# austinjeng/Shift-GCN

Hardware: AMD Instinct MI355X
Metric: skeleton clips/sec fwd+bwd, NTU (3,300,25,2) bs=64; 1/2/4/8 MI355X (higher is better)
Workload: dtype fp32; 1 GPU; NTU Shift-GCN training step (fwd+CE+bwd+SGD), x=(64,3,300,25,2) per GPU; global_batch=64, per_gpu_batch=64, parallelism=dp1, hipgraph=False, world_size=1, backend=none

## Files before the change

### include/shiftgcn.h

```cpp
#ifndef SHIFTGCN_H_
#define SHIFTGCN_H_

#include <stddef.h>

#ifdef __cplusplus
extern "C" {
#endif

#define SGCN_EINVAL (-22)
#define SGCN_ABI_VERSION 23
#define SGCN_ABI_DIAG_FLAG 0x10000

int sgcn_abi_version(void);


int sgcn_tshift_fwd(const float* in, float* out, const float* xpos, const float* ypos,
                    const float* in_scale, const float* in_shift, float* plane_stats,
                    int B, int C, int H, int W, int stride, int ypos_is_raw, void* stream);

int sgcn_tshift_fwd_pre(const float* z, float* out, const float* xpos, const float* ypos,
                        const float* pre_scale, const float* pre_shift, const float* r,
                        const float* r_scale, const float* r_shift, const float* in_scale,
                        const float* in_shift, int B, int C, int H, int W, int stride,
                        int ypos_is_raw, void* stream);

int sgcn_tshift_fwd_tail(const float* in, float* out, const float* xpos, const float* ypos,
                         const float* post_scale, const float* post_shift, const float* r,
                         const float* r_scale, const float* r_shift, const float* gather_m,
                         float* out_gathered, int B, int C, int H, int W, int stride,
                         int ypos_is_raw, void* stream);

int sgcn_tshift_bwd_bnin(const float* dy, const float* y, const float* s, const float* coef,
                         const float* in, const float* xpos, const float* ypos, float* gin,
                         float* gx, float* gy, void* ws, size_t ws_bytes, int B, int C, int H,
                         int W, int ypos_is_raw, void* stream);
size_t sgcn_tshift_bwd_ws_bytes(int B, int C);

int sgcn_tshift_pos_finalize(const void* ws, int B, int C, float* gx, float* gy, void* stream);

int sgcn_tshift_bwd(const float* gout, const float* in, const float* xpos, const float* ypos,
                    const float* in_scale, const float* in_shift, int relu_mask,
                    const float* bn_mean, const float* bn_invstd, float* bn_part, float* gin,
                    float* gx, float* gy, void* ws, size_t ws_bytes, int B, int C, int H,
                    int W, int stride, int ypos_is_raw, void* stream);

int sgcn_tshift_fwd_f64(const double* in, double* out, const double* xpos, const double* ypos,
                        int B, int C, int H, int W, int stride, int ypos_is_raw, void* stream);
size_t sgcn_tshift_bwd_f64_ws_bytes(int B, int C);
int sgcn_tshift_bwd_f64(const double* gout, const double* in, const double* xpos,
                        const double* ypos, double* gin, double* gx, double* gy, void* ws,
                        size_t ws_bytes, int B, int C, int H, int W, int stride,
                        int ypos_is_raw, void* stream);

int sgcn_tshift_bwd_gbn(const float* gout, const float* in, const float* xpos,
                        const float* ypos, const float* in_scale, const float* in_shift,
                        const float* bn_mean, const float* bn_invstd, float* bn_part,
                        const float* z, const float* z_mean, const float* z_invstd,
                        float* z_part, const float* d, const float* d_mean,
                        const float* d_invstd, float* d_part, float* gin, float* gx, float* gy,
                        void* ws, size_t ws_bytes, int B, int C, int H, int W, void* stream);


int sgcn_pw_fwd(const float* w, int w_mcontig, const float* bias, const float* x,
                long long x_bstride, long long x_cstride, int x_tstride, int x_rsign,
                const float* mask, float* y, long long y_bstride, long long y_cstride,
                int y_tstride, int y_rsign, int relu, int accumulate, int B, int M, int K,
                int T, int V, void* stream);

size_t sgcn_pw_tshift_ws_bytes(int K);
int sgcn_pw_fwd_tshift(const float* w, const float* bias, const float* x, long long x_bstride,
                       long long x_cstride, const float* xpos, const float* ypos,
                       const float* in_scale, const float* in_shift, float* x_shifted,
                       void* ws, size_t ws_bytes, float* y, long long y_bstride,
                       long long y_cstride, int relu, int two_row, int B, int M, int K, int T,
                       int V, void* stream);

size_t sgcn_pw_dw_ws_bytes(int B, int M, int Nc, int T, int V);

int sgcn_pw_dw(const float* g, long long g_bstride, long long g_cstride, int g_tstride,
               int g_rsign, const float* x, long long x_bstride, long long x_cstride,
               int x_tstride, int x_rsign, const float* mask, float* dw, int dw_transpose,
               int dw_accumulate, float* dbias, int dbias_accumulate, void* ws,
               size_t ws_bytes, int B, int M, int Nc, int T, int V, void* stream);


size_t sgcn_moments_ws_bytes(int B, int C, int V, int per_joint);

int sgcn_moments(const float* x, float* part, int B, int C, int T, int V, int per_joint,
                 void* stream);


int sgcn_bn_finalize(const float* part, int B, int F, int n_part, int perm_V,
                     const float* gamma, const float* beta, float eps, float momentum,
                     float* running_mean, float* running_var, long long* num_batches,
                     float* mean, float* invstd, float* scale, float* shift, void* stream);

int sgcn_bn_eval_coef(int F, int perm_V, const float* gamma, const float* beta,
                      const float* running_mean, const float* running_var, float eps,
                      float* mean, float* invstd, float* scale, float* shift, void* stream);

int sgcn_bn_apply(const float* x, const float* scale, const float* shift, int per_joint,
                  const float* r, const float* rscale, const float* rshift, int relu,
                  float* y, float* y_stats, const float* gather_m, float* y_gathered, int B,
                  int C, int T, int V, void* stream);
int sgcn_bn_bwd_reduce(const float* dy, const float* y, int relu, const float* x,
                       const float* mean, const float* invstd, int per_joint, const float* r,
                       const float* rmean, const float* rinvstd, const float* dy_coef,
                       float* part, float* rpart, int B, int C, int T, int V, void* stream);

int sgcn_bn_bwd_finalize(const float* part, int B, int F, long long n_total, int perm_V,
                         const float* mean, const float* invstd, const float* gamma,
                         float* dgamma, float* dbeta, int accumulate, int batch_stats,
                         float* coef, void* stream);

int sgcn_bn_bwd_finalize_gbn(const float* part6, int B, int C, int V, long long n_total,
                             const float* dy_coef, const float* dy_mean, const float* mean,
                             const float* invstd, const float* gamma, float* dgamma,
                             float* dbeta, int accumulate, int batch_stats, float* coef,
                             void* stream);

int sgcn_bn_bwd_apply(const float* dy, const float* y, int relu, const float* x,
                      const float* coef, int per_joint, const float* r, const float* rcoef,
                      const float* dy_coef, float* dx, float* dr, int B, int C, int T, int V,
                      void* stream);

int sgcn_mask_prep(const float* mask, float* m, int n, void* stream);

int sgcn_gcn_gather(const float* x0, const float* m, float* xg, int B, int C, int T, int V,
                    void* stream);

int sgcn_gcn_dx_finish(const float* dxt, const float* x0, const float* m, const float* add1,
                       const float* add2, const float* add2_mask, float* dx, float* dmask_part,
                       const float* prev_s, const float* prev_mean, const float* prev_invstd,
                       float* prev_part, int B, int C, int T, int V, void* stream);

int sgcn_mask_grad_finalize(const float* part, const float* mask, int B, int C, int V,
                            float* dmask, int accumulate, void* stream);

int sgcn_modalities(const float* joint, const int* parent, float* out_joint, float* out_bone,
                    float* out_joint_motion, float* out_bone_motion, const float* scale,
                    const float* shift, int planes, int N, int C, int T, int V, int M,
                    void* stream);


size_t sgcn_head_ws_bytes(int N, int C, int V, int M);

int sgcn_head_moments(const float* x, float* part, int N, int C, int T, int V, int M,
                      void* stream);

int sgcn_head_apply(const float* x, const float* scale, const float* shift, float* y, int N,
                    int C, int T, int V, int M, void* stream);

int sgcn_head_bwd_reduce(const float* g, const float* x, const float* mean, const float* invstd,
                         float* part, int N, int C, int T, int V, int M, void* stream);

int sgcn_head_bwd_apply(const float* g, const float* x, const float* coef, float* dx, int N,
                        int C, int T, int V, int M, void* stream);

int sgcn_pool(const float* x, float* out, int N, int M, int C, long long P, void* stream);

int sgcn_pool_bwd(const float* dout, float* dx, int N, int M, int C, long long P,
                  void* stream);


int sgcn_sgd_chunk_elems(void);

int sgcn_sgd_step(const void* table, const int* numel, const int* chunks, int n_chunks,
                  float momentum, int nesterov, void* stream);

#define SGCN_BATCH_MAX 32
int sgcn_tshift_pos_finalize_many(const void* const* partials, float* const* gx,
                                  float* const* gy, const int* B, const int* C, int n,
                                  void* stream);
int sgcn_mask_prep_many(const float* const* mask, float* const* m, const int* count, int n,
                        void* stream);
int sgcn_mask_grad_finalize_many(const float* const* part, const float* const* mask,
                                 float* const* dmask, const int* B, const int* C,
                                 const int* V, int n, void* stream);

#ifdef __cplusplus
}
#endif

#endif
```

### shift-gcn_amd/csrc/bn.hip

```cpp
#include "common.hpp"

namespace sgcn {
namespace {

constexpr int kThreads = 256;

constexpr int kU = 4;

constexpr int kUM = 8;

template <bool PER_JOINT, bool ZU = false>
__global__ __launch_bounds__(kThreads) void moments_kernel(const float* __restrict__ x,
                                                            float2* __restrict__ part, int T,
                                                            int V, int C) {
  SGCN_CRIT_PRIO();
  __shared__ float s1[kThreads], s2[kThreads], red[2 * kThreads / 64];
  const int plane = gridDim.x - 1 - blockIdx.x;
  const int P = T * V;
  const float* __restrict__ xp = x + (size_t)plane * P;
  const int i = threadIdx.x;
  if (PER_JOINT) {
    const int G = kThreads / V;
    float a = 0.f, q = 0.f;
    const int v = i % V, r = i / V;
// ... 286 lines not shown
  if (OUT_STATS) {
    block_sum2(s1, s2, red);
    if (threadIdx.x == 0) {
      const float n = (float)P;
      ystats[plane] = make_float2(k0 + s1 / n, s2 - s1 * s1 / n);
    }
  }
}

template <int NT, int LPT, bool PER_JOINT, int RES, bool RELU, int OUTX, bool ZU>
__global__ __launch_bounds__(NT) void bn_apply_ja_kernel(
    const float* __restrict__ x, const float* __restrict__ scale,
    const float* __restrict__ shift, const float* __restrict__ r,
    const float* __restrict__ rscale, const float* __restrict__ rshift,
    float* __restrict__ y, float2* __restrict__ ystats, const float* __restrict__ gm,
    float* __restrict__ yg, int C, int T, int V) {
  SGCN_CRIT_PRIO();
  constexpr bool OUT_STATS = OUTX == 1, OUT_G = OUTX == 2;
  __shared__ float red[2 * NT / 64];
  const int plane = blockIdx.x, c = plane % C, rc = c % V;
  const int GR = NT / V, NTJ = GR * V, tid = threadIdx.x;
  const bool own = tid < NTJ;
  const int w = tid % V;
  const int P = T * V;
  const size_t off = (size_t)plane * P;
  const unsigned vo = own ? (unsigned)tid * 4u : 0x80000000u, vstep = (unsigned)NTJ * 4u;
  const unsigned pb = (unsigned)P * 4u;
  int wz = w - rc;
  wz = wz < 0 ? wz + V : wz;
  const unsigned xo = vo + (unsigned)((ZU ? wz - w : 0) * 4);
  const unsigned go = vo + (unsigned)((wz - w) * 4);
  float xv[LPT], rv[RES ? LPT : 1];
  {
    const auto xr = make_rsrc(x + off, pb);
#pragma unroll
    for (int e = 0; e < LPT; ++e) xv[e] = bload(xr, xo + e * vstep, 0);
    if (RES) {
      const auto rr = make_rsrc(r + off, pb);
#pragma unroll
      for (int e = 0; e < LPT; ++e) rv[e] = bload(rr, vo + e * vstep, 0);
    }
  }
  const float sc = PER_JOINT ? scale[c * V + w] : scale[c];
  const float sh = PER_JOINT ? shift[c * V + w] : shift[c];
  const float rsc = RES == 2 ? rscale[c] : 1.f, rsh = RES == 2 ? rshift[c] : 0.f;
  const float gmu = OUT_G ? gm[wz * C + c] : 0.f;
  const auto yr = make_rsrc(y + off, pb);
  const auto ygr = make_rsrc(OUT_G ? yg + off : y + off, OUT_G ? pb : 0u);
  const int nval = own ? (P - tid + NTJ - 1) / NTJ : 0;
  float s1 = 0.f;
#pragma unroll
  for (int e = 0; e < LPT; ++e) {
    float a = xv[e] * sc + sh;
    if (RES == 1) a += rv[e];
    if (RES == 2) a += rv[e] * rsc + rsh;
    if (RELU) a = fmaxf(a, 0.f);
    bstore(yr, a, vo + e * vstep, 0);
    if (OUT_G) bstore(ygr, a * gmu, go + e * vstep, 0);
    if (OUT_STATS) {
      xv[e] = e < nval ? a : 0.f;
      s1 += xv[e];
    }
  }
  if (OUT_STATS) {
    s1 = block_sum(s1, red);
    const float mean = s1 / (float)P;
    float m2 = 0.f;
#pragma unroll
    for (int e = 0; e < LPT; ++e) {
      const float d = xv[e] - mean;
      m2 += e < nval ? d * d : 0.f;
    }
    m2 = block_sum(m2, red);
    if (tid == 0) ystats[plane] = make_float2(mean, m2);
  }
}

template <bool PER_JOINT, bool RELU, bool RESBN, bool DYT>
__global__ __launch_bounds__(kThreads) void bn_bwd_reduce_kernel(
    const float* __restrict__ dy, const float* __restrict__ y, const float* __restrict__ x,
    const float* __restrict__ mean, const float* __restrict__ invstd,
    const float* __restrict__ r, const float* __restrict__ rmean,
    const float* __restrict__ rinvstd, const float* __restrict__ dyc, float2* __restrict__ part,
    float2* __restrict__ rpart, int C, int T, int V) {
  SGCN_CRIT_PRIO();
  __shared__ float s0[kThreads], s1[kThreads], red[2 * kThreads / 64];
  const int plane = blockIdx.x, c = plane % C;
  const int P = T * V;
  const size_t off = (size_t)plane * P;
  const int i = threadIdx.x;
  float rm = 0.f, ri = 0.f, d1 = 1.f, d2 = 0.f, d3 = 0.f;
  if (RESBN) { rm = rmean[c]; ri = rinvstd[c]; }
  if (DYT) { d1 = dyc[c]; d2 = dyc[C + c]; d3 = dyc[2 * C + c]; }
  float a0 = 0.f, a1 = 0.f, b0 = 0.f, b1 = 0.f;
  if (PER_JOINT) {
    const int G = kThreads / V;
    const int v = i % V, rr = i / V;
    const int vc = min(v, V - 1);
    const float mu = mean[c * V + vc], is = invstd[c * V + vc];
    int vx = v - c % V;
    vx = vx < 0 ? vx + V : vx;
    const int xd = vx - v;
    if (i < G * V) {
      for (int t0 = rr; t0 < T; t0 += G * kU) {
        float gv[kU], yv[kU], xv[kU], rv[kU];
#pragma unroll
        for (int u = 0; u < kU; ++u) {
          const int o = min(t0 + u * G, T - 1) * V + v;
          gv[u] = dy[off + o];
          if (RELU) yv[u] = y[off + o];
          xv[u] = x[off + o + xd];
          if (RESBN) rv[u] = r[off + o];
        }
#pragma unroll
        for (int u = 0; u < kU; ++u) {
          float g = gv[u];
          if (DYT) g = d1 * g + d2 * yv[u] + d3;
          g = (t0 + u * G < T) ? g : 0.f;
          if (RELU) g = yv[u] > 0.f ? g : 0.f;
          a0 += g;
          a1 += g * ((xv[u] - mu) * is);
          if (RESBN) { b0 += g; b1 += g * ((rv[u] - rm) * ri); }
        }
      }
    }
    if (RESBN) block_sum2(b0, b1, red);
    s0[i] = a0;
    s1[i] = a1;
    __syncthreads();
    if (i < V) {
      float t0 = 0.f, t1 = 0.f;
      for (int g = 0; g < G; ++g) { t0 += s0[g * V + i]; t1 += s1[g * V + i]; }
      part[(size_t)plane * V + i] = make_float2(t0, t1);
    }
    if (RESBN && i == 0) rpart[plane] = make_float2(b0, b1);
  } else {
    const float mu = mean[c], is = invstd[c];
    for (int base = 0; base < P; base += kThreads * kU) {
      float gv[kU], yv[kU], xv[kU], rv[kU];
#pragma unroll
      for (int u = 0; u < kU; ++u) {
        const int o = min(base + u * kThreads + i, P - 1);
        gv[u] = dy[off + o];
        if (RELU) yv[u] = y[off + o];
        xv[u] = x[off + o];
        if (RESBN) rv[u] = r[off + o];
      }
#pragma unroll
      for (int u = 0; u < kU; ++u) {
        float g = gv[u];
        if (DYT) g = d1 * g + d2 * yv[u] + d3;
        g = (base + u * kThreads + i < P) ? g : 0.f;
        if (RELU) g = yv[u] > 0.f ? g : 0.f;
        a0 += g;
        a1 += g * ((xv[u] - mu) * is);
        if (RESBN) { b0 += g; b1 += g * ((rv[u] - rm) * ri); }
      }
    }
    block_sum2(a0, a1, red);
    if (RESBN) block_sum2(b0, b1, red);
    if (i == 0) {
      part[plane] = make_float2(a0, a1);
      if (RESBN) rpart[plane] = make_float2(b0, b1);
    }
  }
}

template <int NT, int LPT, bool PER_JOINT, bool RELU, bool RESBN, bool DYT>
__global__ __launch_bounds__(NT) void bn_bwd_reduce_ja_kernel(
    const float* __restrict__ dy, const float* __restrict__ y, const float* __restrict__ x,
    const float* __restrict__ mean, const float* __restrict__ invstd,
    const float* __restrict__ r, const float* __restrict__ rmean,
    const float* __restrict__ rinvstd, const float* __restrict__ dyc, float2* __restrict__ part,
    float2* __restrict__ rpart, int C, int T, int V) {
  SGCN_CRIT_PRIO();
  __shared__ float s0[NT], s1[NT], red[2 * NT / 64];
  const int plane = blockIdx.x, c = plane % C;
  const int GR = NT / V, NTJ = GR * V, tid = threadIdx.x;
  const bool own = tid < NTJ;
  const int w = tid % V;
  const int P = T * V;
  const size_t off = (size_t)plane * P;
  const unsigned vo = own ? (unsigned)tid * 4u : 0x80000000u, vstep = (unsigned)NTJ * 4u;
  const unsigned pb = (unsigned)P * 4u;
  int vx = w - c % V;
  vx = vx < 0 ? vx + V : vx;
  const unsigned xo = vo + (unsigned)((PER_JOINT ? vx - w : 0) * 4);
  float gv[LPT], yv[RELU ? LPT : 1], xv[LPT], rv[RESBN ? LPT : 1];
  {
    const auto dyr = make_rsrc(dy + off, pb), xr = make_rsrc(x + off, pb);
#pragma unroll
    for (int e = 0; e < LPT; ++e) {
      gv[e] = bload(dyr, vo + e * vstep, 0);
      xv[e] = bload(xr, xo + e * vstep, 0);
    }
    if (RELU) {
      const auto yr = make_rsrc(y + off, pb);
#pragma unroll
      for (int e = 0; e < LPT; ++e) yv[e] = bload(yr, vo + e * vstep, 0);
    }
    if (RESBN) {
      const auto rr = make_rsrc(r + off, pb);
#pragma unroll
      for (int e = 0; e < LPT; ++e) rv[e] = bload(rr, vo + e * vstep, 0);
    }
  }
  float rm = 0.f, ri = 0.f, d1 = 1.f, d2 = 0.f, d3 = 0.f;
  if (RESBN) { rm = rmean[c]; ri = rinvstd[c]; }
  if (DYT) { d1 = dyc[c]; d2 = dyc[C + c]; d3 = dyc[2 * C + c]; }
  const float mu = PER_JOINT ? mean[c * V + w] : mean[c];
  const float is = PER_JOINT ? invstd[c * V + w] : invstd[c];
  const int nval = own ? (P - tid + NTJ - 1) / NTJ : 0;
  float a0 = 0.f, a1 = 0.f, b0 = 0.f, b1 = 0.f;
#pragma unroll
  for (int e = 0; e < LPT; ++e) {
    float g = gv[e];
    if (DYT) g = d1 * g + d2 * yv[e] + d3;
    g = e < nval ? g : 0.f;
    if (RELU) g = yv[e] > 0.f ? g : 0.f;
    a0 += g;
    a1 = fmaf(g, (xv[e] - mu) * is, a1);
    if (RESBN) { b0 += g; b1 = fmaf(g, (rv[e] - rm) * ri, b1); }
  }
  if (PER_JOINT) {
    if (RESBN) block_sum2(b0, b1, red);
    s0[tid] = a0;
    s1[tid] = a1;
    __syncthreads();
    if (tid < V) {
      float t0 = 0.f, t1 = 0.f;
      for (int g = 0; g < GR; ++g) { t0 += s0[g * V + tid]; t1 += s1[g * V + tid]; }
      part[(size_t)plane * V + tid] = make_float2(t0, t1);
    }
    if (RESBN && tid == 0) rpart[plane] = make_float2(b0, b1);
  } else {
    block_sum2(a0, a1, red);
    if (RESBN) block_sum2(b0, b1, red);
    if (tid == 0) {
      part[plane] = make_float2(a0, a1);
      if (RESBN) rpart[plane] = make_float2(b0, b1);
    }
  }
}

__global__ __launch_bounds__(64 * kFSW) void bn_bwd_finalize_kernel(
    const float2* __restrict__ part, int B, int F, double n_total, int perm_V,
    const float* __restrict__ mean, const float* __restrict__ invstd,
    const float* __restrict__ gamma, float* __restrict__ dgamma, float* __restrict__ dbeta,
    int accumulate, int batch_stats, float* __restrict__ coef) {
  SGCN_CRIT_PRIO();
  double sg, sgx, unused;
  int f;
  if (!feature_sums(part, B, F, sg, sgx, unused, f)) return;
  const int rf = ref_feature(f, perm_V, F);
  if (dgamma) dgamma[rf] = accumulate ? dgamma[rf] + (float)sgx : (float)sgx;
  if (dbeta) dbeta[rf] = accumulate ? dbeta[rf] + (float)sg : (float)sg;
  const float g = gamma ? gamma[rf] : 1.f;
  const float3 k = bn_bwd_coef(sg, sgx, g, invstd[f], mean[f], n_total, batch_stats);
  coef[f] = k.x;
  coef[F + f] = k.y;
  coef[2 * F + f] = k.z;
}

#ifndef SGCN_GBN_WAVES
#define SGCN_GBN_WAVES 4
#endif
constexpr int kGbnW = SGCN_GBN_WAVES;
__global__ __launch_bounds__(64 * kGbnW) void bn_bwd_finalize_gbn_kernel(
    const float* __restrict__ part6, int B, int F, int V, double n_total,
    const float* __restrict__ dyc, const float* __restrict__ dym, int C,
    const float* __restrict__ mean, const float* __restrict__ invstd,
    const float* __restrict__ gamma, float* __restrict__ dgamma, float* __restrict__ dbeta,
    int accumulate, int batch_stats, float* __restrict__ coef) {
  SGCN_CRIT_PRIO();
  __shared__ double red[kGbnW - 1][6][64];
  const int lane = threadIdx.x & 63, w = threadIdx.x >> 6;
  const int f = blockIdx.x * 64 + lane;
  const int fc = min(f, F - 1);
// ... 93 lines not shown
      }
    }
#pragma unroll
    for (int u = 0; u < kU; ++u) {
      const int o = base + u * kThreads + threadIdx.x;
      float g = gv[u];
      if (DYT) g = d1 * g + d2 * yv[u] + d3;
      if (RELU) g = yv[u] > 0.f ? g : 0.f;
      if (PER_JOINT) { k1 = k_s[v]; k2 = k_s[kThreads + v]; k3 = k_s[2 * kThreads + v]; }
      if (o < P) {
        int od = o;
        if (GATH) {
          const int w = v - rc;
          od = o - v + (w < 0 ? w + V : w);
        }
        dx[off + od] = k1 * g + k2 * xv[u] + k3;
        if (RES == 1) dr[off + o] = g;
        if (RES == 2) dr[off + o] = q1 * g + q2 * rv[u] + q3;
      }
      v += dv;
      if (v >= V) v -= V;
    }
  }
}

template <int NT, int LPT, int PJM, bool RELU, int RES, bool DYT>
__global__ __launch_bounds__(NT) void bn_bwd_apply_ja_kernel(
    const float* __restrict__ dy, const float* __restrict__ y, const float* __restrict__ x,
    const float* __restrict__ coef, int F, const float* __restrict__ r,
    const float* __restrict__ rcoef, int RF, const float* __restrict__ dyc,
    float* __restrict__ dx, float* __restrict__ dr, int C, int T, int V) {
  SGCN_CRIT_PRIO();
  static_assert(PJM == 0 || PJM == 3, "per-channel, or per-joint gathered (ZU)");
  constexpr bool PER_JOINT = PJM == 3;
  const int plane = blockIdx.x, c = plane % C, rc = c % V;
  const int GR = NT / V, NTJ = GR * V, tid = threadIdx.x;
  const bool own = tid < NTJ;
  const int w = tid % V;
  const int P = T * V;
  const size_t off = (size_t)plane * P;
  const unsigned vo = own ? (unsigned)tid * 4u : 0x80000000u, vstep = (unsigned)NTJ * 4u;
  const unsigned pb = (unsigned)P * 4u;
  int wz = w - rc;
  wz = wz < 0 ? wz + V : wz;
  const unsigned go = vo + (unsigned)((PER_JOINT ? wz - w : 0) * 4);
  float gv[LPT], yv[RELU ? LPT : 1], xv[LPT], rv[RES == 2 ? LPT : 1];
  {
    const auto dyr = make_rsrc(dy + off, pb);
    const auto xr = make_rsrc(x + off, pb);
#pragma unroll
    for (int e = 0; e < LPT; ++e) {
      gv[e] = bload(dyr, vo + e * vstep, 0);
      xv[e] = bload(xr, go + e * vstep, 0);
    }
    if (RELU) {
      const auto yr = make_rsrc(y + off, pb);
#pragma unroll
      for (int e = 0; e < LPT; ++e) yv[e] = bload(yr, vo + e * vstep, 0);
    }
    if (RES == 2) {
      const auto rr = make_rsrc(r + off, pb);
#pragma unroll
      for (int e = 0; e < LPT; ++e) rv[e] = bload(rr, vo + e * vstep, 0);
    }
  }
  const int f = PER_JOINT ? c * V + w : c;
  const float k1 = coef[f], k2 = coef[F + f], k3 = coef[2 * F + f];
  float d1 = 1.f, d2 = 0.f, d3 = 0.f, q1 = 0.f, q2 = 0.f, q3 = 0.f;
  if (DYT) { d1 = dyc[c]; d2 = dyc[C + c]; d3 = dyc[2 * C + c]; }
  if (RES == 2) { q1 = rcoef[c]; q2 = rcoef[RF + c]; q3 = rcoef[2 * RF + c]; }
  const auto dxr = make_rsrc(dx + off, pb);
  const auto drr = make_rsrc(RES ? dr + off : dx + off, RES ? pb : 0u);
#pragma unroll
  for (int e = 0; e < LPT; ++e) {
    float g = gv[e];
    if (DYT) g = d1 * g + d2 * yv[e] + d3;
    if (RELU) g = yv[e] > 0.f ? g : 0.f;
    bstore(dxr, k1 * g + k2 * xv[e] + k3, go + e * vstep, 0);
    if (RES == 1) bstore(drr, g, vo + e * vstep, 0);
    if (RES == 2) bstore(drr, q1 * g + q2 * rv[e] + q3, vo + e * vstep, 0);
  }
}

template <int NT, int LPT, bool ADD1, bool ADD2, bool PART, bool A2M>
__global__ __launch_bounds__(NT) void gcn_dx_finish_ja_kernel(
    const float* __restrict__ dxt, const float* __restrict__ x0, const float* __restrict__ m,
    const float* __restrict__ add1, const float* __restrict__ add2, float* __restrict__ dx,
    float* __restrict__ dmask_part, const float* __restrict__ ps,
    const float* __restrict__ pmean, const float* __restrict__ pinvstd,
    float2* __restrict__ bn_part, int C, int T, int V, const float* __restrict__ add2m) {
  SGCN_CRIT_PRIO();
#ifdef SGCN_DIAG_F1B_REAL
  return;
#endif
  __shared__ float s0[NT];
  __shared__ float red[2 * NT / 64];
  const int plane = blockIdx.x, c = plane % C, rc = c % V;
  const int GR = NT / V, NTJ = GR * V, tid = threadIdx.x;
  const bool own = tid < NTJ;
  const int vd = tid % V;
  int us = vd - rc;
  us = us < 0 ? us + V : us;
  const int P = T * V;
  const size_t off = (size_t)plane * P;
  const unsigned vo = own ? (unsigned)tid * 4u : 0x80000000u, vstep = (unsigned)NTJ * 4u;
  const unsigned pb = (unsigned)P * 4u;
  const unsigned uo = vo + (unsigned)((us - vd) * 4);
  float gv[LPT], xq[LPT], a1[ADD1 ? LPT : 1], a2[ADD2 ? LPT : 1], a2q[A2M ? LPT : 1];
  float sv[PART ? LPT : 1];
  {
#ifdef SGCN_DIAG_F1B_BOUND
    const auto gr = make_rsrc(dxt + off, 0u), xr = make_rsrc(x0 + off, pb);
#else
    const auto gr = make_rsrc(dxt + off, pb), xr = make_rsrc(x0 + off, pb);
#endif
#pragma unroll
    for (int e = 0; e < LPT; ++e) {
      gv[e] = bload(gr, uo + e * vstep, 0);
      xq[e] = bload(xr, vo + e * vstep, 0);
    }
    if (ADD1) {
      const auto ar = make_rsrc(add1 + off, pb);
#pragma unroll
      for (int e = 0; e < LPT; ++e) a1[e] = bload(ar, vo + e * vstep, 0);
    }
    if (ADD2) {
      const auto ar = make_rsrc(add2 + off, pb);
#pragma unroll
      for (int e = 0; e < LPT; ++e) a2[e] = bload(ar, vo + e * vstep, 0);
    }
    if (A2M) {
      const auto ar = make_rsrc(add2m + off, pb);
#pragma unroll
      for (int e = 0; e < LPT; ++e) a2q[e] = bload(ar, vo + e * vstep, 0);
    }
    if (PART) {
      const auto ar = make_rsrc(ps + off, pb);
#pragma unroll
      for (int e = 0; e < LPT; ++e) sv[e] = bload(ar, vo + e * vstep, 0);
    }
  }
  const float mu = m[us * C + c];
  float pm = 0.f, pi = 0.f;
  if (PART) { pm = pmean[c]; pi = pinvstd[c]; }
  const auto dxr = make_rsrc(dx + off, pb);
  float acc = 0.f, b0 = 0.f, b1 = 0.f;
#pragma unroll
  for (int e = 0; e < LPT; ++e) {
    float val = gv[e] * mu;
    if (ADD1) val += a1[e];
    if (ADD2) val += A2M ? (a2q[e] > 0.f ? a2[e] : 0.f) : a2[e];
    bstore(dxr, val, vo + e * vstep, 0);
    acc = fmaf(gv[e], xq[e], acc);
    if (PART) {
      const float g = xq[e] > 0.f ? val : 0.f;
      b0 += g;
      b1 = fmaf(g, (sv[e] - pm) * pi, b1);
    }
  }
  if (PART) {
    block_sum2(b0, b1, red);
    if (tid == 0) bn_part[plane] = make_float2(b0, b1);
  }
  s0[tid] = acc;
  __syncthreads();
  if (tid < V) {
    int vq = tid + rc;
    vq = vq >= V ? vq - V : vq;
    float sum = 0.f;
    for (int g = 0; g < GR; ++g) sum += s0[g * V + vq];
    dmask_part[(size_t)plane * V + tid] = sum;
  }
}

__global__ __launch_bounds__(kThreads) void gcn_gather_kernel(const float* __restrict__ x0,
                                                              const float* __restrict__ m,
                                                              float* __restrict__ xg, int C,
                                                              int T, int V) {
  SGCN_CRIT_PRIO();
  __shared__ float m_s[kThreads];
  const int plane = blockIdx.x, c = plane % C;
  const int P = T * V;
  const size_t off = (size_t)plane * P;
  const int rc = c % V;
  if ((int)threadIdx.x < V) m_s[threadIdx.x] = m[threadIdx.x * C + c];
  __syncthreads();
  const int dv = kThreads % V;
  int w = threadIdx.x % V;
  for (int base = 0; base < P; base += kThreads * kU) {
    float xv[kU], mv[kU];
    int ww = w;
#pragma unroll
    for (int u = 0; u < kU; ++u) {
      const int oraw = base + u * kThreads + (int)threadIdx.x;
      int src = ww + rc;
      src = src >= V ? src - V : src;
      xv[u] = x0[off + min(oraw - ww + src, P - 1)];
      mv[u] = m_s[ww];
      ww += dv;
      if (ww >= V) ww -= V;
    }
#pragma unroll
    for (int u = 0; u < kU; ++u) {
      const int o = base + u * kThreads + (int)threadIdx.x;
      if (o < P) xg[off + o] = xv[u] * mv[u];
    }
    w = ww;
  }
}

template <bool ADD1, bool ADD2, bool PART, bool A2M = false>
__global__ __launch_bounds__(kThreads) void gcn_dx_finish_kernel(
    const float* __restrict__ dxt, const float* __restrict__ x0, const float* __restrict__ m,
    const float* __restrict__ add1, const float* __restrict__ add2, float* __restrict__ dx,
    float* __restrict__ dmask_part, const float* __restrict__ ps,
    const float* __restrict__ pmean, const float* __restrict__ pinvstd,
    float2* __restrict__ bn_part, int C, int T, int V, const float* __restrict__ add2m) {
  SGCN_CRIT_PRIO();
  __shared__ float s0[kThreads];
  const int plane = blockIdx.x, c = plane % C;
  const size_t off = (size_t)plane * T * V;
  const int rc = c % V;
  const int i = threadIdx.x;
  const int G = kThreads / V;
  const int vd = i % V, rr = i / V;
  int us = vd - rc;
  us = us < 0 ? us + V : us;
  const float mu = m[us * C + c];
  float pm = 0.f, pi = 0.f;
  if (PART) { pm = pmean[c]; pi = pinvstd[c]; }
  float acc = 0.f, b0 = 0.f, b1 = 0.f;
  if (i < G * V) {
    for (int t0 = rr; t0 < T; t0 += G * kU) {
      float gv[kU], xq[kU], a1[kU], a2[kU], sv[kU], a2q[kU];
#pragma unroll
      for (int k = 0; k < kU; ++k) {
        const int row = min(t0 + k * G, T - 1) * V;
        gv[k] = dxt[off + row + us];
        xq[k] = x0[off + row + vd];
        if (ADD1) a1[k] = add1[off + row + vd];
        if (ADD2) a2[k] = add2[off + row + vd];
        if (A2M) a2q[k] = add2m[off + row + vd];
        if (PART) sv[k] = ps[off + row + vd];
      }
#pragma unroll
      for (int k = 0; k < kU; ++k) {
        const int t = t0 + k * G;
        float val = gv[k] * mu;
        if (ADD1) val += a1[k];
        if (ADD2) val += A2M ? (a2q[k] > 0.f ? a2[k] : 0.f) : a2[k];
        if (t < T) dx[off + t * V + vd] = val;
        acc += (t < T) ? gv[k] * xq[k] : 0.f;
        if (PART) {
          const float g = (t < T && xq[k] > 0.f) ? val : 0.f;
          b0 += g;
          b1 += g * ((sv[k] - pm) * pi);
        }
      }
    }
  }
  if (PART) {
    __shared__ float red[2 * kThreads / 64];
    block_sum2(b0, b1, red);
    if (i == 0) bn_part[plane] = make_float2(b0, b1);
  }
  s0[i] = acc;
  __syncthreads();
  if (i < V) {
    int vq = i + rc;
    vq = vq >= V ? vq - V : vq;
    float sum = 0.f;
    for (int g = 0; g < G; ++g) sum += s0[g * V + vq];
    dmask_part[(size_t)plane * V + i] = sum;
  }
}

__global__ void mask_prep_kernel(const float* __restrict__ mask, float* __restrict__ m, int n) {
  const int i = blockIdx.x * blockDim.x + threadIdx.x;
  if (i < n) m[i] = tanhf(mask[i]) + 1.f;
}

struct MaskPrepBatch {
  const float* mask[SGCN_BATCH_MAX];
  float* m[SGCN_BATCH_MAX];
  int n[SGCN_BATCH_MAX];
};
__global__ void mask_prep_many_kernel(const MaskPrepBatch t) {
  const int e = blockIdx.y;
  const int i = blockIdx.x * blockDim.x + threadIdx.x;
  if (i < t.n[e]) t.m[e][i] = tanhf(t.mask[e][i]) + 1.f;
}

__device__ __forceinline__ void mask_grad_body(const float* __restrict__ part,
                                               const float* __restrict__ mask, int B, int C,
                                               int V, float* __restrict__ dmask,
                                               int accumulate);
__global__ __launch_bounds__(64 * kFW) void mask_grad_finalize_kernel(
    const float* __restrict__ part, const float* __restrict__ mask, int B, int C, int V,
    float* __restrict__ dmask, int accumulate) {
  mask_grad_body(part, mask, B, C, V, dmask, accumulate);
}
struct MaskGradBatch {
  const float* part[SGCN_BATCH_MAX];
  const float* mask[SGCN_BATCH_MAX];
  float* dmask[SGCN_BATCH_MAX];
  int B[SGCN_BATCH_MAX];
  int C[SGCN_BATCH_MAX];
  int V[SGCN_BATCH_MAX];
};
__global__ __launch_bounds__(64 * kFW) void mask_grad_finalize_many_kernel(const MaskGradBatch t) {
  const int i = blockIdx.y;
  if ((int)blockIdx.x * kFW >= t.C[i] * t.V[i]) return;
  mask_grad_body(t.part[i], t.mask[i], t.B[i], t.C[i], t.V[i], t.dmask[i], 0);
}
__device__ __forceinline__ void mask_grad_body(const float* __restrict__ part,
                                               const float* __restrict__ mask, int B, int C,
                                               int V, float* __restrict__ dmask,
                                               int accumulate) {
  const int F = C * V;
  const int lane = threadIdx.x & 63;
  const int f = blockIdx.x * kFW + (int)(threadIdx.x >> 6);
  const int fc = min(f, F - 1);
  double a = 0.0;
  for (int b0 = lane; b0 < B; b0 += 64 * 4) {
    float pv[4];
#pragma unroll
    for (int u = 0; u < 4; ++u) {
      const int b = b0 + u * 64;
      pv[u] = b < B ? part[(size_t)b * F + fc] : 0.f;
    }
#pragma unroll
    for (int u = 0; u < 4; ++u) a += pv[u];
  }
  const double s = wave_dsum(a);
// ... 105 lines not shown
  if (per_joint == 3) SGCN_REQUIRE(relu && !y_gathered);
  {
    const int nt = T * V <= kJaSplit ? kThreads : 512;
    const int lpt = ja_lpt(T, V, nt);
    if (lpt) {
      const int ox = ys ? 1 : (y_gathered ? 2 : 0);
#define SGCN_AJ(NT, L, PJ, RS, RL, OX, ZU)                                                     \
  bn_apply_ja_kernel<NT, L, PJ, RS, RL, OX, ZU><<<g, NT, 0, st>>>(                             \
      x, scale, shift, r, rscale, rshift, y, ys, gather_m, y_gathered, C, T, V)
#define SGCN_AJ_L(NT, PJ, RS, RL, OX, ZU)                                                      \
  do {                                                                                         \
    if (lpt == 8) SGCN_AJ(NT, 8, PJ, RS, RL, OX, ZU);                                          \
    else if (lpt == 16) SGCN_AJ(NT, 16, PJ, RS, RL, OX, ZU);                                   \
    else if (lpt == 24) SGCN_AJ(NT, 24, PJ, RS, RL, OX, ZU);                                   \
    else SGCN_AJ(NT, 32, PJ, RS, RL, OX, ZU);                                                  \
  } while (0)
#define SGCN_AJ_T(PJ, RS, RL, OX, ZU)                                                          \
  do {                                                                                         \
    if (nt == kThreads) SGCN_AJ_L(kThreads, PJ, RS, RL, OX, ZU);                               \
    else SGCN_AJ_L(512, PJ, RS, RL, OX, ZU);                                                   \
  } while (0)
#define SGCN_AJ_O(PJ, RS, RL, ZU)                                                              \
  do {                                                                                         \
    if (ox == 1) SGCN_AJ_T(PJ, RS, RL, 1, ZU);                                                 \
    else if (ox == 2) SGCN_AJ_T(PJ, RS, RL, 2, ZU);                                            \
    else SGCN_AJ_T(PJ, RS, RL, 0, ZU);                                                         \
  } while (0)
      if (per_joint == 3) {
        if (ys) {
          if (res == 0) SGCN_AJ_T(true, 0, true, 1, true);
          else if (res == 1) SGCN_AJ_T(true, 1, true, 1, true);
          else SGCN_AJ_T(true, 2, true, 1, true);
        } else {
          if (res == 0) SGCN_AJ_T(true, 0, true, 0, true);
          else if (res == 1) SGCN_AJ_T(true, 1, true, 0, true);
          else SGCN_AJ_T(true, 2, true, 0, true);
        }
      } else if (relu) {
        if (res == 0) SGCN_AJ_O(false, 0, true, false);
        else if (res == 1) SGCN_AJ_O(false, 1, true, false);
        else SGCN_AJ_O(false, 2, true, false);
      } else {
        if (res == 0) SGCN_AJ_O(false, 0, false, false);
        else if (res == 1) SGCN_AJ_O(false, 1, false, false);
        else SGCN_AJ_O(false, 2, false, false);
      }
#undef SGCN_AJ_O
#undef SGCN_AJ_T
#undef SGCN_AJ_L
#undef SGCN_AJ
      SGCN_LAUNCH_CHECK();
      return 0;
    }
  }
#define SGCN_APPLY_X(PJ, RS, RL, OX)                                                        \
  bn_apply_kernel<PJ, RS, RL, OX><<<g, kThreads, 0, st>>>(x, scale, shift, r, rscale, rshift, y, \
                                                          ys, gather_m, y_gathered, C, T, V)
#define SGCN_APPLY(PJ, RS, RL)                                                               \
  (ys ? SGCN_APPLY_X(PJ, RS, RL, 1)                                                          \
      : (y_gathered ? SGCN_APPLY_X(PJ, RS, RL, 2) : SGCN_APPLY_X(PJ, RS, RL, 0)))
#define SGCN_APPLY_R(PJ, RL) \
  if (res == 0) SGCN_APPLY(PJ, 0, RL); else if (res == 1) SGCN_APPLY(PJ, 1, RL); else SGCN_APPLY(PJ, 2, RL)
  if (per_joint == 3) {
#define SGCN_APPLY_ZU(RS)                                                                      \
  (ys ? bn_apply_kernel<true, RS, true, 1, true><<<g, kThreads, 0, st>>>(                      \
            x, scale, shift, r, rscale, rshift, y, ys, gather_m, y_gathered, C, T, V)          \
      : bn_apply_kernel<true, RS, true, 0, true><<<g, kThreads, 0, st>>>(                      \
            x, scale, shift, r, rscale, rshift, y, ys, gather_m, y_gathered, C, T, V))
    if (res == 0) SGCN_APPLY_ZU(0); else if (res == 1) SGCN_APPLY_ZU(1); else SGCN_APPLY_ZU(2);
#undef SGCN_APPLY_ZU
  }
  else if (relu) { SGCN_APPLY_R(false, true); } else { SGCN_APPLY_R(false, false); }
#undef SGCN_APPLY_R
#undef SGCN_APPLY
#undef SGCN_APPLY_X
  SGCN_LAUNCH_CHECK();
  return 0;
}

int sgcn_bn_bwd_reduce(const float* dy, const float* y, int relu, const float* x,
                       const float* mean, const float* invstd, int per_joint, const float* r,
                       const float* rmean,
                       const float* rinvstd, const float* dy_coef, float* part, float* rpart,
                       int B, int C, int T, int V, void* stream) {
  SGCN_PLANE_CHECK();
  SGCN_REQUIRE(B > 0 && T > 0 && dy && x && mean && invstd && part && (y || !relu));
  SGCN_REQUIRE(!dy_coef || (y && relu));
  SGCN_REQUIRE((r == nullptr) == (rpart == nullptr) && (!r || (rmean && rinvstd)));
  SGCN_REQUIRE(per_joint == 0 || per_joint == 3);
  hipStream_t st = (hipStream_t)stream;
  dim3 g(B * C);
  const bool rb = r != nullptr;
  if (per_joint == 3) SGCN_REQUIRE(relu);
  {
    const int nt = T * V <= kJaSplit ? kThreads : 512;
    const int lpt = ja_lpt(T, V, nt);
    if (lpt) {
#define SGCN_RJ(NT, L, PJ, RL, RB)                                                             \
  (dy_coef ? bn_bwd_reduce_ja_kernel<NT, L, PJ, RL, RB, true><<<g, NT, 0, st>>>(                \
                 dy, y, x, mean, invstd, r, rmean, rinvstd, dy_coef, (float2*)part,            \
                 (float2*)rpart, C, T, V)                                                      \
           : bn_bwd_reduce_ja_kernel<NT, L, PJ, RL, RB, false><<<g, NT, 0, st>>>(               \
                 dy, y, x, mean, invstd, r, rmean, rinvstd, dy_coef, (float2*)part,            \
                 (float2*)rpart, C, T, V))
#define SGCN_RJ_L(NT, PJ, RL, RB)                                                              \
  do {                                                                                         \
    if (lpt == 8) SGCN_RJ(NT, 8, PJ, RL, RB); else if (lpt == 16) SGCN_RJ(NT, 16, PJ, RL, RB); \
    else if (lpt == 24) SGCN_RJ(NT, 24, PJ, RL, RB);                                           \
    else SGCN_RJ(NT, 32, PJ, RL, RB);                                                          \
  } while (0)
#define SGCN_RJ_T(PJ, RL, RB)                                                                  \
  do { if (nt == kThreads) SGCN_RJ_L(kThreads, PJ, RL, RB); else SGCN_RJ_L(512, PJ, RL, RB); } while (0)
      if (per_joint == 3) { if (rb) SGCN_RJ_T(true, true, true); else SGCN_RJ_T(true, true, false); }
      else if (relu) { if (rb) SGCN_RJ_T(false, true, true); else SGCN_RJ_T(false, true, false); }
      else { if (rb) SGCN_RJ_T(false, false, true); else SGCN_RJ_T(false, false, false); }
#undef SGCN_RJ_T
#undef SGCN_RJ_L
#undef SGCN_RJ
      SGCN_LAUNCH_CHECK();
      return 0;
    }
  }
#define SGCN_RED(PJ, RL, RB)                                                                \
  (dy_coef ? bn_bwd_reduce_kernel<PJ, RL, RB, true><<<g, kThreads, 0, st>>>(                   \
                 dy, y, x, mean, invstd, r, rmean, rinvstd, dy_coef, (float2*)part,           \
                 (float2*)rpart, C, T, V)                                                     \
           : bn_bwd_reduce_kernel<PJ, RL, RB, false><<<g, kThreads, 0, st>>>(                  \
                 dy, y, x, mean, invstd, r, rmean, rinvstd, dy_coef, (float2*)part,           \
                 (float2*)rpart, C, T, V))
  if (per_joint == 3) {
    if (rb) SGCN_RED(true, true, true); else SGCN_RED(true, true, false);
  } else {
    if (relu) { if (rb) SGCN_RED(false, true, true); else SGCN_RED(false, true, false); }
    else { if (rb) SGCN_RED(false, false, true); else SGCN_RED(false, false, false); }
  }
#undef SGCN_RED
  SGCN_LAUNCH_CHECK();
  return 0;
}

int sgcn_bn_bwd_finalize(const float* part, int B, int F, long long n_total, int perm_V,
                         const float* mean, const float* invstd, const float* gamma,
                         float* dgamma, float* dbeta, int accumulate, int batch_stats,
                         float* coef, void* stream) {
  SGCN_REQUIRE(part && B > 0 && F > 0 && n_total > 0 && mean && invstd && coef);
  SGCN_REQUIRE(perm_V <= 0 || F % perm_V == 0);
  bn_bwd_finalize_kernel<<<(F + 63) / 64, 64 * kFSW, 0, (hipStream_t)stream>>>(
      (const float2*)part, B, F, (double)n_total, perm_V, mean, invstd, gamma, dgamma, dbeta,
      accumulate, batch_stats, coef);
  SGCN_LAUNCH_CHECK();
  return 0;
}

int sgcn_bn_bwd_finalize_gbn(const float* part6, int B, int C, int V, long long n_total,
                             const float* dy_coef, const float* dy_mean, const float* mean,
                             const float* invstd, const float* gamma, float* dgamma,
                             float* dbeta, int accumulate, int batch_stats, float* coef,
                             void* stream) {
  SGCN_REQUIRE(part6 && B > 0 && C > 0 && V > 0 && n_total > 0 && dy_coef && dy_mean && mean &&
               invstd && coef);
  const int F = C * V;
  bn_bwd_finalize_gbn_kernel<<<(F + 63) / 64, 64 * kGbnW, 0, (hipStream_t)stream>>>(
      part6, B, F, V, (double)n_total, dy_coef, dy_mean, C, mean, invstd, gamma, dgamma, dbeta,
      accumulate, batch_stats, coef);
  SGCN_LAUNCH_CHECK();
  return 0;
}

int sgcn_bn_bwd_apply(const float* dy, const float* y, int relu, const float* x,
                      const float* coef, int per_joint, const float* r, const float* rcoef,
                      const float* dy_coef, float* dx, float* dr, int B, int C, int T, int V,
                      void* stream) {
  SGCN_PLANE_CHECK();
  if (B == 0 || T == 0) return 0;
  SGCN_REQUIRE(dy && x && coef && dx && (y || !relu));
  SGCN_REQUIRE(!dy_coef || (y && relu));
  SGCN_REQUIRE(!rcoef || (r && dr));
  SGCN_REQUIRE(per_joint == 0 || per_joint == 3);
  hipStream_t st = (hipStream_t)stream;
  const int res = dr == nullptr ? 0 : (rcoef ? 2 : 1);
  const int F = per_joint ? C * V : C;
  dim3 g(B * C);
  if (per_joint == 3) SGCN_REQUIRE(relu);
  {
    const int nt = T * V <= kJaSplit ? kThreads : 512;
    const int lpt = ja_lpt(T, V, nt);
    if (lpt) {
#define SGCN_BJ(NT, L, PJ, RL, RS)                                                             \
  (dy_coef ? bn_bwd_apply_ja_kernel<NT, L, PJ, RL, RS, true><<<g, NT, 0, st>>>(                 \
                 dy, y, x, coef, F, r, rcoef, C, dy_coef, dx, dr, C, T, V)             \
           : bn_bwd_apply_ja_kernel<NT, L, PJ, RL, RS, false><<<g, NT, 0, st>>>(                \
                 dy, y, x, coef, F, r, rcoef, C, dy_coef, dx, dr, C, T, V))
#define SGCN_BJ_L(NT, PJ, RL, RS)                                                              \
  do {                                                                                         \
    if (lpt == 8) SGCN_BJ(NT, 8, PJ, RL, RS);                                                  \
    else if (lpt == 16) SGCN_BJ(NT, 16, PJ, RL, RS);                                           \
    else if (lpt == 24) SGCN_BJ(NT, 24, PJ, RL, RS);                                           \
    else SGCN_BJ(NT, 32, PJ, RL, RS);                                                          \
  } while (0)
#define SGCN_BJ_T(PJ, RL, RS)                                                                  \
  do { if (nt == kThreads) SGCN_BJ_L(kThreads, PJ, RL, RS); else SGCN_BJ_L(512, PJ, RL, RS); } while (0)
#define SGCN_BJ_R(PJ, RL)                                                                      \
  do {                                                                                         \
    if (res == 0) SGCN_BJ_T(PJ, RL, 0);                                                        \
    else if (res == 1) SGCN_BJ_T(PJ, RL, 1);                                                   \
    else SGCN_BJ_T(PJ, RL, 2);                                                                 \
  } while (0)
      if (per_joint == 3) SGCN_BJ_R(3, true);
      else if (relu) SGCN_BJ_R(0, true);
      else SGCN_BJ_R(0, false);
#undef SGCN_BJ_R
#undef SGCN_BJ_T
// ... 2 lines not shown
      SGCN_LAUNCH_CHECK();
      return 0;
    }
  }
#define SGCN_BA(PJ, RL, RS)                                                                   \
  (dy_coef ? bn_bwd_apply_kernel<PJ, RL, RS, true><<<g, kThreads, 0, st>>>(                      \
                 dy, y, x, coef, F, r, rcoef, C, dy_coef, dx, dr, C, T, V)                      \
           : bn_bwd_apply_kernel<PJ, RL, RS, false><<<g, kThreads, 0, st>>>(                     \
                 dy, y, x, coef, F, r, rcoef, C, dy_coef, dx, dr, C, T, V))
#define SGCN_BA_R(PJ, RL) \
  if (res == 0) SGCN_BA(PJ, RL, 0); else if (res == 1) SGCN_BA(PJ, RL, 1); else SGCN_BA(PJ, RL, 2)
  if (per_joint == 3) { SGCN_BA_R(3, true); }
  else if (relu) { SGCN_BA_R(0, true); } else { SGCN_BA_R(0, false); }
#undef SGCN_BA_R
#undef SGCN_BA
  SGCN_LAUNCH_CHECK();
  return 0;
}

int sgcn_mask_prep(const float* mask, float* m, int n, void* stream) {
  SGCN_REQUIRE(mask && m && n > 0);
  mask_prep_kernel<<<(n + 255) / 256, 256, 0, (hipStream_t)stream>>>(mask, m, n);
  SGCN_LAUNCH_CHECK();
  return 0;
}

int sgcn_mask_prep_many(const float* const* mask, float* const* m, const int* count, int n,
                        void* stream) {
  SGCN_REQUIRE(n >= 0 && n <= SGCN_BATCH_MAX);
  if (n == 0) return 0;
  SGCN_REQUIRE(mask && m && count);
  MaskPrepBatch t{};
  int mx = 0;
  for (int i = 0; i < n; ++i) {
    SGCN_REQUIRE(mask[i] && m[i] && count[i] > 0);
    t.mask[i] = mask[i];
    t.m[i] = m[i];
    t.n[i] = count[i];
    mx = max(mx, count[i]);
  }
  mask_prep_many_kernel<<<dim3((mx + 255) / 256, n), 256, 0, (hipStream_t)stream>>>(t);
  SGCN_LAUNCH_CHECK();
  return 0;
}

int sgcn_mask_grad_finalize_many(const float* const* part, const float* const* mask,
                                 float* const* dmask, const int* B, const int* C,
                                 const int* V, int n, void* stream) {
  SGCN_REQUIRE(n >= 0 && n <= SGCN_BATCH_MAX);
  if (n == 0) return 0;
  SGCN_REQUIRE(part && mask && dmask && B && C && V);
  MaskGradBatch t{};
  int mf = 0;
  for (int i = 0; i < n; ++i) {
    SGCN_REQUIRE(part[i] && mask[i] && dmask[i] && B[i] > 0 && C[i] > 0 && V[i] > 0);
    t.part[i] = part[i];
    t.mask[i] = mask[i];
    t.dmask[i] = dmask[i];
    t.B[i] = B[i];
    t.C[i] = C[i];
    t.V[i] = V[i];
    mf = max(mf, C[i] * V[i]);
  }
  mask_grad_finalize_many_kernel<<<dim3((mf + kFW - 1) / kFW, n), 64 * kFW, 0,
                                   (hipStream_t)stream>>>(t);
  SGCN_LAUNCH_CHECK();
  return 0;
}

int sgcn_gcn_gather(const float* x0, const float* m, float* xg, int B, int C, int T, int V,
                    void* stream) {
  SGCN_PLANE_CHECK();
  if (B == 0 || T == 0) return 0;
  SGCN_REQUIRE(x0 && m && xg && x0 != xg);
  gcn_gather_kernel<<<B * C, kThreads, 0, (hipStream_t)stream>>>(x0, m, xg, C, T, V);
  SGCN_LAUNCH_CHECK();
  return 0;
}

int sgcn_gcn_dx_finish(const float* dxt, const float* x0, const float* m, const float* add1,
                       const float* add2, const float* add2_mask, float* dx, float* dmask_part,
                       const float* prev_s, const float* prev_mean, const float* prev_invstd,
                       float* prev_part, int B,
                       int C, int T, int V, void* stream) {
  SGCN_PLANE_CHECK();
  if (B == 0 || T == 0) return 0;
  SGCN_REQUIRE(dxt && x0 && m && dx && dmask_part);
  SGCN_REQUIRE(!prev_part || (prev_s && prev_mean && prev_invstd));
  SGCN_REQUIRE(!add2_mask || add2);
  hipStream_t st = (hipStream_t)stream;
  float2* pp = (float2*)prev_part;
  if (add2_mask) SGCN_REQUIRE(add1);
  {
    const int nt = T * V <= kJaSplit ? kThreads : 512;
    const int lpt = ja_lpt(T, V, nt);
    if (lpt) {
#define SGCN_FJ(NT, L, A1, A2, PT, AM)                                                         \
  gcn_dx_finish_ja_kernel<NT, L, A1, A2, PT, AM><<<B * C, NT, 0, st>>>(                        \
      dxt, x0, m, add1, add2, dx, dmask_part, prev_s, prev_mean, prev_invstd, pp, C, T, V,     \
      add2_mask)
#define SGCN_FJ_L(NT, A1, A2, PT, AM)                                                          \
  do {                                                                                         \
    if (lpt == 8) SGCN_FJ(NT, 8, A1, A2, PT, AM);                                              \
    else if (lpt == 16) SGCN_FJ(NT, 16, A1, A2, PT, AM);                                       \
    else if (lpt == 24) SGCN_FJ(NT, 24, A1, A2, PT, AM);                                       \
    else SGCN_FJ(NT, 32, A1, A2, PT, AM);                                                      \
  } while (0)
#define SGCN_FJ_T(A1, A2, PT, AM)                                                              \
  do { if (nt == kThreads) SGCN_FJ_L(kThreads, A1, A2, PT, AM); else SGCN_FJ_L(512, A1, A2, PT, AM); } while (0)
#define SGCN_FJ_P(A1, A2, AM)                                                                  \
  do { if (pp) SGCN_FJ_T(A1, A2, true, AM); else SGCN_FJ_T(A1, A2, false, AM); } while (0)
      if (add2_mask) SGCN_FJ_P(true, true, true);
      else if (add1) { if (add2) SGCN_FJ_P(true, true, false); else SGCN_FJ_P(true, false, false); }
      else { if (add2) SGCN_FJ_P(false, true, false); else SGCN_FJ_P(false, false, false); }
#undef SGCN_FJ_P
#undef SGCN_FJ_T
#undef SGCN_FJ_L
#undef SGCN_FJ
      SGCN_LAUNCH_CHECK();
      return 0;
    }
  }
  if (add2_mask) {
    if (pp)
      gcn_dx_finish_kernel<true, true, true, true><<<B * C, kThreads, 0, st>>>(
          dxt, x0, m, add1, add2, dx, dmask_part, prev_s, prev_mean, prev_invstd, pp, C, T, V,
          add2_mask);
    else
      gcn_dx_finish_kernel<true, true, false, true><<<B * C, kThreads, 0, st>>>(
          dxt, x0, m, add1, add2, dx, dmask_part, prev_s, prev_mean, prev_invstd, pp, C, T, V,
          add2_mask);
    SGCN_LAUNCH_CHECK();
    return 0;
  }
#define SGCN_FIN(A1, A2, PT)                                                                \
  gcn_dx_finish_kernel<A1, A2, PT><<<B * C, kThreads, 0, st>>>(                           \
      dxt, x0, m, add1, add2, dx, dmask_part, prev_s, prev_mean, prev_invstd, pp, C, T, V,  \
      nullptr)
#define SGCN_FIN_P(A1, A2)                                                                  \
  do {                                                                                      \
    if (pp) SGCN_FIN(A1, A2, true);                                                         \
    else SGCN_FIN(A1, A2, false);                                                           \
  } while (0)
  if (add1) { if (add2) SGCN_FIN_P(true, true); else SGCN_FIN_P(true, false); }
  else { if (add2) SGCN_FIN_P(false, true); else SGCN_FIN_P(false, false); }
#undef SGCN_FIN_P
#undef SGCN_FIN
  SGCN_LAUNCH_CHECK();
  return 0;
}

int sgcn_mask_grad_finalize(const float* part, const float* mask, int B, int C, int V,
                            float* dmask, int accumulate, void* stream) {
  SGCN_REQUIRE(part && mask && dmask && B > 0 && C > 0 && V > 0);
  mask_grad_finalize_kernel<<<(C * V + kFW - 1) / kFW, 64 * kFW, 0,
                              (hipStream_t)stream>>>(part, mask, B, C, V, dmask, accumulate);
  SGCN_LAUNCH_CHECK();
  return 0;
}

}
```

### shift-gcn_amd/csrc/head.hip

```cpp
#include "common.hpp"

namespace sgcn {
namespace {

constexpr int kHT = 256;
constexpr int kHU = 8;

__device__ __forceinline__ int clip_col(int j, int V, int M) {
  const int m = j / V, v = j - m * V;
  return v * M + m;
}

__global__ __launch_bounds__(kHT) void head_moments_kernel(const float* __restrict__ x,
                                                           float2* __restrict__ part, int C,
                                                           int T, int V, int M) {
  SGCN_CRIT_PRIO();
  __shared__ float s1[kHT], s2[kHT];
  const int nc = blockIdx.x, n = nc / C, c = nc - n * C;
  const int J = V * M, F = J * C;
  const float* __restrict__ xs = x + (size_t)nc * T * J;
  const int i = threadIdx.x;
  const int Jc = min(J, kHT), G = kHT / Jc;
  const int jl = i % Jc, r = i / Jc;
  for (int jb = 0; jb < J; jb += Jc) {
// ... 82 lines not shown
        for (int u = 0; u < kHU; ++u) {
          const float gg = (t0 + u * G < T) ? gv[u] : 0.f;
          a += gg;
          b += gg * ((xv[u] - mu) * is);
        }
      }
    }
    s1[i] = a;
    s2[i] = b;
    __syncthreads();
    if (i < Jc && jb + i < J) {
      float ta = 0.f, tb = 0.f;
      for (int k = 0; k < G; ++k) { ta += s1[k * Jc + i]; tb += s2[k * Jc + i]; }
      const int jj = jb + i, mm = jj / V, vv = jj - mm * V;
      part[(size_t)n * F + (mm * V + vv) * C + c] = make_float2(ta, tb);
    }
    __syncthreads();
  }
}

__global__ __launch_bounds__(kHT) void head_bwd_apply_kernel(
    const float* __restrict__ g, const float* __restrict__ x, const float* __restrict__ coef,
    float* __restrict__ dx, long long total, int C, int T, int V, int M) {
  SGCN_CRIT_PRIO();
  const long long i = (long long)blockIdx.x * kHT + threadIdx.x;
  if (i >= total) return;
  long long r = i;
  const int m = (int)(r % M); r /= M;
  const int v = (int)(r % V); r /= V;
  const int t = (int)(r % T); r /= T;
  const int c = (int)(r % C);
  const long long n = r / C;
  const int F = M * V * C, f = (m * V + v) * C + c;
  const float gv = g[(((n * M + m) * C + c) * T + t) * V + v];
  dx[i] = coef[f] * gv + coef[F + f] * x[i] + coef[2 * F + f];
}

__global__ __launch_bounds__(kHT) void pool_kernel(const float* __restrict__ x,
                                                   float* __restrict__ out, int C, int M,
                                                   long long P) {
  SGCN_CRIT_PRIO();
  __shared__ float red[2 * kHT / 64];
  const int nc = blockIdx.x, n = nc / C, c = nc - n * C;
  float acc = 0.f;
  for (int m = 0; m < M; ++m) {
    const float* __restrict__ xp = x + (((size_t)n * M + m) * C + c) * P;
    float s[4] = {0.f, 0.f, 0.f, 0.f};
    for (long long p0 = threadIdx.x; p0 < P; p0 += 4 * kHT) {
#pragma unroll
      for (int u = 0; u < 4; ++u) {
        const long long p = p0 + u * kHT;
        s[u] += p < P ? xp[p] : 0.f;
      }
    }
    float tot = (s[0] + s[1]) + (s[2] + s[3]);
    tot = block_sum(tot, red);
    acc += tot * (1.f / (float)P);
  }
  if (threadIdx.x == 0) out[nc] = acc * (1.f / (float)M);
}

__global__ __launch_bounds__(kHT) void pool_bwd_kernel(const float* __restrict__ dout,
                                                       float* __restrict__ dx, long long total,
                                                       int C, int M, long long P) {
  SGCN_CRIT_PRIO();
  const long long i0 = ((long long)blockIdx.x * kHT + threadIdx.x) * 4;
  if (i0 >= total) return;
  const float rm = 1.f / (float)M, rp = 1.f / (float)P;
  float v[4];
#pragma unroll
  for (int u = 0; u < 4; ++u) {
    const long long row = (i0 + u) / P;
    const int c = (int)(row % C);
    const long long n = row / C / M;
    v[u] = i0 + u < total ? (dout[n * C + c] * rm) * rp : 0.f;
  }
  if (i0 + 4 <= total) {
    *reinterpret_cast<float4*>(dx + i0) = make_float4(v[0], v[1], v[2], v[3]);
  } else {
    for (int u = 0; u < 4 && i0 + u < total; ++u) dx[i0 + u] = v[u];
  }
}

unsigned grid1(long long total) { return (unsigned)((total + kHT - 1) / kHT); }

}
}

using namespace sgcn;

extern "C" {

size_t sgcn_head_ws_bytes(int N, int C, int V, int M) {
  return (size_t)(N > 0 ? N : 0) * C * V * M * sizeof(float2);
}

int sgcn_head_moments(const float* x, float* part, int N, int C, int T, int V, int M,
                      void* stream) {
  SGCN_REQUIRE(N >= 0 && C > 0 && T > 0 && V > 0 && M > 0);
  if (N == 0) return 0;
  SGCN_REQUIRE(x && part);
  SGCN_REQUIRE((long long)N * C < (1ll << 31) && (long long)T * V * M < (1ll << 31));
  head_moments_kernel<<<N * C, kHT, 0, (hipStream_t)stream>>>(x, (float2*)part, C, T, V, M);
  SGCN_LAUNCH_CHECK();
  return 0;
}

int sgcn_head_apply(const float* x, const float* scale, const float* shift, float* y, int N,
                    int C, int T, int V, int M, void* stream) {
  SGCN_REQUIRE(N >= 0 && C > 0 && T > 0 && V > 0 && M > 0);
  const long long total = (long long)N * M * C * T * V;
  if (total == 0) return 0;
  SGCN_REQUIRE(x && scale && shift && y);
  SGCN_REQUIRE(total < (1ll << 40));
  head_apply_kernel<<<grid1(total), kHT, 0, (hipStream_t)stream>>>(x, scale, shift, y, total,
                                                                    C, T, V, M);
  SGCN_LAUNCH_CHECK();
  return 0;
}

int sgcn_head_bwd_reduce(const float* g, const float* x, const float* mean, const float* invstd,
                         float* part, int N, int C, int T, int V, int M, void* stream) {
  SGCN_REQUIRE(N >= 0 && C > 0 && T > 0 && V > 0 && M > 0);
  if (N == 0) return 0;
  SGCN_REQUIRE(g && x && mean && invstd && part);
  SGCN_REQUIRE((long long)N * C < (1ll << 31) && (long long)T * V * M < (1ll << 31));
  head_bwd_reduce_kernel<<<N * C, kHT, 0, (hipStream_t)stream>>>(g, x, mean, invstd,
                                                                 (float2*)part, C, T, V, M);
  SGCN_LAUNCH_CHECK();
  return 0;
}

int sgcn_head_bwd_apply(const float* g, const float* x, const float* coef, float* dx, int N,
                        int C, int T, int V, int M, void* stream) {
  SGCN_REQUIRE(N >= 0 && C > 0 && T > 0 && V > 0 && M > 0);
  const long long total = (long long)N * M * C * T * V;
  if (total == 0) return 0;
  SGCN_REQUIRE(g && x && coef && dx);
  SGCN_REQUIRE(total < (1ll << 40));
  head_bwd_apply_kernel<<<grid1(total), kHT, 0, (hipStream_t)stream>>>(g, x, coef, dx, total, C,
                                                                        T, V, M);
  SGCN_LAUNCH_CHECK();
  return 0;
}

int sgcn_pool(const float* x, float* out, int N, int M, int C, long long P, void* stream) {
  SGCN_REQUIRE(N >= 0 && M > 0 && C > 0 && P > 0);
  if (N == 0) return 0;
  SGCN_REQUIRE(x && out);
  SGCN_REQUIRE((long long)N * C < (1ll << 31));
  pool_kernel<<<N * C, kHT, 0, (hipStream_t)stream>>>(x, out, C, M, P);
  SGCN_LAUNCH_CHECK();
  return 0;
}

int sgcn_pool_bwd(const float* dout, float* dx, int N, int M, int C, long long P,
                  void* stream) {
  SGCN_REQUIRE(N >= 0 && M > 0 && C > 0 && P > 0);
  const long long total = (long long)N * M * C * P;
  if (total == 0) return 0;
  SGCN_REQUIRE(dout && dx && ((uintptr_t)dx & 15) == 0);
  SGCN_REQUIRE(total < (1ll << 40));
  pool_bwd_kernel<<<grid1((total + 3) / 4), kHT, 0, (hipStream_t)stream>>>(dout, dx, total, C,
                                                                           M, P);
  SGCN_LAUNCH_CHECK();
  return 0;
}

}
```

### shift-gcn_amd/csrc/tshift.hip

```cpp
#include "common.hpp"

#pragma clang fp contract(off)

namespace sgcn {
namespace {

constexpr int kThreads = 256;


struct Geom {
  int x1, y1;
  float dx, dy;
};

__device__ __forceinline__ Geom make_geom(float x, float y) {
  Geom g;
  g.x1 = (int)floorf(x);
  g.y1 = (int)floorf(y);
  g.dx = x - (float)g.x1;
  g.dy = y - (float)g.y1;
  return g;
}

__device__ __forceinline__ float blend(float q11, float q21, float q12, float q22, float dx,
// ... 660 lines not shown
        const int h2 = h1 + 1;
        const int hq1 = (h1 % 2 == 0) ? h1 / 2 : -1;
        const int hq2 = (h2 % 2 == 0) ? h2 / 2 : -1;
        TapIdx t1, t2;
        tap_idx(hq1, w1, Ho, W, t1);
        tap_idx(hq2, w1, Ho, W, t2);
        ti.o00 = t1.o00; ti.o01 = t1.o01; ti.m00 = t1.m00; ti.m01 = t1.m01;
        ti.o10 = t2.o00; ti.o11 = t2.o01; ti.m10 = t2.m00; ti.m11 = t2.m01;
      }
      float val = 0.f;
      if (nt > 0) {
        const float q11 = sel(gs[ti.o00], ti.m00), q21 = sel(gs[ti.o01], ti.m01);
        const float q12 = sel(gs[ti.o10], ti.m10), q22 = sel(gs[ti.o11], ti.m11);
        val = blend(q11, q21, q12, q22, r.dx, r.dy);
      }
      const float rin = xs[o];
      if (RELU_MASK) val = rin > 0.f ? val : 0.f;
      gi[o] = val;
      if (BNP) {
        bs0 += val;
        bs1 += val * ((rin - bmu) * bis);
      }
      pos.next();
    }
  }

  if (JA) {
    const Geom g = make_geom(x, y);
    const int NTJ = (NT / W) * W, GR = NT / W;
    if ((int)threadIdx.x < NTJ) {
      const int w = (int)threadIdx.x % W, wc = w + g.x1;
      const bool c0 = (unsigned)wc < (unsigned)W, c1 = (unsigned)(wc + 1) < (unsigned)W;
      const int cc0 = min(max(wc, 0), W - 1), cc1 = min(max(wc + 1, 0), W - 1);
      int h = (int)threadIdx.x / W;
      for (int o = threadIdx.x; o < nt; o += NTJ, h += GR) {
        const int rr = h * STRIDE + g.y1;
        const bool r0 = (unsigned)rr < (unsigned)Hb, r1 = (unsigned)(rr + 1) < (unsigned)Hb;
        const int p0 = min(max(rr, 0), Hb - 1) * W, p1 = min(max(rr + 1, 0), Hb - 1) * W;
        float q11 = xs[p0 + cc0], q21 = xs[p0 + cc1], q12 = xs[p1 + cc0], q22 = xs[p1 + cc1];
        if (AFFINE) { q11 = q11 * a + b; q21 = q21 * a + b; q12 = q12 * a + b; q22 = q22 * a + b; }
        q11 = (r0 && c0) ? q11 : 0.f;
        q21 = (r0 && c1) ? q21 : 0.f;
        q12 = (r1 && c0) ? q12 : 0.f;
        q22 = (r1 && c1) ? q22 : 0.f;
        const float vx = (1.f - g.dy) * (q21 - q11) + g.dy * (q22 - q12);
        const float vy = (1.f - g.dx) * (q12 - q11) + g.dx * (q22 - q21);
        const float gg = gs[o];
        ax += vx * gg;
        ay += vy * gg;
      }
    }
  } else {
    const Geom g = make_geom(x, y);
    Walker pos(threadIdx.x, NT, W);
    for (int o = threadIdx.x; o < nt; o += NT) {
      TapIdx ti;
      tap_idx(pos.h * STRIDE + g.y1, pos.w + g.x1, Hb, W, ti);
      float q11 = xs[ti.o00], q21 = xs[ti.o01], q12 = xs[ti.o10], q22 = xs[ti.o11];
      if (AFFINE) { q11 = q11 * a + b; q21 = q21 * a + b; q12 = q12 * a + b; q22 = q22 * a + b; }
      q11 = sel(q11, ti.m00);
      q21 = sel(q21, ti.m01);
      q12 = sel(q12, ti.m10);
      q22 = sel(q22, ti.m11);
      const float vx = (1.f - g.dy) * (q21 - q11) + g.dy * (q22 - q12);
      const float vy = (1.f - g.dx) * (q12 - q11) + g.dx * (q22 - q21);
      const float gg = gs[o];
      ax += vx * gg;
      ay += vy * gg;
      pos.next();
    }
  }
  if (BNP) {
    block_sum4(ax, ay, bs0, bs1, red);
    if (threadIdx.x == 0) {
      pgrad[plane] = make_float2(ax, ay);
      bn_part[plane] = make_float2(bs0, bs1);
    }
  } else {
    block_sum2(ax, ay, red);
    if (threadIdx.x == 0) pgrad[plane] = make_float2(ax, ay);
  }
}

template <int NT, int LPT, bool AFFINE, bool RELU_MASK, bool BNP, bool GP, bool GBN,
          bool GBD = false>
__global__ __launch_bounds__(NT) void tshift_bwd_ra_kernel(
    const float* __restrict__ gout, const float* __restrict__ in,
    const float* __restrict__ xpos, const float* __restrict__ ypos,
    const float* __restrict__ scale, const float* __restrict__ shift,
    const float* __restrict__ bn_mean, const float* __restrict__ bn_invstd,
    float* __restrict__ gin, float2* __restrict__ pgrad, float2* __restrict__ bn_part, int C,
    int H, int W, const float* __restrict__ gdy, const float* __restrict__ gy,
    const float* __restrict__ gx, const float* __restrict__ gcoef,
    const float* __restrict__ gz, const float* __restrict__ gzm,
    const float* __restrict__ gzi, float* __restrict__ gzpart, const float* __restrict__ gd = nullptr,
    const float* __restrict__ gdm = nullptr, const float* __restrict__ gdi = nullptr,
    float* __restrict__ gdpart = nullptr) {
  SGCN_CRIT_PRIO();
  static_assert(!GBN || (AFFINE && BNP && !GP), "GBN: shift_in with BNP");
  static_assert(!GBD || GBN, "GBD extends GBN");
  extern __shared__ float lds[];
  __shared__ float red[4 * NT / 64];
  const int plane = gridDim.x - 1 - blockIdx.x;
  const int c = plane % C;
  const int n = H * W, WP = W + 2;
  const int GR = NT / W, NTE = GR * W;
  const int tid = threadIdx.x;
  const bool own = tid < NTE;
  const int w = tid % W, h0 = tid / W;
  const unsigned vo = own ? (unsigned)tid * 4u : 0x80000000u;
  const unsigned vstep = (unsigned)NTE * 4u, nbytes = (unsigned)n * 4u;
  const size_t poff = (size_t)plane * n;
#ifdef SGCN_DIAG_X1B_BOUND
  const unsigned gbytes = AFFINE && !GP && C >= SGCN_DIAG_X1B_BOUND ? 0u : nbytes;
#else
  const unsigned gbytes = nbytes;
#endif
  float t[LPT], rin_r[LPT];
  float zr[GBN ? LPT : 1], dr[GBD ? LPT : 1];
  {
    const auto inr = make_rsrc(in + poff, nbytes);
    if (GP) {
      const auto dyr = make_rsrc(gdy + poff, nbytes);
      const auto yr = make_rsrc(gy + poff, nbytes);
      const auto xr = make_rsrc(gx + poff, nbytes);
      float u1[LPT], u2[LPT];
#pragma unroll
      for (int e = 0; e < LPT; ++e) {
        const unsigned vb = vo + e * vstep;
        t[e] = bload(dyr, vb, 0);
        u1[e] = bload(yr, vb, 0);
        u2[e] = bload(xr, vb, 0);
        rin_r[e] = bload(inr, vb, 0);
      }
      const float k1 = gcoef[c], k2 = gcoef[C + c], k3 = gcoef[2 * C + c];
#pragma unroll
      for (int e = 0; e < LPT; ++e) t[e] = k1 * (u1[e] > 0.f ? t[e] : 0.f) + k2 * u2[e] + k3;
    } else {
      const auto gr = make_rsrc(gout + poff, gbytes);
#pragma unroll
      for (int e = 0; e < LPT; ++e) {
        t[e] = bload(gr, vo + e * vstep, 0);
        rin_r[e] = bload(inr, vo + e * vstep, 0);
      }
      if (GBN) {
        const auto zrr = make_rsrc(gz + poff, nbytes);
        int wz = w - c % W;
        wz = wz < 0 ? wz + W : wz;
        const unsigned zo = vo + (unsigned)((wz - w) * 4);
#pragma unroll
        for (int e = 0; e < LPT; ++e) zr[e] = bload(zrr, zo + e * vstep, 0);
      }
      if (GBD) {
        const auto drr = make_rsrc(gd + poff, nbytes);
#pragma unroll
        for (int e = 0; e < LPT; ++e) dr[e] = bload(drr, vo + e * vstep, 0);
      }
    }
  }
  zero_pad<NT>(lds, H, W);
  const int lbase = (h0 + kPadRows) * WP + w + 1, lstep = GR * WP;
  const int lspare = ra_pad_floats(H, W);
#pragma unroll
  for (int e = 0; e < LPT; ++e)
    lds[own && e * NTE + tid < n ? lbase + e * lstep : lspare] = t[e];
  float bmu = 0.f, bis = 0.f;
  if (BNP) { bmu = bn_mean[c]; bis = bn_invstd[c]; }
  const float x = xpos[c], y = ypos[c];
  float a = 1.f, b = 0.f;
  if (AFFINE) { a = scale[c]; b = shift[c]; }
  float zm = 0.f, zi = 0.f, dmu = 0.f, dis = 0.f;
  if (GBN) { zm = gzm[c * W + w]; zi = gzi[c * W + w]; }
  if (GBD) { dmu = gdm[c]; dis = gdi[c]; }
  __syncthreads();

  const Geom r = make_geom(-x, -y);
  const Geom g = make_geom(x, y);
  const bool fits = r.y1 >= -kPadRows && r.y1 <= kPadRows - 1 && g.y1 >= -kPadRows &&
                    g.y1 <= kPadRows - 1 && r.x1 >= -1 && r.x1 <= 0 && g.x1 >= -1 && g.x1 <= 0;
  const int kq = r.y1 * WP + r.x1, kg = (-g.y1 - 1) * WP - g.x1 - 1;
  const int nfull = n / NTE;
  const int lmax = (H - 1 + kPadRows) * WP + W;
  const auto gir = make_rsrc(gin + poff, nbytes);
  float bs0 = 0.f, bs1 = 0.f, ax = 0.f, ay = 0.f;
  float a6[6] = {0.f, 0.f, 0.f, 0.f, 0.f, 0.f};
  float d6[6] = {0.f, 0.f, 0.f, 0.f, 0.f, 0.f};
  auto elem = [&](int e, bool tail, float q11, float q21, float q12, float q22, float G11,
                  float G21, float G12, float G22) {
    const bool ok = !tail || e * NTE + tid < n;
    float val = blend(q11, q21, q12, q22, r.dx, r.dy);
    const float rin = rin_r[e];
    if (RELU_MASK) val = rin > 0.f ? val : 0.f;
    if (tail) val = ok ? val : 0.f;
    bstore(gir, val, vo + e * vstep, 0);
    if (GBN) {
      const bool act = rin > 0.f;
      const float hc = act ? rin - bmu : 0.f, zh = act ? (zr[e] - zm) * zi : 0.f;
      const float vv = act ? val : 0.f;
      a6[0] += vv;
      a6[1] += hc;
      a6[2] += act ? 1.f : 0.f;
      a6[3] = fmaf(vv, zh, a6[3]);
      a6[4] = fmaf(hc, zh, a6[4]);
      a6[5] += zh;
      if (GBD) {
        const float dh = act ? (dr[e] - dmu) * dis : 0.f;
        d6[0] += vv;
        d6[1] += hc;
        d6[2] += act ? 1.f : 0.f;
        d6[3] = fmaf(vv, dh, d6[3]);
        d6[4] = fmaf(hc, dh, d6[4]);
        d6[5] += dh;
      }
    }
    if (BNP) {
      bs0 += val;
      bs1 = fmaf(val, (rin - bmu) * bis, bs1);
    }
    const float cx = (1.f - g.dy) * (G21 - G11) + g.dy * (G22 - G12);
    const float cy = (1.f - g.dx) * (G12 - G11) + g.dx * (G22 - G21);
// ... 235 lines not shown
  return true;
}

template <int EPT, int STRIDE>
void launch_bwd(bool affine, bool relu, const float* gout, const float* in, const float* xpos,
                const float* ypos, const float* scale, const float* shift, const float* bmu,
                const float* bis, float* gin, float2* pg, float2* bp, int B, int C, int H,
                int W, int Ho, int add_half, hipStream_t st) {
  dim3 grid(B * C), block(kThreads);
#define SGCN_BWD(A, R, P)                                                                    \
  tshift_bwd_kernel<EPT, A, R, STRIDE, P><<<grid, block, 0, st>>>(                            \
      gout, in, xpos, ypos, scale, shift, bmu, bis, gin, pg, bp, C, H, W, Ho, add_half)
  if (bp) {
    if (affine) {
      if (relu) SGCN_BWD(true, true, true); else SGCN_BWD(true, false, true);
    } else {
      if (relu) SGCN_BWD(false, true, true); else SGCN_BWD(false, false, true);
    }
  } else {
    if (affine) {
      if (relu) SGCN_BWD(true, true, false); else SGCN_BWD(true, false, false);
    } else {
      if (relu) SGCN_BWD(false, true, false); else SGCN_BWD(false, false, false);
    }
  }
#undef SGCN_BWD
}

constexpr int kBwdThreads = 512;

template <int LPT, bool JA>
void launch_bwd_s2(bool affine, bool relu, const float* gout, const float* in,
                   const float* xpos, const float* ypos, const float* scale,
                   const float* shift, const float* bmu, const float* bis, float* gin,
                   float2* pg, float2* bp, int B, int C, int H, int W, int Ho, int add_half,
                   hipStream_t st) {
  constexpr int NT = kBwdThreads;
  dim3 grid(B * C), block(NT);
  const size_t lds = (size_t)(H + Ho) * W * sizeof(float);
#define SGCN_BWDL(A, R, P)                                                                  \
  tshift_bwd_s2_kernel<NT, LPT, A, R, P, JA><<<grid, block, lds, st>>>(                      \
      gout, in, xpos, ypos, scale, shift, bmu, bis, gin, pg, bp, C, H, W, Ho, add_half)
  if (bp) {
    if (affine) {
      if (relu) SGCN_BWDL(true, true, true); else SGCN_BWDL(true, false, true);
    } else {
      if (relu) SGCN_BWDL(false, true, true); else SGCN_BWDL(false, false, true);
    }
  } else {
    if (affine) {
      if (relu) SGCN_BWDL(true, true, false); else SGCN_BWDL(true, false, false);
    } else {
      if (relu) SGCN_BWDL(false, true, false); else SGCN_BWDL(false, false, false);
    }
  }
#undef SGCN_BWDL
}

int pick_lpt(int n, int nt) {
  const int per = (n + nt - 1) / nt;
  return per <= 8 ? 8 : (per <= 16 ? 16 : 32);
}

int ra_lpt(int n, int nt, int W) {
  const int nte = (nt / W) * W;
  if (nte <= 0 || W > 64) return 0;
  const int per = (n + nte - 1) / nte;
  if (nt == 512 && per > 8 && per <= 12) return 12;
  if (nt == 512 && per > 16 && per <= 20) return 20;
  return per <= 8 ? 8 : (per <= 16 ? 16 : (per <= 24 ? 24 : (per <= 32 ? 32 : 0)));
}

constexpr int kRaSplit256 = 8192;
#ifndef SGCN_GBD_SPLIT
#define SGCN_GBD_SPLIT 1
#endif

size_t ra_lds_bytes(int H, int W, int nt, bool gbn) {
  const int f = ra_pad_floats(H, W);
  return (size_t)(gbn ? max(f + 1, 6 * nt) : f + 1) * sizeof(float);
}
constexpr size_t kRaLdsMax = 65536;

template <bool AFFINE, bool RELU, bool BNP, bool GP, bool GBN, bool GBD = false>
bool launch_ra(int nt, const float* gout, const float* in, const float* xpos,
               const float* ypos, const float* scale, const float* shift, const float* bmu,
               const float* bis, float* gin, float2* pg, float2* bp, int B, int C, int H,
               int W, const float* gdy, const float* gy, const float* gx, const float* gcoef,
               const float* gz, const float* gzm, const float* gzi, float* gzpart,
               hipStream_t st, const float* gd = nullptr, const float* gdm = nullptr,
               const float* gdi = nullptr, float* gdpart = nullptr) {
  const int lpt = ra_lpt(H * W, nt, W);
  const size_t lds = ra_lds_bytes(H, W, nt, GBN);
  if (lpt == 0 || lds > kRaLdsMax) return false;
#define SGCN_RA(NT, L)                                                                         \
  tshift_bwd_ra_kernel<NT, L, AFFINE, RELU, BNP, GP, GBN, GBD><<<B * C, NT, lds, st>>>(        \
      gout, in, xpos, ypos, scale, shift, bmu, bis, gin, pg, bp, C, H, W, gdy, gy, gx, gcoef,  \
      gz, gzm, gzi, gzpart, gd, gdm, gdi, gdpart)
  if (nt == 256) {
    if (lpt == 8) SGCN_RA(256, 8); else if (lpt == 16) SGCN_RA(256, 16); else if (lpt == 24) SGCN_RA(256, 24); else SGCN_RA(256, 32);
  } else {
    if (lpt == 8) SGCN_RA(512, 8); else if (lpt == 12) SGCN_RA(512, 12); else if (lpt == 16) SGCN_RA(512, 16);
    else if (lpt == 20) SGCN_RA(512, 20); else if (lpt == 24) SGCN_RA(512, 24); else SGCN_RA(512, 32);
  }
#undef SGCN_RA
  return true;
}

int pick_ept(int n) {
  const int per = (n + kThreads - 1) / kThreads;
  return per <= 8 ? 8 : (per <= 16 ? 16 : 32);
}

}
}

using namespace sgcn;

extern "C" {

int sgcn_tshift_fwd(const float* in, float* out, const float* xpos, const float* ypos,
                    const float* in_scale, const float* in_shift, float* plane_stats, int B,
                    int C, int H, int W, int stride, int ypos_is_raw, void* stream) {
  SGCN_REQUIRE(B >= 0 && C > 0 && H >= 0 && W > 0 && stride >= 1);
  SGCN_REQUIRE((in_scale == nullptr) == (in_shift == nullptr));
  const int Ho = H / stride;
  if (B == 0 || Ho == 0) return 0;
  SGCN_REQUIRE(in && out && xpos && ypos);
  SGCN_REQUIRE((long long)H * W < (1LL << 30) && (long long)B * C < (1LL << 31));
  hipStream_t st = (hipStream_t)stream;
  const bool aff = in_scale != nullptr, stats = plane_stats != nullptr;
  float2* ps = (float2*)plane_stats;
  const int ah = (ypos_is_raw && stride != 1) ? 1 : 0;
  if (H * W <= kFwdLdsMax2 &&
      (H * W <= kFwdLdsMax
           ? launch_fwd_pad<kThreads>(aff, stats, in, out, xpos, ypos, in_scale, in_shift, ps, B, C, H, W, Ho, stride, ah, st)
           : launch_fwd_pad<512>(aff, stats, in, out, xpos, ypos, in_scale, in_shift, ps, B, C, H, W, Ho, stride, ah, st))) {
    SGCN_LAUNCH_CHECK();
    return 0;
  }
  if (H * W <= kFwdLdsMax) {
    switch (pick_lpt(H * W, kThreads)) {
      case 8: launch_fwd_lds<8>(aff, stats, in, out, xpos, ypos, in_scale, in_shift, ps, B, C, H, W, Ho, stride, ah, st); break;
      case 16: launch_fwd_lds<16>(aff, stats, in, out, xpos, ypos, in_scale, in_shift, ps, B, C, H, W, Ho, stride, ah, st); break;
      default: launch_fwd_lds<32>(aff, stats, in, out, xpos, ypos, in_scale, in_shift, ps, B, C, H, W, Ho, stride, ah, st); break;
    }
    SGCN_LAUNCH_CHECK();
    return 0;
  }
  if (H * W <= kFwdLdsMax2) {
    launch_fwd_lds<32, 512>(aff, stats, in, out, xpos, ypos, in_scale, in_shift, ps, B, C, H, W, Ho, stride, ah, st);
    SGCN_LAUNCH_CHECK();
    return 0;
  }
  switch (pick_ept(Ho * W)) {
    case 8: launch_fwd<8>(aff, stats, in, out, xpos, ypos, in_scale, in_shift, ps, B, C, H, W, Ho, stride, ah, st); break;
    case 16: launch_fwd<16>(aff, stats, in, out, xpos, ypos, in_scale, in_shift, ps, B, C, H, W, Ho, stride, ah, st); break;
    default: launch_fwd<32>(aff, stats, in, out, xpos, ypos, in_scale, in_shift, ps, B, C, H, W, Ho, stride, ah, st); break;
  }
  SGCN_LAUNCH_CHECK();
  return 0;
}

int sgcn_tshift_fwd_pre(const float* z, float* out, const float* xpos, const float* ypos,
                        const float* pre_scale, const float* pre_shift, const float* r,
                        const float* r_scale, const float* r_shift, const float* in_scale,
                        const float* in_shift, int B, int C, int H, int W, int stride,
                        int ypos_is_raw, void* stream) {
  SGCN_REQUIRE(B >= 0 && C > 0 && H >= 0 && W > 0 && W <= 1024 && stride >= 1);
  SGCN_REQUIRE((r_scale == nullptr) == (r_shift == nullptr));
  SGCN_REQUIRE(H * W <= kFwdLdsMax2);
  const int Ho = H / stride;
  if (B == 0 || Ho == 0) return 0;
  SGCN_REQUIRE(z && out && xpos && ypos && pre_scale && pre_shift && r && in_scale &&
               in_shift && out != z);
  SGCN_REQUIRE((long long)B * C < (1LL << 31));
  hipStream_t st = (hipStream_t)stream;
  const int ah = (ypos_is_raw && stride != 1) ? 1 : 0;
  {
    const int nt = H * W <= kFwdLdsMax ? kThreads : 512;
    const int lpt = pad_fwd_lpt(H, W, nt);
// ... 33 lines not shown
    }
  } else {
    SGCN_PRE_R(512, 32);
  }
#undef SGCN_PRE_R
#undef SGCN_PRE
  SGCN_LAUNCH_CHECK();
  return 0;
}

int sgcn_tshift_fwd_tail(const float* in, float* out, const float* xpos, const float* ypos,
                         const float* post_scale, const float* post_shift, const float* r,
                         const float* r_scale, const float* r_shift, const float* gather_m,
                         float* out_gathered, int B, int C, int H, int W, int stride,
                         int ypos_is_raw, void* stream) {
  SGCN_REQUIRE(B >= 0 && C > 0 && H >= 0 && W > 0 && W <= 1024 && stride >= 1);
  SGCN_REQUIRE((r_scale == nullptr) == (r_shift == nullptr) && (r || !r_scale));
  SGCN_REQUIRE((gather_m == nullptr) == (out_gathered == nullptr));
  SGCN_REQUIRE(H * W <= kFwdLdsMax2);
  const int Ho = H / stride;
  if (B == 0 || Ho == 0) return 0;
  SGCN_REQUIRE(in && out && xpos && ypos && post_scale && post_shift && out != in);
  SGCN_REQUIRE((long long)B * C < (1LL << 31));
  hipStream_t st = (hipStream_t)stream;
  const int ah = (ypos_is_raw && stride != 1) ? 1 : 0;
  const int res = r == nullptr ? 0 : (r_scale ? 2 : 1);
  const bool go = out_gathered != nullptr;
  {
    const int nt = H * W <= kFwdLdsMax ? kThreads : 512;
    const int lpt = pad_fwd_lpt(H, W, nt);
    if (lpt) {
      const size_t plds = (size_t)(ra_pad_floats(H, W) + 1) * sizeof(float);
#define SGCN_TAILP(NT, L, R, G)                                                                \
  tshift_fwd_pad_kernel<NT, L, 2, false, false, R, G><<<B * C, NT, plds, st>>>(                \
      in, out, xpos, ypos, post_scale, post_shift, nullptr, C, H, W, Ho, stride, ah, nullptr,  \
      nullptr, r, r_scale, r_shift, gather_m, out_gathered)
#define SGCN_TAILP_RG(NT, L)                                                                   \
  do {                                                                                         \
    if (res == 0) { if (go) SGCN_TAILP(NT, L, 0, true); else SGCN_TAILP(NT, L, 0, false); }    \
    else if (res == 1) { if (go) SGCN_TAILP(NT, L, 1, true); else SGCN_TAILP(NT, L, 1, false); } \
    else { if (go) SGCN_TAILP(NT, L, 2, true); else SGCN_TAILP(NT, L, 2, false); }             \
  } while (0)
      if (nt == kThreads) {
        if (lpt == 8) SGCN_TAILP_RG(kThreads, 8); else if (lpt == 16) SGCN_TAILP_RG(kThreads, 16); else if (lpt == 24) SGCN_TAILP_RG(kThreads, 24); else SGCN_TAILP_RG(kThreads, 32);
      } else {
        if (lpt == 8) SGCN_TAILP_RG(512, 8); else if (lpt == 12) SGCN_TAILP_RG(512, 12); else if (lpt == 16) SGCN_TAILP_RG(512, 16);
        else if (lpt == 20) SGCN_TAILP_RG(512, 20); else if (lpt == 24) SGCN_TAILP_RG(512, 24); else SGCN_TAILP_RG(512, 32);
      }
#undef SGCN_TAILP_RG
#undef SGCN_TAILP
      SGCN_LAUNCH_CHECK();
      return 0;
    }
  }
  const size_t lds = (size_t)H * W * sizeof(float);
#define SGCN_TAIL(NT, L, R, G)                                                                \
  tshift_fwd_tail_kernel<NT, L, R, G><<<B * C, NT, lds, st>>>(                                \
      in, out, xpos, ypos, post_scale, post_shift, r, r_scale, r_shift, gather_m,            \
      out_gathered, C, H, W, Ho, stride, ah)
#define SGCN_TAIL_RG(NT, L)                                                                   \
  do {                                                                                        \
    if (res == 0) { if (go) SGCN_TAIL(NT, L, 0, true); else SGCN_TAIL(NT, L, 0, false); }     \
    else if (res == 1) { if (go) SGCN_TAIL(NT, L, 1, true); else SGCN_TAIL(NT, L, 1, false); } \
    else { if (go) SGCN_TAIL(NT, L, 2, true); else SGCN_TAIL(NT, L, 2, false); }              \
  } while (0)
  if (H * W <= kFwdLdsMax) {
    switch (pick_lpt(H * W, kThreads)) {
      case 8: SGCN_TAIL_RG(kThreads, 8); break;
      case 16: SGCN_TAIL_RG(kThreads, 16); break;
      default: SGCN_TAIL_RG(kThreads, 32); break;
    }
  } else {
    SGCN_TAIL_RG(512, 32);
  }
#undef SGCN_TAIL_RG
#undef SGCN_TAIL
  SGCN_LAUNCH_CHECK();
  return 0;
}

int sgcn_tshift_bwd_bnin(const float* dy, const float* y, const float* s, const float* coef,
                         const float* in, const float* xpos, const float* ypos, float* gin,
                         float* gx, float* gy, void* ws, size_t ws_bytes, int B, int C, int H,
                         int W, int ypos_is_raw, void* stream) {
  SGCN_REQUIRE(B > 0 && C > 0 && H > 0 && W > 0);
  SGCN_REQUIRE(H * W <= kBwdLdsMax);
  SGCN_REQUIRE(dy && y && s && coef && in && xpos && ypos && gin && ws);
  SGCN_REQUIRE((gx == nullptr) == (gy == nullptr));
  SGCN_REQUIRE(ws_bytes >= sgcn_tshift_bwd_ws_bytes(B, C));
  SGCN_REQUIRE((long long)B * C < (1LL << 31));
  (void)ypos_is_raw;
  hipStream_t st = (hipStream_t)stream;
  float2* pg = (float2*)ws;
  const int ntb = H * W <= 4096 ? 256 : 512;
  const bool ok = launch_ra<false, true, false, true, false>(
      ntb, nullptr, in, xpos, ypos, nullptr, nullptr, nullptr, nullptr, gin, pg, nullptr, B, C,
      H, W, dy, y, s, coef, nullptr, nullptr, nullptr, nullptr, st);
  SGCN_REQUIRE(ok);
  SGCN_LAUNCH_CHECK();
  if (gx) tshift_pos_finalize_kernel<<<(C + 3) / 4, 256, 0, st>>>(pg, B, C, gx, gy);
  SGCN_LAUNCH_CHECK();
  return 0;
}

size_t sgcn_tshift_bwd_ws_bytes(int B, int C) { return (size_t)B * C * sizeof(float2); }

int sgcn_tshift_pos_finalize_many(const void* const* partials, float* const* gx,
                                  float* const* gy, const int* B, const int* C, int n,
                                  void* stream) {
  SGCN_REQUIRE(n >= 0 && n <= SGCN_BATCH_MAX);
  if (n == 0) return 0;
  SGCN_REQUIRE(partials && gx && gy && B && C);
  PosBatch t{};
  int max_c = 0;
  for (int i = 0; i < n; ++i) {
    SGCN_REQUIRE(partials[i] && gx[i] && gy[i] && B[i] > 0 && C[i] > 0);
    t.p[i] = (const float2*)partials[i];
    t.gx[i] = gx[i];
    t.gy[i] = gy[i];
    t.B[i] = B[i];
    t.C[i] = C[i];
    max_c = max(max_c, C[i]);
  }
  tshift_pos_finalize_many_kernel<<<dim3((max_c + 3) / 4, n), 256, 0, (hipStream_t)stream>>>(t);
  SGCN_LAUNCH_CHECK();
  return 0;
}

int sgcn_tshift_pos_finalize(const void* ws, int B, int C, float* gx, float* gy, void* stream) {
  SGCN_REQUIRE(B > 0 && C > 0 && ws && gx && gy);
  tshift_pos_finalize_kernel<<<(C + 3) / 4, 256, 0, (hipStream_t)stream>>>((const float2*)ws, B,
                                                                           C, gx, gy);
  SGCN_LAUNCH_CHECK();
  return 0;
}

int sgcn_tshift_bwd_gbn(const float* gout, const float* in, const float* xpos,
                        const float* ypos, const float* in_scale, const float* in_shift,
                        const float* bn_mean, const float* bn_invstd, float* bn_part,
                        const float* z, const float* z_mean, const float* z_invstd,
                        float* z_part, const float* d, const float* d_mean,
                        const float* d_invstd, float* d_part, float* gin, float* gx, float* gy,
                        void* ws, size_t ws_bytes, int B, int C, int H, int W, void* stream) {
  SGCN_REQUIRE(B > 0 && C > 0 && H > 0 && W > 0 && W <= 64);
  SGCN_REQUIRE((d == nullptr) == (d_part == nullptr) && (!d || (d_mean && d_invstd)));
  SGCN_REQUIRE(H * W <= kBwdLdsMax);
  SGCN_REQUIRE(gout && in && xpos && ypos && in_scale && in_shift && bn_mean && bn_invstd &&
               bn_part && z && z_mean && z_invstd && z_part && gin && ws);
  SGCN_REQUIRE((gx == nullptr) == (gy == nullptr));
  SGCN_REQUIRE(ws_bytes >= sgcn_tshift_bwd_ws_bytes(B, C));
  SGCN_REQUIRE((long long)B * C < (1LL << 31));
  hipStream_t st = (hipStream_t)stream;
  float2* pg = (float2*)ws;
  float2* bp = (float2*)bn_part;
  const int n = H * W;
  const int l256 = n <= kRaSplit256 ? ra_lpt(n, 256, W) : 0;
  const int ntg = l256 && !(SGCN_GBD_SPLIT && d && l256 > 24) ? 256 : kBwdThreads;
  const bool ok =
      d ? launch_ra<true, false, true, false, true, true>(
              ntg, gout, in, xpos, ypos, in_scale, in_shift, bn_mean, bn_invstd, gin, pg, bp, B,
              C, H, W, nullptr, nullptr, nullptr, nullptr, z, z_mean, z_invstd, z_part, st, d,
              d_mean, d_invstd, d_part)
        : launch_ra<true, false, true, false, true>(
              ntg, gout, in, xpos, ypos, in_scale, in_shift, bn_mean, bn_invstd, gin, pg, bp, B,
              C, H, W, nullptr, nullptr, nullptr, nullptr, z, z_mean, z_invstd, z_part, st);
  SGCN_REQUIRE(ok);
  SGCN_LAUNCH_CHECK();
  if (gx) tshift_pos_finalize_kernel<<<(C + 3) / 4, 256, 0, st>>>(pg, B, C, gx, gy);
  SGCN_LAUNCH_CHECK();
  return 0;
}

int sgcn_tshift_bwd(const float* gout, const float* in, const float* xpos, const float* ypos,
                    const float* in_scale, const float* in_shift, int relu_mask,
                    const float* bn_mean, const float* bn_invstd, float* bn_part, float* gin,
                    float* gx, float* gy, void* ws, size_t ws_bytes, int B, int C, int H,
                    int W, int stride, int ypos_is_raw, void* stream) {
  SGCN_REQUIRE(B > 0 && C > 0 && H >= 0 && W > 0 && (stride == 1 || stride == 2));
  SGCN_REQUIRE((in_scale == nullptr) == (in_shift == nullptr));
  const int Ho = H / stride;
// ... 60 lines not shown
```

### shift-gcn_amd/shiftgcn/_lib.py

```python
from __future__ import annotations

import ctypes
import os

import torch

LIB_NAME = "libshiftgcn_hip.so"
LIB_PATH = os.path.join(os.path.dirname(os.path.abspath(__file__)), LIB_NAME)
LIB_PATH = os.environ.get("SGCN_LIB_PATH", LIB_PATH)
ABI_VERSION = 23
BATCH_MAX = 32
ABI_DIAG_FLAG = 0x10000
EINVAL = -22

_lib = None

_P = ctypes.c_void_p
_I = ctypes.c_int
_F = ctypes.c_float
_Z = ctypes.c_size_t
_L = ctypes.c_longlong

SIGNATURES = {
    "sgcn_abi_version": (_I, []),
    "sgcn_sgd_chunk_elems": (_I, []),
    "sgcn_sgd_step": (_I, [_P, _P, _P, _I, _F, _I, _P]),
    "sgcn_tshift_fwd": (_I, [_P, _P, _P, _P, _P, _P, _P, _I, _I, _I, _I, _I, _I, _P]),
    "sgcn_tshift_fwd_pre": (_I, [_P, _P, _P, _P, _P, _P, _P, _P, _P, _P, _P, _I, _I, _I, _I,
                                 _I, _I, _P]),
    "sgcn_tshift_fwd_tail": (_I, [_P, _P, _P, _P, _P, _P, _P, _P, _P, _P, _P, _I, _I, _I, _I,
                                  _I, _I, _P]),
    "sgcn_tshift_bwd_ws_bytes": (_Z, [_I, _I]),
    "sgcn_tshift_pos_finalize": (_I, [_P, _I, _I, _P, _P, _P]),
    "sgcn_tshift_bwd": (_I, [_P, _P, _P, _P, _P, _P, _I, _P, _P, _P, _P, _P, _P, _P, _Z, _I,
                             _I, _I, _I, _I, _I, _P]),
    "sgcn_tshift_fwd_f64": (_I, [_P, _P, _P, _P, _I, _I, _I, _I, _I, _I, _P]),
    "sgcn_tshift_bwd_f64_ws_bytes": (_Z, [_I, _I]),
    "sgcn_tshift_bwd_f64": (_I, [_P, _P, _P, _P, _P, _P, _P, _P, _Z, _I, _I, _I, _I, _I, _I,
                                 _P]),
    "sgcn_pw_fwd": (_I, [_P, _I, _P, _P, _L, _L, _I, _I, _P, _P, _L, _L, _I, _I, _I, _I, _I,
                         _I, _I, _I, _I, _P]),
    "sgcn_pw_tshift_ws_bytes": (_Z, [_I]),
    "sgcn_pw_fwd_tshift": (_I, [_P, _P, _P, _L, _L, _P, _P, _P, _P, _P, _P, _Z, _P, _L, _L, _I,
                                _I, _I, _I, _I, _I, _I, _P]),
    "sgcn_pw_dw_ws_bytes": (_Z, [_I, _I, _I, _I, _I]),
    "sgcn_pw_dw": (_I, [_P, _L, _L, _I, _I, _P, _L, _L, _I, _I, _P, _P, _I, _I, _P, _I, _P, _Z,
                        _I, _I, _I, _I, _I, _P]),
    "sgcn_moments_ws_bytes": (_Z, [_I, _I, _I, _I]),
    "sgcn_moments": (_I, [_P, _P, _I, _I, _I, _I, _I, _P]),
    "sgcn_bn_finalize": (_I, [_P, _I, _I, _I, _I, _P, _P, _F, _F, _P, _P, _P, _P, _P, _P, _P,
                              _P]),
    "sgcn_bn_eval_coef": (_I, [_I, _I, _P, _P, _P, _P, _F, _P, _P, _P, _P, _P]),
    "sgcn_bn_apply": (_I, [_P, _P, _P, _I, _P, _P, _P, _I, _P, _P, _P, _P, _I, _I, _I, _I,
                           _P]),
    "sgcn_bn_bwd_reduce": (_I, [_P, _P, _I, _P, _P, _P, _I, _P, _P, _P, _P, _P, _P, _I, _I, _I,
                                _I, _P]),
    "sgcn_bn_bwd_finalize": (_I, [_P, _I, _I, _L, _I, _P, _P, _P, _P, _P, _I, _I, _P, _P]),
    "sgcn_bn_bwd_apply": (_I, [_P, _P, _I, _P, _P, _I, _P, _P, _P, _P, _P, _I, _I, _I, _I,
                               _P]),
    "sgcn_mask_prep": (_I, [_P, _P, _I, _P]),
    "sgcn_gcn_gather": (_I, [_P, _P, _P, _I, _I, _I, _I, _P]),
    "sgcn_gcn_dx_finish": (_I, [_P, _P, _P, _P, _P, _P, _P, _P, _P, _P, _P, _P, _I, _I, _I, _I,
                                _P]),
    "sgcn_tshift_bwd_bnin": (_I, [_P, _P, _P, _P, _P, _P, _P, _P, _P, _P, _P, _Z, _I, _I, _I,
                                  _I, _I, _P]),
    "sgcn_mask_grad_finalize": (_I, [_P, _P, _I, _I, _I, _P, _I, _P]),
    "sgcn_modalities": (_I, [_P, _P, _P, _P, _P, _P, _P, _P, _I, _I, _I, _I, _I, _I, _P]),
    "sgcn_tshift_bwd_gbn": (_I, [_P, _P, _P, _P, _P, _P, _P, _P, _P, _P, _P, _P, _P, _P, _P, _P,
                                 _P, _P, _P, _P, _P, _Z, _I, _I, _I, _I, _P]),
    "sgcn_bn_bwd_finalize_gbn": (_I, [_P, _I, _I, _I, _L, _P, _P, _P, _P, _P, _P, _P, _I, _I,
                                      _P, _P]),
    "sgcn_head_ws_bytes": (_Z, [_I, _I, _I, _I]),
    "sgcn_head_moments": (_I, [_P, _P, _I, _I, _I, _I, _I, _P]),
    "sgcn_head_apply": (_I, [_P, _P, _P, _P, _I, _I, _I, _I, _I, _P]),
    "sgcn_head_bwd_reduce": (_I, [_P, _P, _P, _P, _P, _I, _I, _I, _I, _I, _P]),
    "sgcn_head_bwd_apply": (_I, [_P, _P, _P, _P, _I, _I, _I, _I, _I, _P]),
    "sgcn_pool": (_I, [_P, _P, _I, _I, _I, _L, _P]),
    "sgcn_pool_bwd": (_I, [_P, _P, _I, _I, _I, _L, _P]),
    "sgcn_tshift_pos_finalize_many": (_I, [_P, _P, _P, _P, _P, _I, _P]),
    "sgcn_mask_prep_many": (_I, [_P, _P, _P, _I, _P]),
    "sgcn_mask_grad_finalize_many": (_I, [_P, _P, _P, _P, _P, _P, _I, _P]),
}


class NativeLibraryError(RuntimeError):
    pass


def _open(path):
    lib = ctypes.CDLL(path, mode=ctypes.RTLD_LOCAL)
    lib.sgcn_abi_version.restype = _I
    lib.sgcn_abi_version.argtypes = []
    abi = lib.sgcn_abi_version()
    if abi & ABI_DIAG_FLAG:
        if os.environ.get("SGCN_ALLOW_DIAG_LIB") != "1" or os.path.basename(path) == LIB_NAME:
            raise NativeLibraryError(
                f"{path} is a DIAGNOSTIC build (SGCN_PW_DIAG / SGCN_PW_STAMPS / SGCN_DIAG_*: "
                "its results are wrong); rebuild with `make -C shift-gcn_amd/csrc`")
        abi &= ~ABI_DIAG_FLAG
    if abi != ABI_VERSION:
        raise NativeLibraryError(f"{path}: ABI version {abi} != {ABI_VERSION}; rebuild it")
    for name, (res, args) in SIGNATURES.items():
        fn = getattr(lib, name)
        fn.restype = res
        fn.argtypes = args
    return lib


def load():
    global _lib
    if _lib is not None:
        return _lib
    if not os.path.exists(LIB_PATH):
        raise NativeLibraryError(
            f"{LIB_PATH} not found: build it with `python -c 'import __graft_entry__ as g; "
            f"g.build()'` (or `make -C shift-gcn_amd/csrc`). There is no CPU fallback.")
    _lib = _open(LIB_PATH)
    return _lib


def check(rc: int, name: str) -> None:
    if rc == 0:
        return
    if rc == EINVAL:
        raise ValueError(f"{name}: invalid argument (shape/pointer/stride)")
    raise RuntimeError(f"{name}: HIP error {rc}")
```

### shift-gcn_amd/shiftgcn/fused.py

```python
from __future__ import annotations

import os
import threading

import torch

from . import ops
from .ops import PlaneView as PV


def _empty(*shape, like):
    return torch.empty(shape, device=like.device, dtype=torch.float32)


_SIDE = {}


def _side_stream(device):
    s = _SIDE.get(device)
    if s is None:
        s = _SIDE[device] = torch.cuda.Stream(device=device)
    return s


# ... 114 lines not shown
def _pos_grads(gx, gy, shift):
    if not isinstance(gx, ops.PosPartials):
        return gx, gy
    ox, oy = ops.grad_like(shift.xpos), ops.grad_like(shift.ypos)
    if BATCH_SIDE:
        _task(gx.ws.device).pos.append((gx, ox, oy))
    else:
        with _OffPath(True, gx.ws):
            gx.finalize(ox, oy)
    return _Later(ox), _Later(oy)


def _pos_alloc(shift, off):
    return None if off else (ops.grad_like(shift.xpos), ops.grad_like(shift.ypos))


TAIL_MAIN = int(os.environ.get("SGCN_TAIL_MAIN", "3"))


class GcnSaved:
    __slots__ = ("x0", "xg", "Z", "zst", "D0", "dst", "H", "m", "h_moments")


def gcn_forward(mod, x0, training, off=False):
    B, Cin, T, V = x0.shape
    Cout = mod.out_channels
    D0 = dst = None
    if mod.has_down:
        conv, bn = mod.down[0], mod.down[1]
        D0 = _empty(B, Cout, T, V, like=x0)
        down = _OffPath(off, x0)
        with down:
            ops.pw_fwd(conv.weight, False, conv.bias, PV(x0), PV(D0), Cout, Cin, T, V)
            if training:
                dst = ops.bn_finalize(ops.moments(D0, False), B, Cout, T * V, bn)
            else:
                dst = ops.bn_eval_coef(bn, Cout)
    cache = mod.__dict__.pop("_gather_cache", None)
    if cache is not None and cache[0] is x0:
        xg, m = cache[1], cache[2]
    else:
        m = _mask_of(mod)
        xg = ops.gcn_gather(x0, m)
    Z = _empty(B, Cout, T, V, like=x0)
    ops.pw_fwd(mod.Linear_weight, True, mod.Linear_bias, PV(xg), PV(Z), Cout, Cin, T, V)
    if training:
        zst = ops.bn_finalize(ops.moments(Z, 3), B, Cout * V, T, mod.bn, perm_V=V)
    else:
        zst = ops.bn_eval_coef(mod.bn, Cout * V, perm_V=V)
    if mod.has_down:
        down.wait()
        H, hm = ops.bn_apply(Z, zst, 3, r=D0, rst=dst, relu=True, out_stats=training)
    else:
        H, hm = ops.bn_apply(Z, zst, 3, r=x0, relu=True, out_stats=training)
    s = GcnSaved()
    s.x0, s.xg, s.Z, s.zst, s.D0, s.dst, s.H, s.m = x0, xg, Z, zst, D0, dst, H, m
    s.h_moments = hm
    return H, s


def _mask_of(gcn):
    fm = gcn.Feature_Mask
    r = gcn.__dict__.get("_mask_ready")
    if r is not None and r[0] is fm and r[1] == fm._version:
        return r[2]
    if gcn.training:
        return ops.mask_prep(fm)
    return ops.cached(gcn, "_sgcn_mask", ops._src_key((fm,)), lambda: ops.mask_prep(fm),
                      fm.device)


def prepare_masks(gcns):
    fms = [g.Feature_Mask for g in gcns]
    if any(g.training for g in gcns):
        ms = ops.mask_prep_many(fms)
    else:
        ms = ops.cached(gcns[0], "_sgcn_masks", ops._src_key(fms) + tuple(map(id, gcns)),
                        lambda: ops.mask_prep_many(fms), fms[0].device)
    for g, m in zip(gcns, ms):
        g.__dict__["_mask_ready"] = (g.Feature_Mask, g.Feature_Mask._version, m)


def gcn_backward(mod, s: GcnSaved, dH, extra_dx=None, dy_coef=None, prev=None, extra_out=None,
                 pre6=None, off=False):
    x0 = s.x0
    B, Cin, T, V = x0.shape
    Cout = mod.out_channels
    g = {}
    rpart = None
    if pre6 is not None:
        assert dy_coef is not None and (pre6[2] is not None) == mod.has_down
        coefZ, g["bn.weight"], g["bn.bias"] = ops.bn_bwd_finalize_gbn(
            pre6[0], B, Cout, V, B * T, dy_coef, pre6[1], s.zst, mod.bn)
    else:
        if mod.has_down:
            conv, bnd = mod.down[0], mod.down[1]
            part, rpart = ops.bn_bwd_reduce(dH, s.H, True, s.Z, s.zst, 3, r=s.D0,
                                            rst=s.dst, dy_coef=dy_coef)
        else:
            part, rpart = ops.bn_bwd_reduce(dH, s.H, True, s.Z, s.zst, 3, dy_coef=dy_coef)
        coefZ, g["bn.weight"], g["bn.bias"] = ops.bn_bwd_finalize(part, B, Cout * V, B * T,
                                                                   s.zst, mod.bn, perm_V=V)
    dZ = _empty(B, Cout, T, V, like=x0)
    g_id = dD0 = None
    if mod.has_down:
        conv, bnd = mod.down[0], mod.down[1]
        if pre6 is not None:
            coefD, g["down.1.weight"], g["down.1.bias"] = ops.bn_bwd_finalize_gbn(
                pre6[2], B, Cout, 1, B * T * V, dy_coef, pre6[1], s.dst, bnd)
        else:
            coefD, g["down.1.weight"], g["down.1.bias"] = ops.bn_bwd_finalize(
                rpart, B, Cout, B * T * V, s.dst, bnd)
        dD0 = _empty(B, Cout, T, V, like=x0)
        ops.bn_bwd_apply(dH, s.H, True, s.Z, coefZ, 3, r=s.D0, rcoef=coefD, dr=dD0, dx=dZ,
                         dy_coef=dy_coef)
    else:
        g_id = _empty(B, Cin, T, V, like=x0)
        ops.bn_bwd_apply(dH, s.H, True, s.Z, coefZ, 3, dr=g_id, dx=dZ, dy_coef=dy_coef)
    dLW = ops.grad_like(mod.Linear_weight)
    dLb = ops.grad_like(mod.Linear_bias)
    dXt = _empty(B, Cin, T, V, like=x0)
    ops.pw_fwd(mod.Linear_weight, False, None, PV(dZ), PV(dXt), Cin, Cout, T, V)
    with _OffPath(off, dZ, s.xg):
        ops.pw_dw(PV(dZ), PV(s.xg), dLW, Cout, Cin, T, V, transpose=True, dbias=dLb)
    g["Linear_weight"], g["Linear_bias"] = _late(dLW, off), _late(dLb, off)
    a2, a2m = extra_dx if isinstance(extra_dx, tuple) else (extra_dx, None)
    if prev is not None:
        dx, mpart, extra_out["prev_part"] = ops.gcn_dx_finish(dXt, x0, s.m, add1=g_id,
                                                              add2=a2, prev=prev,
                                                              add2_mask=a2m)
    else:
        dx, mpart = ops.gcn_dx_finish(dXt, x0, s.m, add1=g_id, add2=a2, add2_mask=a2m)
    dmask = ops.grad_like(mod.Feature_Mask)
    fm = mod.Feature_Mask
    if BATCH_SIDE and (off or _defer_ok((fm,))):
        _task(mpart.device).mask.append((mpart, fm, B, Cin, V, dmask))
        g["Feature_Mask"] = _Later(dmask)
    else:
        with _OffPath(off, mpart):
            ops.mask_grad_finalize(mpart, fm, B, Cin, V, out=dmask)
        g["Feature_Mask"] = _late(dmask, off)
    if mod.has_down:
        dWd = ops.grad_like(conv.weight)
        dbd = ops.grad_like(conv.bias)
        ops.pw_fwd(conv.weight, True, None, PV(dD0), PV(dx), Cin, Cout, T, V, accumulate=True)
        with _OffPath(off, dD0, x0):
            ops.pw_dw(PV(dD0), PV(x0), dWd, Cout, Cin, T, V, dbias=dbd)
        g["down.0.weight"], g["down.0.bias"] = _late(dWd, off), _late(dbd, off)
    return dx, g


class TcnSaved:
    __slots__ = ("H", "ast", "As", "R", "S", "sst")


def tshift_fused(C):
    return C >= TSHIFT_FUSION_MIN_C


def folded_conv_bn(conv, bn):
    srcs = (conv.weight, conv.bias, bn.weight, bn.bias, bn.running_mean, bn.running_var)
    key = ops._src_key(srcs) + (float(bn.eps),)

    def make():
        st = ops.bn_eval_coef(bn, conv.out_channels)
        with torch.no_grad():
            w = (conv.weight.detach() *
                 st.scale.view(-1, *([1] * (conv.weight.dim() - 1)))).contiguous()
            b = (conv.bias.detach() * st.scale + st.shift if conv.bias is not None
                 else st.shift.clone())
        return w, b
    return ops.cached(conv, "_sgcn_fold", key, make, conv.weight.device)


def convbn_infer_folded(mod, x):
    B, Cin, T, V = x.shape
    conv = mod.conv
    Cout = conv.out_channels
    To = (T - 1) // mod.stride + 1
    w, b = folded_conv_bn(conv, mod.bn)
    R = _empty(B, Cout, To, V, like=x)
    ops.pw_fwd(w, False, b, PV(x, mod.stride), PV(R), Cout, Cin, To, V)
    return R


def gcn_infer_z(mod, x0):
    B, Cin, T, V = x0.shape
    Cout = mod.out_channels
    cache = mod.__dict__.pop("_gather_cache", None)
    if cache is not None and cache[0] is x0:
        xg = cache[1]
    else:
        xg = ops.gcn_gather(x0, _mask_of(mod))
    Z = _empty(B, Cout, T, V, like=x0)
    ops.pw_fwd(mod.Linear_weight, True, mod.Linear_bias, PV(xg), PV(Z, 1, +1), Cout, Cin, T, V)
    zst = ops.bn_eval_coef(mod.bn, Cout * V, perm_V=V)
    if mod.has_down:
        conv, bn = mod.down[0], mod.down[1]
        D0 = _empty(B, Cout, T, V, like=x0)
        if EVAL_FOLD:
            w, b = folded_conv_bn(conv, bn)
            ops.pw_fwd(w, False, b, PV(x0), PV(D0), Cout, Cin, T, V)
            return Z, zst, D0, None
        ops.pw_fwd(conv.weight, False, conv.bias, PV(x0), PV(D0), Cout, Cin, T, V)
        return Z, zst, D0, ops.bn_eval_coef(bn, Cout)
    return Z, zst, x0, None


def tcn_core_forward(mod, H, training, h_moments=None, tail=None, pre=None):
    src = H if H is not None else pre[0]
    B, C, T, V = src.shape
    Cout = mod.out_channels
    si, so = mod.shift_in, mod.shift_out
    stride = so.stride
    if training:
# ... 32 lines not shown
    return S, sst, s


def tcn_core_backward(mod, s: TcnSaved, dS, materialize_dx=True, gpre=None, gcn_z=None,
                      out=None, off=False):
    H = s.H
    B, C, T, V = H.shape
    Cout = mod.out_channels
    si, so = mod.shift_in, mod.shift_out
    g = {}
    if gpre is not None:
        dRp, gx, gy = ops.tshift_bwd_bnin(gpre[0], gpre[1], s.S, gpre[2], s.R,
                                          so.xpos.detach(), so.ypos.detach(), defer_pos=off,
                                          pos_out=_pos_alloc(so, off))
    else:
        dRp, gx, gy = ops.tshift_bwd(dS, s.R, so.xpos.detach(), so.ypos.detach(), so.stride,
                                     relu_mask=True, defer_pos=off,
                                     pos_out=_pos_alloc(so, off))
    g["shift_out.xpos"], g["shift_out.ypos"] = _pos_grads(gx, gy, so)
    tl = mod.temporal_linear
    dWt = ops.grad_like(tl.weight)
    dbt = ops.grad_like(tl.bias)

    dAs = _empty(B, C, T, V, like=H)
    ops.pw_fwd(tl.weight, True, None, PV(dRp), PV(dAs), C, Cout, T, V)
    with _OffPath(off, dRp, s.As):
        ops.pw_dw(PV(dRp), PV(s.As), dWt, Cout, C, T, V, dbias=dbt)
    g["temporal_linear.weight"], g["temporal_linear.bias"] = _late(dWt, off), _late(dbt, off)
    if gcn_z is not None and GBN_FUSION and si.stride == 1 and ops.ra_fits(T * V, V):
        down = gcn_z[2] if len(gcn_z) > 2 else None
        res = ops.tshift_bwd_gbn(dAs, H, si.xpos.detach(), si.ypos.detach(), s.ast, gcn_z[0],
                                 gcn_z[1], defer_pos=off, down=down,
                                 pos_out=_pos_alloc(si, off))
        dA, gx, gy, part, zpart = res[:5]
        out["pre6"] = (zpart, s.ast, res[5] if down is not None else None)
    else:
        dA, gx, gy, part = ops.tshift_bwd(
            dAs, H, si.xpos.detach(), si.ypos.detach(), si.stride, scale=s.ast.scale,
            shift=s.ast.shift, bn_stats=s.ast, defer_pos=off, pos_out=_pos_alloc(si, off))
    g["shift_in.xpos"], g["shift_in.ypos"] = _pos_grads(gx, gy, si)
    coef, g["bn.weight"], g["bn.bias"] = ops.bn_bwd_finalize(part, B, C, B * T * V, s.ast,
                                                             mod.bn)
    if not materialize_dx:
        return (dA, coef), g
    dH = ops.bn_bwd_apply(dA, None, False, H, coef, False)
    return dH, g


class ConvBnSaved:
    __slots__ = ("x", "Rc", "rst", "To")


def convbn_core_forward(mod, x, training):
    B, Cin, T, V = x.shape
    conv, bn = mod.conv, mod.bn
    Cout = conv.out_channels
    s_t = mod.stride
    To = (T - 1) // s_t + 1
    Rc = _empty(B, Cout, To, V, like=x)
    ops.pw_fwd(conv.weight, False, conv.bias, PV(x, s_t), PV(Rc), Cout, Cin, To, V)
    if training:
        rst = ops.bn_finalize(ops.moments(Rc, False), B, Cout, To * V, bn)
    else:
        rst = ops.bn_eval_coef(bn, Cout)
    s = ConvBnSaved()
    s.x, s.Rc, s.rst, s.To = x, Rc, rst, To
    return Rc, rst, s


def convbn_dx_and_dw(mod, s: ConvBnSaved, dRc, dx, accumulate, off=False):
    B, Cin, T, V = s.x.shape
    conv = mod.conv
    Cout = conv.out_channels
    dW = ops.grad_like(conv.weight)
    db = ops.grad_like(conv.bias)
    ops.pw_fwd(conv.weight, True, None, PV(dRc), PV(dx, mod.stride), Cin, Cout, s.To, V,
               accumulate=accumulate)
    with _OffPath(off, dRc, s.x):
        ops.pw_dw(PV(dRc), PV(s.x, mod.stride), dW, Cout, Cin, s.To, V, dbias=db)
    return {"conv.weight": _late(dW, off), "conv.bias": _late(db, off)}


class UnitSaved:
    __slots__ = ("x", "gs", "ts", "rs", "out", "prev", "off")


def unit_forward(unit, x, training):
    consumer = unit.__dict__.get("_gather_consumer")
    if (not training and _INFER.active and
            x.shape[2] * x.shape[3] <= ops.TAIL_MAX_PLANE):
        pre = gcn_infer_z(unit.gcn1, x)
        r = rst = None
        if unit.residual_kind == "conv":
            if EVAL_FOLD:
                r = convbn_infer_folded(unit.residual, x)
            else:
                r, rst, _ = convbn_core_forward(unit.residual, x, training)
        elif unit.residual_kind == "identity":
            r = x
        gm = _mask_of(consumer) if consumer is not None else None
        out, xg_next = tcn_core_forward(unit.tcn1, None, training, tail=(r, rst, gm),
                                        pre=pre)
        if gm is not None:
            consumer.__dict__["_gather_cache"] = (out, xg_next, gm)
        return out, None
    prev = unit.__dict__.pop("_prev_tail", None)
    prev = prev[1:] if prev is not None and prev[0] is x else None
    off = (ASYNC_DW and bool(unit.__dict__.get("_off_path")) and
           not torch.cuda.is_current_stream_capturing())
    mp = None
    if consumer is not None:
        if "_mask_ready" in consumer.__dict__:
            gm = _mask_of(consumer)
        else:
            mp = _OffPath(off, consumer.Feature_Mask)
            with mp:
                gm = ops.mask_prep(consumer.Feature_Mask)
    H, gs = gcn_forward(unit.gcn1, x, training, off=off)
    rs = None
    if unit.residual_kind == "conv":
        res = _OffPath(off, x)
        with res:
            Rc, rst, rs = convbn_core_forward(unit.residual, x, training)
    S, sst, ts = tcn_core_forward(unit.tcn1, H, training, h_moments=gs.h_moments)
    if mp is not None:
        mp.wait()
    elif consumer is None:
        gm = None
    if unit.residual_kind == "conv":
        res.wait()
        out = ops.bn_apply(S, sst, False, r=Rc, rst=rst, relu=True, gather_m=gm)
    elif unit.residual_kind == "identity":
        out = ops.bn_apply(S, sst, False, r=x, relu=True, gather_m=gm)
    else:
        out = ops.bn_apply(S, sst, False, relu=True, gather_m=gm)
    if gm is not None:
        out, xg_next = out
        consumer.__dict__["_gather_cache"] = (out, xg_next, gm)
    nxt = unit.__dict__.get("_next_unit")
    if (nxt is not None and unit.residual_kind != "conv" and nxt.residual_kind != "conv"
            and not nxt.gcn1.has_down):
        nxt.__dict__["_prev_tail"] = (out, (S, sst), unit)
    s = UnitSaved()
    s.x, s.gs, s.ts, s.rs, s.out, s.prev = x, gs, ts, rs, out, prev
    s.off = off
    return out, s


def _gcn_z(unit, s: UnitSaved):
    if unit.gcn1.has_down:
        return (s.gs.Z, s.gs.zst, (s.gs.D0, s.gs.dst)) if GBN_FUSION >= 2 else None
    return (s.gs.Z, s.gs.zst)


def _off_path_ok(unit, s: UnitSaved):
    if not s.off or torch.cuda.is_current_stream_capturing():
        return False
    if not _defer_ok([p for p in unit.parameters() if p.requires_grad]):
        return False
    _task(s.x.device).side = True
    return True


def unit_backward(unit, s: UnitSaved, dout):
    return _unit_backward(unit, s, dout, _off_path_ok(unit, s))


def _unit_backward(unit, s: UnitSaved, dout, off):
    ts = s.ts
    S = ts.S
    so = unit.tcn1.shift_out
    B, Cout, To, V = S.shape
    kind = unit.residual_kind
    g = {}
    cached = unit.__dict__.pop("_bwd_part", None)
    if cached is not None and cached[0] is dout and kind != "conv":
        part, rpart = cached[1], None
    elif kind == "conv":
        part, rpart = ops.bn_bwd_reduce(dout, s.out, True, S, ts.sst, False, r=s.rs.Rc,
                                        rst=s.rs.rst)
    else:
        part, rpart = ops.bn_bwd_reduce(dout, s.out, True, S, ts.sst, False)
    coef2, g["tcn1.bn2.weight"], g["tcn1.bn2.bias"] = ops.bn_bwd_finalize(
        part, B, Cout, B * To * V, ts.sst, unit.tcn1.bn2)
    if kind != "conv" and so.stride == 1 and ops.ra_fits(To * V, V):
        fo = {}
        (dA, coefA), gt = tcn_core_backward(unit.tcn1, ts, None, materialize_dx=False,
                                            gpre=(dout, s.out, coef2), gcn_z=_gcn_z(unit, s),
                                            out=fo, off=off)
        g.update({"tcn1." + k: v for k, v in gt.items()})
        extra = {}
        dx, gg = gcn_backward(unit.gcn1, s.gs, dA,
                              extra_dx=(dout, s.out) if kind == "identity" else None,
                              dy_coef=coefA, prev=None if s.prev is None else s.prev[0],
                              extra_out=extra, pre6=fo.get("pre6"), off=off)
        if s.prev is not None:
            s.prev[1].__dict__["_bwd_part"] = (dx, extra["prev_part"])
        g.update({"gcn1." + k: v for k, v in gg.items()})
        return dx, g
    dS = torch.empty_like(S)
    dres = None
    if kind == "conv":
        coefR, g["residual.bn.weight"], g["residual.bn.bias"] = ops.bn_bwd_finalize(
            rpart, B, Cout, B * To * V, s.rs.rst, unit.residual.bn)
        dres = torch.empty_like(s.rs.Rc)
        ops.bn_bwd_apply(dout, s.out, True, S, coef2, False, r=s.rs.Rc, rcoef=coefR, dr=dres,
                         dx=dS)
    elif kind == "identity":
        dres = torch.empty_like(s.x)
        ops.bn_bwd_apply(dout, s.out, True, S, coef2, False, dr=dres, dx=dS)
    else:
        ops.bn_bwd_apply(dout, s.out, True, S, coef2, False, dx=dS)
    fo = {}
    (dA, coefA), gt = tcn_core_backward(unit.tcn1, ts, dS, materialize_dx=False,
                                        gcn_z=_gcn_z(unit, s), out=fo, off=off)
    g.update({"tcn1." + k: v for k, v in gt.items()})
    extra = {}
    dx, gg = gcn_backward(unit.gcn1, s.gs, dA, extra_dx=dres if kind == "identity" else None,
                          dy_coef=coefA, prev=None if s.prev is None else s.prev[0],
                          extra_out=extra, pre6=fo.get("pre6"), off=off)
    if s.prev is not None:
        s.prev[1].__dict__["_bwd_part"] = (dx, extra["prev_part"])
    g.update({"gcn1." + k: v for k, v in gg.items()})
    if kind == "conv":
        gr = convbn_dx_and_dw(unit.residual, s.rs, dres, dx, accumulate=True, off=off)
        g.update({"residual." + k: v for k, v in gr.items()})
    return dx, g


TSHIFT_FUSION_MIN_C = int(os.environ.get("SGCN_TSHIFT_FUSION_MIN_C", "512"))
TSHIFT_TWO_ROW = int(os.environ.get("SGCN_TSHIFT_TWO_ROW", "2"))
EVAL_FOLD = int(os.environ.get("SGCN_EVAL_FOLD", "1"))
GBN_FUSION = int(os.environ.get("SGCN_GBN_FUSION", "2"))
ASYNC_DW = int(os.environ.get("SGCN_ASYNC_DW", "1"))


def trainable(module):
    return [(n, p) for n, p in module.named_parameters() if p.requires_grad]


class _BlockFunction(torch.autograd.Function):

    @staticmethod
    def forward(ctx, impl, module, x, *params):
        fwd, bwd = impl
        training = module.training
        y, saved = fwd(module, x.contiguous(), training)
        ctx.impl, ctx.module, ctx.saved, ctx.training = impl, module, saved, training
        tr = trainable(module)
        ctx.names, ctx.params = [n for n, _ in tr], [p for _, p in tr]
        ctx.save_for_backward(x, y)
        return y

    @staticmethod
    def backward(ctx, dy):
        ctx.saved_tensors
        if ctx.saved is None:
            raise RuntimeError(
                f"{type(ctx.module).__name__}: backward through the fused HIP block was "
                "called a second time; its saved activations are released after the first "
                "backward (retain_graph=True / double backward is not supported)")
        _, bwd = ctx.impl
        dx, grads = bwd(ctx.module, ctx.saved, dy.contiguous())
        ctx.saved = None
        out = []
        for n, p in zip(ctx.names, ctx.params):
            g = grads.get(n)
            if isinstance(g, _Later):
                _task(g.t.device).grads.append((p, g.t))
                g = None
            out.append(g)
        return (None, None, dx) + tuple(out)


class _InferFlag(threading.local):
    active = False


_INFER = _InferFlag()


def run_block(impl, module, x):
    params = [p for _, p in trainable(module)]
    prev = _INFER.active
    _INFER.active = not (torch.is_grad_enabled() and
                         (x.requires_grad or any(p.requires_grad for p in params)))
    try:
        return _BlockFunction.apply(impl, module, x, *params)
    finally:
        _INFER.active = prev


def _gcn_standalone_bwd(mod, s, dy):
    return gcn_backward(mod, s, dy)


def _tcn_standalone_fwd(mod, H, training):
    S, sst, ts = tcn_core_forward(mod, H, training)
    y = ops.bn_apply(S, sst, False)
    return y, ts


def _tcn_standalone_bwd(mod, ts, dy):
    S = ts.S
    B, C, To, V = S.shape
    part, _ = ops.bn_bwd_reduce(dy, None, False, S, ts.sst, False)
    coef, dg, db = ops.bn_bwd_finalize(part, B, C, B * To * V, ts.sst, mod.bn2)
    dS = ops.bn_bwd_apply(dy, None, False, S, coef, False)
    dH, g = tcn_core_backward(mod, ts, dS)
    g["bn2.weight"], g["bn2.bias"] = dg, db
    return dH, g


def _convbn_standalone_fwd(mod, x, training):
    Rc, rst, s = convbn_core_forward(mod, x, training)
    return ops.bn_apply(Rc, rst, False), s


def _convbn_standalone_bwd(mod, s, dy):
    B, C, To, V = s.Rc.shape
    part, _ = ops.bn_bwd_reduce(dy, None, False, s.Rc, s.rst, False)
    coef, dg, db = ops.bn_bwd_finalize(part, B, C, B * To * V, s.rst, mod.bn)
    dRc = ops.bn_bwd_apply(dy, None, False, s.Rc, coef, False)
    dx = torch.zeros_like(s.x)
    g = convbn_dx_and_dw(mod, s, dRc, dx, accumulate=True)
    g["bn.weight"], g["bn.bias"] = dg, db
    return dx, g


GCN_IMPL = (gcn_forward, _gcn_standalone_bwd)
TCN_IMPL = (_tcn_standalone_fwd, _tcn_standalone_bwd)
CONVBN_IMPL = (_convbn_standalone_fwd, _convbn_standalone_bwd)
UNIT_IMPL = (unit_forward, unit_backward)
```

### shift-gcn_amd/shiftgcn/head.py

```python
from __future__ import annotations

import torch

from . import ops


def _batch_stats(bn) -> bool:
    return bn.training or (bn.running_mean is None and bn.running_var is None)


class _DataBnFunction(torch.autograd.Function):
    @staticmethod
    def forward(ctx, x, weight, bias, bn):
        N, C, T, V, M = x.shape
        F = M * V * C
        if _batch_stats(bn):
            if N * T <= 1:
                raise ValueError("Expected more than 1 value per channel when training, got "
                                 f"input size {torch.Size([N, F, T])}")
            st = ops.bn_finalize(ops.head_moments(x), N, F, T, bn, training=bn.training)
        else:
            st = ops.bn_eval_coef(bn, F)
        ctx.save_for_backward(x)
        ctx.st, ctx.bn = st, bn
        return ops.head_apply(x, st)

    @staticmethod
    def backward(ctx, gy):
        (x,) = ctx.saved_tensors
        st, bn = ctx.st, ctx.bn
        N, C, T, V, M = x.shape
        gy = gy.contiguous()
        part = ops.head_bwd_reduce(gy, x, st)
        coef, dgamma, dbeta = ops.bn_bwd_finalize(part, N, M * V * C, N * T, st, bn)
        dx = ops.head_bwd_apply(gy, x, coef) if ctx.needs_input_grad[0] else None
        return (dx, dgamma if ctx.needs_input_grad[1] else None,
                dbeta if ctx.needs_input_grad[2] else None, None)


class _PoolFunction(torch.autograd.Function):
    @staticmethod
    def forward(ctx, x, N, M):
        ctx.shape, ctx.N, ctx.M = x.shape, N, M
        return ops.pool(x, N, M)

    @staticmethod
    def backward(ctx, g):
        return ops.pool_bwd(g.contiguous(), ctx.shape, ctx.N, ctx.M), None, None


class _LinearSlotsFunction(torch.autograd.Function):

    @staticmethod
    def forward(ctx, x, weight, bias):
        ctx.save_for_backward(x, weight)
        ctx.params = (weight, bias)
        return torch.nn.functional.linear(x, weight, bias)

    @staticmethod
    def backward(ctx, g):
        x, w = ctx.saved_tensors
        weight, bias = ctx.params
        dx = g.mm(w) if ctx.needs_input_grad[0] else None
        dw = db = None
        if ctx.needs_input_grad[1]:
            dw = ops.grad_like(weight)
            torch.mm(g.t(), x, out=dw)
        if bias is not None and ctx.needs_input_grad[2]:
            db = ops.grad_like(bias)
            torch.sum(g, 0, out=db)
        return dx, dw, db


def linear(fc, x):
    if ops.grad_slot(fc.weight) is None or x.dim() != 2:
        return fc(x)
    return _LinearSlotsFunction.apply(x, fc.weight, fc.bias)


def data_bn_planes(bn, x):
    ops.check_input(x, "input")
    if x.dim() != 5:
        raise RuntimeError(f"expected a (N, C, T, V, M) clip, got shape {tuple(x.shape)}")
    N, C, T, V, M = x.shape
    if bn.num_features != M * V * C:
        raise RuntimeError(f"data_bn has {bn.num_features} features, the clip {M * V * C}")
    return _DataBnFunction.apply(x, bn.weight, bn.bias, bn)


def pool(x, N, M):
    ops.check_input(x, "input")
    if x.shape[0] != N * M:
        raise RuntimeError(f"expected {N * M} planes, got {x.shape[0]}")
    return _PoolFunction.apply(x, N, M)
```

### shift-gcn_amd/shiftgcn/ops.py

```python
from __future__ import annotations

import ctypes

import torch

from . import _lib

_F32 = torch.float32


def _ptr(t):
    if t is None:
        return None
    return t.data_ptr()


class LaunchTimer:

    def __init__(self, ops_filter=None, detail=False):
        self.ops_filter = ops_filter
        self.detail = detail
        self.records = []

    def begin(self, op, flops, nbytes, device):
# ... 304 lines not shown
        if (scale is not None or shift is not None or relu_mask or bn_stats is not None):
            raise RuntimeError("the fused shift options are float32-only")
        return _tshift_bwd_f64(gout, inp, xpos, ypos, stride, ypos_is_raw)
    check_input(gout, "grad_output")
    check_input(inp, "input")
    check_input(xpos, "xpos")
    check_input(ypos, "ypos")
    _opt(scale, "scale"), _opt(shift, "shift")
    B, C, H, W = inp.shape
    lib = _lib.load()
    dev = inp.device
    gin = torch.empty_like(inp)
    nbytes = lib.sgcn_tshift_bwd_ws_bytes(B, C)
    ws = torch.empty((max(nbytes, 4) + 3) // 4, device=dev, dtype=_F32)
    gx, gy, pp = _pos_out(defer_pos, ws, B, C, dev, pos_out)
    bpart = torch.empty((B * C * 2,), device=dev, dtype=_F32) if bn_stats is not None else None
    nb = 4 * (gout.numel() + 2 * inp.numel())
    with _timed("tshift_bwd", 0, nb, inp, _shp(inp)):
        rc = lib.sgcn_tshift_bwd(_ptr(gout), _ptr(inp), _ptr(xpos), _ptr(ypos), _ptr(scale),
                                 _ptr(shift), int(bool(relu_mask)),
                                 _ptr(bn_stats.mean) if bn_stats is not None else None,
                                 _ptr(bn_stats.invstd) if bn_stats is not None else None,
                                 _ptr(bpart), _ptr(gin), _ptr(gx), _ptr(gy), _ptr(ws), nbytes,
                                 B, C, H, W, stride, int(ypos_is_raw), _stream(inp))
    _lib.check(rc, "sgcn_tshift_bwd")
    if pp is not None:
        gx = pp
    if bn_stats is not None:
        return gin, gx, gy, bpart
    return gin, gx, gy


GBN_MAX_PLANE = 16384


def ra_fits(n, V):
    if V > 64 or n > GBN_MAX_PLANE:
        return False
    if (n // V + 2 * 4) * (V + 2) + 1 > 16384:
        return False
    nt = 256 if n <= 4096 else 512
    return -(-n // ((nt // V) * V)) <= 32


def tshift_bwd_gbn(gout, inp, xpos, ypos, st: "BnStats", z, zst: "BnStats", defer_pos=False,
                   down=None, pos_out=None):
    check_input(gout, "grad_output")
    check_input(inp, "input")
    check_input(z, "z")
    if down is not None:
        check_input(down[0], "d")
    B, C, H, W = inp.shape
    lib = _lib.load()
    dev = inp.device
    gin = torch.empty_like(inp)
    nbytes = lib.sgcn_tshift_bwd_ws_bytes(B, C)
    ws = torch.empty((max(nbytes, 4) + 3) // 4, device=dev, dtype=_F32)
    gx, gy, pp = _pos_out(defer_pos, ws, B, C, dev, pos_out)
    bpart = torch.empty((B * C * 2,), device=dev, dtype=_F32)
    zpart = torch.empty((6 * B * C * W,), device=dev, dtype=_F32)
    d, dst, dpart = None, None, None
    if down is not None:
        d, dst = down
        dpart = torch.empty((6 * B * C,), device=dev, dtype=_F32)
    nb = 4 * (gout.numel() + (3 if down is None else 4) * inp.numel())
    with _timed("tshift_bwd", 0, nb, inp, ("GBND " if down is not None else "GBN ") + _shp(inp)):
        rc = lib.sgcn_tshift_bwd_gbn(_ptr(gout), _ptr(inp), _ptr(xpos), _ptr(ypos),
                                     _ptr(st.scale), _ptr(st.shift), _ptr(st.mean),
                                     _ptr(st.invstd), _ptr(bpart), _ptr(z), _ptr(zst.mean),
                                     _ptr(zst.invstd), _ptr(zpart), _ptr(d),
                                     _ptr(dst.mean if dst is not None else None),
                                     _ptr(dst.invstd if dst is not None else None),
                                     _ptr(dpart), _ptr(gin), _ptr(gx), _ptr(gy), _ptr(ws),
                                     nbytes, B, C, H, W, _stream(inp))
    _lib.check(rc, "sgcn_tshift_bwd_gbn")
    if down is not None:
        return gin, (pp if pp is not None else gx), gy, bpart, zpart, dpart
    return gin, (pp if pp is not None else gx), gy, bpart, zpart


BNIN_MAX_PLANE = 16384


def tshift_bwd_bnin(dy, y, s, coef, inp, xpos, ypos, defer_pos=False, pos_out=None):
    for t, n in ((dy, "dy"), (y, "y"), (s, "s"), (inp, "input"), (coef, "coef")):
        check_input(t, n)
    B, C, H, W = inp.shape
    lib = _lib.load()
    dev = inp.device
    gin = torch.empty_like(inp)
    nbytes = lib.sgcn_tshift_bwd_ws_bytes(B, C)
    ws = torch.empty((max(nbytes, 4) + 3) // 4, device=dev, dtype=_F32)
    gx, gy, pp = _pos_out(defer_pos, ws, B, C, dev, pos_out)
    nb = 4 * (3 * dy.numel() + 2 * inp.numel())
    with _timed("tshift_bwd", 0, nb, inp, _shp(inp)):
        rc = lib.sgcn_tshift_bwd_bnin(
            _ptr(dy), _ptr(y), _ptr(s), _ptr(coef), _ptr(inp), _ptr(xpos), _ptr(ypos),
            _ptr(gin), _ptr(gx), _ptr(gy), _ptr(ws), nbytes, B, C, H, W, 1, _stream(inp))
    _lib.check(rc, "sgcn_tshift_bwd_bnin")
    return gin, (pp if pp is not None else gx), gy


class PlaneView:

    __slots__ = ("t", "bstride", "cstride", "tstride", "rsign")

    def __init__(self, t, tstride=1, rsign=0):
        check_input(t, "plane operand")
        self.t = t
        self.bstride = t.stride(0)
        self.cstride = t.stride(1)
        self.tstride = tstride
        self.rsign = rsign


PW_MAX_ELEMS = 1 << 29


def _plane_extent(v: PlaneView, B, C, T, V):
    return (B - 1) * v.bstride + C * v.cstride + T * v.tstride * V


def _batch_chunk(views, B, T, V):
    bc = B
    for v, C in views:
        per = v.bstride
        fixed = C * v.cstride + T * v.tstride * V
        if fixed >= PW_MAX_ELEMS:
            raise ValueError("pointwise operand plane too large for one sample")
        if (B - 1) * per + fixed >= PW_MAX_ELEMS:
            bc = min(bc, max(1, (PW_MAX_ELEMS - 1 - fixed) // max(per, 1) + 1))
    return bc


def pw_fwd(w, w_mcontig, bias, x: PlaneView, out: PlaneView, M, K, T, V, mask=None,
           relu=False, accumulate=False):
    check_input(w, "weight")
    _opt(bias, "bias"), _opt(mask, "mask")
    B = x.t.shape[0]
    lib = _lib.load()
    P = B * T * V
    bc = _batch_chunk([(x, K), (out, M)], B, T, V)
    det = (f"M{M} K{K} T{T} V{V} xrot{x.rsign} yrot{out.rsign} mask{int(mask is not None)} "
           f"ts{x.tstride}{out.tstride} acc{int(accumulate)} mc{int(w_mcontig)}")
    with _timed("pw_fwd", 2.0 * P * M * K, 4.0 * P * (M * (2 if accumulate else 1) + K), x.t,
                det):
        for b0 in range(0, B, bc):
            nb = min(bc, B - b0)
            rc = lib.sgcn_pw_fwd(_ptr(w), int(w_mcontig), _ptr(bias),
                                 x.t.data_ptr() + 4 * b0 * x.bstride, x.bstride,
                                 x.cstride, x.tstride, x.rsign, _ptr(mask),
                                 out.t.data_ptr() + 4 * b0 * out.bstride,
                                 out.bstride, out.cstride, out.tstride, out.rsign, int(relu),
                                 int(accumulate), nb, M, K, T, V, _stream(x.t))
            _lib.check(rc, "sgcn_pw_fwd")
    return out.t


def pw_dw(g: PlaneView, x: PlaneView, dw, M, Nc, T, V, mask=None, transpose=False,
          accumulate=False, dbias=None, dbias_accumulate=False):
    check_input(dw, "dw")
    _opt(dbias, "dbias"), _opt(mask, "mask")
    B = g.t.shape[0]
    lib = _lib.load()
    bc = _batch_chunk([(g, M), (x, Nc)], B, T, V)
    nbytes = lib.sgcn_pw_dw_ws_bytes(bc, M, Nc, T, V)
    ws = torch.empty((nbytes + 3) // 4, device=g.t.device, dtype=_F32)
    P = B * T * V
    det = (f"M{M} N{Nc} T{T} V{V} grot{g.rsign} xrot{x.rsign} mask{int(mask is not None)} "
           f"ts{g.tstride}{x.tstride}")
    with _timed("pw_dw", 2.0 * P * M * Nc, 4.0 * P * (M + Nc), g.t, det):
        for b0 in range(0, B, bc):
            nb = min(bc, B - b0)
            first = b0 == 0
            rc = lib.sgcn_pw_dw(g.t.data_ptr() + 4 * b0 * g.bstride, g.bstride, g.cstride,
                                g.tstride, g.rsign, x.t.data_ptr() + 4 * b0 * x.bstride,
                                x.bstride, x.cstride, x.tstride, x.rsign, _ptr(mask),
                                _ptr(dw), int(transpose), int(accumulate or not first),
                                _ptr(dbias), int(dbias_accumulate or not first), _ptr(ws),
                                nbytes, nb, M, Nc, T, V, _stream(g.t))
            _lib.check(rc, "sgcn_pw_dw")
# ... 43 lines not shown
                                      _stream(x))
    _lib.check(rc, "sgcn_moments")
    return part


class BnStats:

    __slots__ = ("mean", "invstd", "scale", "shift", "buf", "batch")

    def __init__(self, F, device, batch=True):
        buf = torch.empty((4, F), device=device, dtype=_F32)
        self.buf = buf
        self.mean, self.invstd, self.scale, self.shift = buf[0], buf[1], buf[2], buf[3]
        self.batch = batch


def bn_finalize(part, B, F, n_part, bn, perm_V=0, training=True):
    st = BnStats(F, part.device)
    lib = _lib.load()
    track = training and bn.track_running_stats and bn.running_mean is not None
    if track and bn.momentum is None:
        raise NotImplementedError("BatchNorm momentum=None is not supported on the HIP path")
    momentum = bn.momentum if bn.momentum is not None else 0.0
    with _timed("finalize", 0, 4 * part.numel(), part):
        rc = lib.sgcn_bn_finalize(
            _ptr(part), B, F, n_part, perm_V, _ptr(bn.weight), _ptr(bn.bias), float(bn.eps),
            float(momentum), _ptr(bn.running_mean) if track else None,
            _ptr(bn.running_var) if track else None,
            _ptr(bn.num_batches_tracked) if track else None, _ptr(st.mean),
            _ptr(st.invstd), _ptr(st.scale), _ptr(st.shift), _stream(part))
    _lib.check(rc, "sgcn_bn_finalize")
    if track:
        bump_versions((bn.running_mean, bn.running_var, bn.num_batches_tracked))
        if torch.cuda.is_current_stream_capturing():
            mark_captured_writes()
    return st


def bn_eval_coef(bn, F, perm_V=0, device=None):
    key = _src_key((bn.weight, bn.bias, bn.running_mean, bn.running_var)) + (
        float(bn.eps), F, perm_V)
    return cached(bn, "_sgcn_eval_coef", key, lambda: _bn_eval_coef(bn, F, perm_V),
                  bn.running_mean.device)


def _bn_eval_coef(bn, F, perm_V):
    st = BnStats(F, bn.running_mean.device, batch=False)
    with _timed("finalize", 0, 4 * 8 * F, bn.running_mean):
        rc = _lib.load().sgcn_bn_eval_coef(F, perm_V, _ptr(bn.weight), _ptr(bn.bias),
                                           _ptr(bn.running_mean), _ptr(bn.running_var),
                                           float(bn.eps), _ptr(st.mean), _ptr(st.invstd),
                                           _ptr(st.scale), _ptr(st.shift),
                                           _stream(bn.running_mean))
    _lib.check(rc, "sgcn_bn_eval_coef")
    return st


def bn_apply(x, st: BnStats, per_joint, r=None, rst: BnStats = None, relu=False, out=None,
             out_stats=None, gather_m=None):
    check_input(x, "input")
    if r is not None:
        check_input(r, "residual")
    B, C, T, V = x.shape
    y = torch.empty_like(x) if out is None else out
    ys = torch.empty((B * C * 2,), device=x.device, dtype=_F32) if out_stats else None
    yg = torch.empty_like(y) if gather_m is not None else None
    nb = 4 * x.numel() * (2 + (r is not None) + (yg is not None))
    with _timed("bn_apply", 0, nb, x, _shp(x)):
        rc = _lib.load().sgcn_bn_apply(
            _ptr(x), _ptr(st.scale), _ptr(st.shift), int(per_joint), _ptr(r),
            _ptr(rst.scale) if rst is not None else None,
            _ptr(rst.shift) if rst is not None else None, int(relu), _ptr(y), _ptr(ys),
            _ptr(gather_m), _ptr(yg), B, C, T, V, _stream(x))
    _lib.check(rc, "sgcn_bn_apply")
    if gather_m is not None:
        return y, yg
    return y if out_stats is None else (y, ys)


def bn_bwd_reduce(dy, y, relu, x, st: BnStats, per_joint, r=None, rst: BnStats = None,
                  dy_coef=None):
    check_input(dy, "grad_output")
    B, C, T, V = x.shape
    dev = x.device
    part = torch.empty((B * C * (V if per_joint else 1) * 2,), device=dev, dtype=_F32)
    rpart = torch.empty((B * C * 2,), device=dev, dtype=_F32) if r is not None else None
    nb = 4 * x.numel() * (2 + (y is not None) + (r is not None))
    with _timed("bn_bwd_reduce", 0, nb, x, _shp(x)):
        rc = _lib.load().sgcn_bn_bwd_reduce(_ptr(dy), _ptr(y), int(relu), _ptr(x),
                                            _ptr(st.mean), _ptr(st.invstd), int(per_joint),
                                            _ptr(r), _ptr(rst.mean) if rst else None,
                                            _ptr(rst.invstd) if rst else None, _ptr(dy_coef),
                                            _ptr(part), _ptr(rpart), B, C, T, V, _stream(x))
    _lib.check(rc, "sgcn_bn_bwd_reduce")
    return part, rpart


def bn_bwd_finalize(part, B, F, n_total, st: BnStats, bn, perm_V=0):
    dev = part.device
    coef = torch.empty((3, F), device=dev, dtype=_F32)
    dgamma = grad_like(bn.weight) if bn.weight is not None else None
    dbeta = grad_like(bn.bias) if bn.bias is not None else None
    with _timed("finalize", 0, 4 * part.numel(), part):
        rc = _lib.load().sgcn_bn_bwd_finalize(_ptr(part), B, F, int(n_total), perm_V,
                                              _ptr(st.mean), _ptr(st.invstd), _ptr(bn.weight),
                                              _ptr(dgamma), _ptr(dbeta), 0, int(st.batch),
                                              _ptr(coef), _stream(part))
    _lib.check(rc, "sgcn_bn_bwd_finalize")
    return coef, dgamma, dbeta


def bn_bwd_finalize_gbn(part6, B, C, V, n_total, dy_coef, dy_st: BnStats, st: BnStats, bn):
    dev = part6.device
    F = C * V
    coef = torch.empty((3, F), device=dev, dtype=_F32)
    dgamma = grad_like(bn.weight) if bn.weight is not None else None
    dbeta = grad_like(bn.bias) if bn.bias is not None else None
    with _timed("finalize", 0, 4 * part6.numel(), part6):
        rc = _lib.load().sgcn_bn_bwd_finalize_gbn(_ptr(part6), B, C, V, int(n_total),
                                                  _ptr(dy_coef), _ptr(dy_st.mean),
                                                  _ptr(st.mean), _ptr(st.invstd),
                                                  _ptr(bn.weight), _ptr(dgamma), _ptr(dbeta), 0,
                                                  int(st.batch), _ptr(coef), _stream(part6))
    _lib.check(rc, "sgcn_bn_bwd_finalize_gbn")
    return coef, dgamma, dbeta


def bn_bwd_apply(dy, y, relu, x, coef, per_joint, r=None, rcoef=None, dr=None, dx=None,
                 dy_coef=None):
    B, C, T, V = x.shape
    dx = torch.empty_like(x) if dx is None else dx
    nb = 4 * x.numel() * (3 + (y is not None) + (r is not None) + (dr is not None))
    with _timed("bn_bwd_apply", 0, nb, x, _shp(x)):
        rc = _lib.load().sgcn_bn_bwd_apply(
            _ptr(dy), _ptr(y), int(relu), _ptr(x), _ptr(coef), int(per_joint), _ptr(r),
            _ptr(rcoef), _ptr(dy_coef), _ptr(dx), _ptr(dr), B, C, T, V, _stream(x))
    _lib.check(rc, "sgcn_bn_bwd_apply")
    return dx


def mask_prep(mask):
    check_input(mask, "Feature_Mask")
    m = torch.empty_like(mask)
    with _timed("finalize", 0, 8 * mask.numel(), mask):
        rc = _lib.load().sgcn_mask_prep(_ptr(mask), _ptr(m), mask.numel(), _stream(mask))
    _lib.check(rc, "sgcn_mask_prep")
    return m


def _arr(ctype, vals):
    return (ctype * len(vals))(*vals)


def _chunks(xs):
    for i in range(0, len(xs), _lib.BATCH_MAX):
        yield xs[i:i + _lib.BATCH_MAX]


def mask_prep_many(masks):
    outs = []
    for ch in _chunks(list(masks)):
        for mk in ch:
            check_input(mk, "Feature_Mask")
        o = [torch.empty_like(mk) for mk in ch]
        with _timed("finalize", 0, 8 * sum(m.numel() for m in ch), ch[0]):
            rc = _lib.load().sgcn_mask_prep_many(
                _arr(ctypes.c_void_p, [m.data_ptr() for m in ch]),
                _arr(ctypes.c_void_p, [t.data_ptr() for t in o]),
                _arr(ctypes.c_int, [m.numel() for m in ch]), len(ch), _stream(ch[0]))
        _lib.check(rc, "sgcn_mask_prep_many")
        outs += o
    return outs


def pos_finalize_many(entries):
    for ch in _chunks(list(entries)):
        for _, gx, gy in ch:
            check_input(gx, "gx")
            check_input(gy, "gy")
        with _timed("finalize", 0, sum(pp.ws.numel() * 4 for pp, _, _ in ch), ch[0][1]):
            rc = _lib.load().sgcn_tshift_pos_finalize_many(
                _arr(ctypes.c_void_p, [pp.ws.data_ptr() for pp, _, _ in ch]),
                _arr(ctypes.c_void_p, [gx.data_ptr() for _, gx, _ in ch]),
                _arr(ctypes.c_void_p, [gy.data_ptr() for _, _, gy in ch]),
                _arr(ctypes.c_int, [pp.B for pp, _, _ in ch]),
                _arr(ctypes.c_int, [pp.C for pp, _, _ in ch]), len(ch), _stream(ch[0][1]))
        _lib.check(rc, "sgcn_tshift_pos_finalize_many")


def mask_grad_finalize_many(entries):
    for ch in _chunks(list(entries)):
        for e in ch:
            check_input(e[5], "dmask")
        with _timed("finalize", 0, sum(e[0].numel() * 4 for e in ch), ch[0][0]):
            rc = _lib.load().sgcn_mask_grad_finalize_many(
                _arr(ctypes.c_void_p, [e[0].data_ptr() for e in ch]),
                _arr(ctypes.c_void_p, [e[1].data_ptr() for e in ch]),
                _arr(ctypes.c_void_p, [e[5].data_ptr() for e in ch]),
                _arr(ctypes.c_int, [e[2] for e in ch]), _arr(ctypes.c_int, [e[3] for e in ch]),
                _arr(ctypes.c_int, [e[4] for e in ch]), len(ch), _stream(ch[0][0]))
        _lib.check(rc, "sgcn_mask_grad_finalize_many")


def gcn_gather(x0, m):
    B, C, T, V = x0.shape
    xg = torch.empty_like(x0)
    with _timed("gcn_gather", 0, 8 * x0.numel(), x0, _shp(x0)):
        rc = _lib.load().sgcn_gcn_gather(_ptr(x0), _ptr(m), _ptr(xg), B, C, T, V,
                                         _stream(x0))
    _lib.check(rc, "sgcn_gcn_gather")
    return xg


def gcn_dx_finish(dxt, x0, m, add1=None, add2=None, prev=None, add2_mask=None):
    B, C, T, V = dxt.shape
    dx = torch.empty_like(dxt)
    part = torch.empty((B * C * V,), device=dxt.device, dtype=_F32)
    pp = torch.empty((B * C * 2,), device=dxt.device, dtype=_F32) if prev is not None else None
    ps, pst = prev if prev is not None else (None, None)
    nb = 4 * dxt.numel() * (3 + sum(t is not None for t in (add1, add2, add2_mask, ps)))
    with _timed("gcn_dx_finish", 0, nb, dxt, _shp(dxt)):
        rc = _lib.load().sgcn_gcn_dx_finish(_ptr(dxt), _ptr(x0), _ptr(m), _ptr(add1),
                                            _ptr(add2), _ptr(add2_mask), _ptr(dx), _ptr(part),
                                            _ptr(ps), _ptr(pst.mean) if pst else None,
                                            _ptr(pst.invstd) if pst else None, _ptr(pp), B, C,
                                            T, V, _stream(dxt))
    _lib.check(rc, "sgcn_gcn_dx_finish")
    return (dx, part) if prev is None else (dx, part, pp)


def mask_grad_finalize(part, mask, B, C, V, out=None):
    dmask = torch.empty_like(mask) if out is None else out
    with _timed("finalize", 0, 4 * part.numel(), mask):
        rc = _lib.load().sgcn_mask_grad_finalize(_ptr(part), _ptr(mask), B, C, V, _ptr(dmask),
                                                 0, _stream(mask))
    _lib.check(rc, "sgcn_mask_grad_finalize")
    return dmask


def head_moments(x):
    check_input(x, "input")
    N, C, T, V, M = x.shape
    part = torch.empty((N * M * V * C * 2,), device=x.device, dtype=_F32)
    with _timed("head", 0, 4 * x.numel(), x):
        rc = _lib.load().sgcn_head_moments(_ptr(x), _ptr(part), N, C, T, V, M, _stream(x))
    _lib.check(rc, "sgcn_head_moments")
    return part


def head_apply(x, st: BnStats):
    N, C, T, V, M = x.shape
    y = torch.empty((N * M, C, T, V), device=x.device, dtype=_F32)
    with _timed("head", 0, 8 * x.numel(), x):
        rc = _lib.load().sgcn_head_apply(_ptr(x), _ptr(st.scale), _ptr(st.shift), _ptr(y), N, C,
                                         T, V, M, _stream(x))
    _lib.check(rc, "sgcn_head_apply")
    return y


def head_bwd_reduce(g, x, st: BnStats):
    check_input(g, "grad_output")
    N, C, T, V, M = x.shape
    part = torch.empty((N * M * V * C * 2,), device=x.device, dtype=_F32)
    with _timed("head", 0, 8 * x.numel(), x):
        rc = _lib.load().sgcn_head_bwd_reduce(_ptr(g), _ptr(x), _ptr(st.mean), _ptr(st.invstd),
                                              _ptr(part), N, C, T, V, M, _stream(x))
    _lib.check(rc, "sgcn_head_bwd_reduce")
    return part


def head_bwd_apply(g, x, coef):
    N, C, T, V, M = x.shape
    dx = torch.empty_like(x)
    with _timed("head", 0, 12 * x.numel(), x):
        rc = _lib.load().sgcn_head_bwd_apply(_ptr(g), _ptr(x), _ptr(coef), _ptr(dx), N, C, T, V,
                                             M, _stream(x))
    _lib.check(rc, "sgcn_head_bwd_apply")
    return dx


def pool(x, N, M):
    check_input(x, "input")
    C = x.shape[1]
    P = x.numel() // max(1, N * M * C)
    out = torch.empty((N, C), device=x.device, dtype=_F32)
    with _timed("pool", 0, 4 * x.numel(), x):
        rc = _lib.load().sgcn_pool(_ptr(x), _ptr(out), N, M, C, P, _stream(x))
    _lib.check(rc, "sgcn_pool")
    return out


def pool_bwd(dout, shape, N, M):
    check_input(dout, "grad_output")
    dx = torch.empty(shape, device=dout.device, dtype=_F32)
    C = shape[1]
    P = dx.numel() // max(1, N * M * C)
    with _timed("pool", 0, 4 * dx.numel(), dout):
        rc = _lib.load().sgcn_pool_bwd(_ptr(dout), _ptr(dx), N, M, C, P, _stream(dout))
    _lib.check(rc, "sgcn_pool_bwd")
    return dx
```

### shift-gcn_amd/shiftgcn/shift_gcn.py

```python
from __future__ import annotations

import contextlib
import importlib
import math

import numpy as np
import torch
import torch.nn as nn

from . import fused, head
from .shift import Shift


def import_class(name):
    components = name.split(".")
    mod = importlib.import_module(components[0])
    for comp in components[1:]:
        try:
            mod = getattr(mod, comp)
        except AttributeError:
            mod = importlib.import_module(mod.__name__ + "." + comp)
    return mod


# ... 94 lines not shown
        super().__init__()
        self.gcn1 = Shift_gcn(in_channels, out_channels, A, num_point=num_point)
        self.tcn1 = Shift_tcn(out_channels, out_channels, stride=stride)
        self.relu = nn.ReLU()
        if not residual:
            self.residual = lambda x: 0
            self.residual_kind = "none"
        elif in_channels == out_channels and stride == 1:
            self.residual = lambda x: x
            self.residual_kind = "identity"
        else:
            self.residual = tcn(in_channels, out_channels, kernel_size=1, stride=stride)
            self.residual_kind = "conv"

    def forward(self, x):
        return fused.run_block(fused.UNIT_IMPL, self, x)


class Model(nn.Module):

    def __init__(self, num_class=60, num_point=25, num_person=2, graph=None,
                 graph_args=dict(), in_channels=3):
        super().__init__()
        if graph is None:
            raise ValueError()
        if isinstance(graph, str):
            try:
                Graph = import_class(graph)
            except ImportError:
                if not graph.startswith("graph."):
                    raise
                Graph = import_class("shiftgcn." + graph)
        else:
            Graph = graph
        self.graph = Graph(**graph_args)
        A = self.graph.A
        self.num_person, self.in_channels = num_person, in_channels
        self.data_bn = nn.BatchNorm1d(num_person * in_channels * num_point)
        self.l1 = TCN_GCN_unit(3, 64, A, residual=False, num_point=num_point)
        self.l2 = TCN_GCN_unit(64, 64, A, num_point=num_point)
        self.l3 = TCN_GCN_unit(64, 64, A, num_point=num_point)
        self.l4 = TCN_GCN_unit(64, 64, A, num_point=num_point)
        self.l5 = TCN_GCN_unit(64, 128, A, stride=2, num_point=num_point)
        self.l6 = TCN_GCN_unit(128, 128, A, num_point=num_point)
        self.l7 = TCN_GCN_unit(128, 128, A, num_point=num_point)
        self.l8 = TCN_GCN_unit(128, 256, A, stride=2, num_point=num_point)
        self.l9 = TCN_GCN_unit(256, 256, A, num_point=num_point)
        self.l10 = TCN_GCN_unit(256, 256, A, num_point=num_point)
        self.fc = nn.Linear(256, num_class)
        nn.init.normal_(self.fc.weight, 0, math.sqrt(2.0 / num_class))
        bn_init(self.data_bn, 1)

    def forward(self, x):
        N, C, T, V, M = x.size()
        x = head.data_bn_planes(self.data_bn, x.contiguous())
        return self.forward_planes(x, N, M)

    def forward_planes(self, x, N, M):
        units = [getattr(self, f"l{k}") for k in range(1, 11)]
        with linked_units(units):
            for u in units:
                x = u(x)
        x = head.pool(x, N, M)
        return head.linear(self.fc, x)


@contextlib.contextmanager
def linked_units(units):
    try:
        for u, nxt in zip(units[:-1], units[1:]):
            u.__dict__["_gather_consumer"] = nxt.gcn1
            u.__dict__["_next_unit"] = nxt
        for i, u in enumerate(units):
            if i or not fused.TAIL_MAIN & 2:
                u.__dict__["_off_path"] = True
        fused.prepare_masks([u.gcn1 for u in units])
        yield
    finally:
        for u in units:
            u.__dict__.pop("_gather_consumer", None)
            u.__dict__.pop("_next_unit", None)
            u.__dict__.pop("_off_path", None)
            u.__dict__.pop("_prev_tail", None)
            u.gcn1.__dict__.pop("_gather_cache", None)
            u.gcn1.__dict__.pop("_mask_ready", None)
```

Before: 2010 clips/s.

## Propagate per-plane pooled gradient into last unit backward instead of materializing

Global-average-pool backward now emits one gradient value per (sample, channel) plane rather than a full broadcast tensor. The last unit's backward kernels (BN reduce, tshift bwd, gcn dx finish) read that scalar per plane through new flags. A mask_dx option also applies the next unit's ReLU mask to dx directly, so a later pass can skip it. Both aim to cut full-size gradient reads and writes, at the cost of more kernel variants and extra flag plumbing.

```diff
diff --git a/include/shiftgcn.h b/include/shiftgcn.h
--- a/include/shiftgcn.h
+++ b/include/shiftgcn.h
@@ -8,7 +8,7 @@
 #endif
 
 #define SGCN_EINVAL (-22)
-#define SGCN_ABI_VERSION 23
+#define SGCN_ABI_VERSION 24
 #define SGCN_ABI_DIAG_FLAG 0x10000
 
 int sgcn_abi_version(void);
@@ -33,7 +33,7 @@
 int sgcn_tshift_bwd_bnin(const float* dy, const float* y, const float* s, const float* coef,
                          const float* in, const float* xpos, const float* ypos, float* gin,
                          float* gx, float* gy, void* ws, size_t ws_bytes, int B, int C, int H,
-                         int W, int ypos_is_raw, void* stream);
+                         int W, int ypos_is_raw, int dy_plane, void* stream);
 size_t sgcn_tshift_bwd_ws_bytes(int B, int C);
 
 int sgcn_tshift_pos_finalize(const void* ws, int B, int C, float* gx, float* gy, void* stream);
@@ -106,7 +106,8 @@
 int sgcn_bn_bwd_reduce(const float* dy, const float* y, int relu, const float* x,
                        const float* mean, const float* invstd, int per_joint, const float* r,
                        const float* rmean, const float* rinvstd, const float* dy_coef,
-                       float* part, float* rpart, int B, int C, int T, int V, void* stream);
+                       float* part, float* rpart, int B, int C, int T, int V, int dy_plane,
+                       void* stream);
 
 int sgcn_bn_bwd_finalize(const float* part, int B, int F, long long n_total, int perm_V,
                          const float* mean, const float* invstd, const float* gamma,
@@ -129,10 +130,12 @@
 int sgcn_gcn_gather(const float* x0, const float* m, float* xg, int B, int C, int T, int V,
                     void* stream);
 
+#define SGCN_DXF_MASK_DX 1
+#define SGCN_DXF_ADD2_PLANE 2
 int sgcn_gcn_dx_finish(const float* dxt, const float* x0, const float* m, const float* add1,
                        const float* add2, const float* add2_mask, float* dx, float* dmask_part,
                        const float* prev_s, const float* prev_mean, const float* prev_invstd,
-                       float* prev_part, int B, int C, int T, int V, void* stream);
+                       float* prev_part, int B, int C, int T, int V, int flags, void* stream);
 
 int sgcn_mask_grad_finalize(const float* part, const float* mask, int B, int C, int V,
                             float* dmask, int accumulate, void* stream);
@@ -162,6 +165,9 @@
 int sgcn_pool_bwd(const float* dout, float* dx, int N, int M, int C, long long P,
                   void* stream);
 
+int sgcn_pool_bwd_planes(const float* dout, float* dplane, int N, int M, int C, long long P,
+                         void* stream);
+
 
 int sgcn_sgd_chunk_elems(void);
 
diff --git a/shift-gcn_amd/csrc/bn.hip b/shift-gcn_amd/csrc/bn.hip
--- a/shift-gcn_amd/csrc/bn.hip
+++ b/shift-gcn_amd/csrc/bn.hip
@@ -392,13 +392,15 @@
     const float* __restrict__ mean, const float* __restrict__ invstd,
     const float* __restrict__ r, const float* __restrict__ rmean,
     const float* __restrict__ rinvstd, const float* __restrict__ dyc, float2* __restrict__ part,
-    float2* __restrict__ rpart, int C, int T, int V) {
+    float2* __restrict__ rpart, int C, int T, int V, int dyp) {
   SGCN_CRIT_PRIO();
   __shared__ float s0[kThreads], s1[kThreads], red[2 * kThreads / 64];
   const int plane = blockIdx.x, c = plane % C;
   const int P = T * V;
   const size_t off = (size_t)plane * P;
   const int i = threadIdx.x;
+  const float* __restrict__ dyq = dyp ? dy + plane : dy + off;
+  const int dys = dyp ? 0 : 1;
   float rm = 0.f, ri = 0.f, d1 = 1.f, d2 = 0.f, d3 = 0.f;
   if (RESBN) { rm = rmean[c]; ri = rinvstd[c]; }
   if (DYT) { d1 = dyc[c]; d2 = dyc[C + c]; d3 = dyc[2 * C + c]; }
@@ -417,7 +419,7 @@
 #pragma unroll
         for (int u = 0; u < kU; ++u) {
           const int o = min(t0 + u * G, T - 1) * V + v;
-          gv[u] = dy[off + o];
+          gv[u] = dyq[o * dys];
           if (RELU) yv[u] = y[off + o];
           xv[u] = x[off + o + xd];
           if (RESBN) rv[u] = r[off + o];
@@ -451,7 +453,7 @@
 #pragma unroll
       for (int u = 0; u < kU; ++u) {
         const int o = min(base + u * kThreads + i, P - 1);
-        gv[u] = dy[off + o];
+        gv[u] = dyq[o * dys];
         if (RELU) yv[u] = y[off + o];
         xv[u] = x[off + o];
         if (RESBN) rv[u] = r[off + o];
@@ -482,7 +484,7 @@
     const float* __restrict__ mean, const float* __restrict__ invstd,
     const float* __restrict__ r, const float* __restrict__ rmean,
     const float* __restrict__ rinvstd, const float* __restrict__ dyc, float2* __restrict__ part,
-    float2* __restrict__ rpart, int C, int T, int V) {
+    float2* __restrict__ rpart, int C, int T, int V, int dyp) {
   SGCN_CRIT_PRIO();
   __shared__ float s0[NT], s1[NT], red[2 * NT / 64];
   const int plane = blockIdx.x, c = plane % C;
@@ -498,12 +500,18 @@
   const unsigned xo = vo + (unsigned)((PER_JOINT ? vx - w : 0) * 4);
   float gv[LPT], yv[RELU ? LPT : 1], xv[LPT], rv[RESBN ? LPT : 1];
   {
-    const auto dyr = make_rsrc(dy + off, pb), xr = make_rsrc(x + off, pb);
-#pragma unroll
-    for (int e = 0; e < LPT; ++e) {
-      gv[e] = bload(dyr, vo + e * vstep, 0);
-      xv[e] = bload(xr, xo + e * vstep, 0);
-    }
+    const auto xr = make_rsrc(x + off, pb);
+    if (dyp) {
+      const float pv = dy[plane];
+#pragma unroll
+      for (int e = 0; e < LPT; ++e) gv[e] = pv;
+    } else {
+      const auto dyr = make_rsrc(dy + off, pb);
+#pragma unroll
+      for (int e = 0; e < LPT; ++e) gv[e] = bload(dyr, vo + e * vstep, 0);
+    }
+#pragma unroll
+    for (int e = 0; e < LPT; ++e) xv[e] = bload(xr, xo + e * vstep, 0);
     if (RELU) {
       const auto yr = make_rsrc(y + off, pb);
 #pragma unroll
@@ -763,13 +771,14 @@
   }
 }
 
-template <int NT, int LPT, bool ADD1, bool ADD2, bool PART, bool A2M>
+template <int NT, int LPT, bool ADD1, bool ADD2, bool PART, int A2M>
 __global__ __launch_bounds__(NT) void gcn_dx_finish_ja_kernel(
     const float* __restrict__ dxt, const float* __restrict__ x0, const float* __restrict__ m,
     const float* __restrict__ add1, const float* __restrict__ add2, float* __restrict__ dx,
     float* __restrict__ dmask_part, const float* __restrict__ ps,
     const float* __restrict__ pmean, const float* __restrict__ pinvstd,
-    float2* __restrict__ bn_part, int C, int T, int V, const float* __restrict__ add2m) {
+    float2* __restrict__ bn_part, int C, int T, int V, const float* __restrict__ add2m,
+    int flags) {
   SGCN_CRIT_PRIO();
 #ifdef SGCN_DIAG_F1B_REAL
   return;
@@ -787,7 +796,9 @@
   const unsigned vo = own ? (unsigned)tid * 4u : 0x80000000u, vstep = (unsigned)NTJ * 4u;
   const unsigned pb = (unsigned)P * 4u;
   const unsigned uo = vo + (unsigned)((us - vd) * 4);
-  float gv[LPT], xq[LPT], a1[ADD1 ? LPT : 1], a2[ADD2 ? LPT : 1], a2q[A2M ? LPT : 1];
+  const bool mdx = flags & SGCN_DXF_MASK_DX;
+  constexpr bool A2P = A2M == 2;
+  float gv[LPT], xq[LPT], a1[ADD1 ? LPT : 1], a2[ADD2 && !A2P ? LPT : 1], a2q[A2M ? LPT : 1];
   float sv[PART ? LPT : 1];
   {
 #ifdef SGCN_DIAG_F1B_BOUND
@@ -805,7 +816,7 @@
 #pragma unroll
       for (int e = 0; e < LPT; ++e) a1[e] = bload(ar, vo + e * vstep, 0);
     }
-    if (ADD2) {
+    if (ADD2 && !A2P) {
       const auto ar = make_rsrc(add2 + off, pb);
 #pragma unroll
       for (int e = 0; e < LPT; ++e) a2[e] = bload(ar, vo + e * vstep, 0);
@@ -822,16 +833,17 @@
     }
   }
   const float mu = m[us * C + c];
-  float pm = 0.f, pi = 0.f;
+  float pm = 0.f, pi = 0.f, a2v = 0.f;
   if (PART) { pm = pmean[c]; pi = pinvstd[c]; }
+  if (A2P) a2v = add2[plane];
   const auto dxr = make_rsrc(dx + off, pb);
   float acc = 0.f, b0 = 0.f, b1 = 0.f;
 #pragma unroll
   for (int e = 0; e < LPT; ++e) {
     float val = gv[e] * mu;
     if (ADD1) val += a1[e];
-    if (ADD2) val += A2M ? (a2q[e] > 0.f ? a2[e] : 0.f) : a2[e];
-    bstore(dxr, val, vo + e * vstep, 0);
+    if (ADD2) val += A2M ? (a2q[e] > 0.f ? (A2P ? a2v : a2[e]) : 0.f) : a2[e];
+    bstore(dxr, (xq[e] > 0.f || !mdx) ? val : 0.f, vo + e * vstep, 0);
     acc = fmaf(gv[e], xq[e], acc);
     if (PART) {
       const float g = xq[e] > 0.f ? val : 0.f;
@@ -896,8 +908,10 @@
     const float* __restrict__ add1, const float* __restrict__ add2, float* __restrict__ dx,
     float* __restrict__ dmask_part, const float* __restrict__ ps,
     const float* __restrict__ pmean, const float* __restrict__ pinvstd,
-    float2* __restrict__ bn_part, int C, int T, int V, const float* __restrict__ add2m) {
+    float2* __restrict__ bn_part, int C, int T, int V, const float* __restrict__ add2m,
+    int flags) {
   SGCN_CRIT_PRIO();
+  const bool mdx = flags & SGCN_DXF_MASK_DX, a2p = flags & SGCN_DXF_ADD2_PLANE;
   __shared__ float s0[kThreads];
   const int plane = blockIdx.x, c = plane % C;
   const size_t off = (size_t)plane * T * V;
@@ -920,7 +934,7 @@
         gv[k] = dxt[off + row + us];
         xq[k] = x0[off + row + vd];
         if (ADD1) a1[k] = add1[off + row + vd];
-        if (ADD2) a2[k] = add2[off + row + vd];
+        if (ADD2) a2[k] = a2p ? add2[plane] : add2[off + row + vd];
         if (A2M) a2q[k] = add2m[off + row + vd];
         if (PART) sv[k] = ps[off + row + vd];
       }
@@ -930,7 +944,7 @@
         float val = gv[k] * mu;
         if (ADD1) val += a1[k];
         if (ADD2) val += A2M ? (a2q[k] > 0.f ? a2[k] : 0.f) : a2[k];
-        if (t < T) dx[off + t * V + vd] = val;
+        if (t < T) dx[off + t * V + vd] = (xq[k] > 0.f || !mdx) ? val : 0.f;
         acc += (t < T) ? gv[k] * xq[k] : 0.f;
         if (PART) {
           const float g = (t < T && xq[k] > 0.f) ? val : 0.f;
@@ -1202,9 +1216,10 @@
                        const float* mean, const float* invstd, int per_joint, const float* r,
                        const float* rmean,
                        const float* rinvstd, const float* dy_coef, float* part, float* rpart,
-                       int B, int C, int T, int V, void* stream) {
+                       int B, int C, int T, int V, int dy_plane, void* stream) {
   SGCN_PLANE_CHECK();
   SGCN_REQUIRE(B > 0 && T > 0 && dy && x && mean && invstd && part && (y || !relu));
+  const int dyp = dy_plane != 0;
   SGCN_REQUIRE(!dy_coef || (y && relu));
   SGCN_REQUIRE((r == nullptr) == (rpart == nullptr) && (!r || (rmean && rinvstd)));
   SGCN_REQUIRE(per_joint == 0 || per_joint == 3);
@@ -1219,10 +1234,10 @@
 #define SGCN_RJ(NT, L, PJ, RL, RB)                                                             \
   (dy_coef ? bn_bwd_reduce_ja_kernel<NT, L, PJ, RL, RB, true><<<g, NT, 0, st>>>(                \
                  dy, y, x, mean, invstd, r, rmean, rinvstd, dy_coef, (float2*)part,            \
-                 (float2*)rpart, C, T, V)                                                      \
+                 (float2*)rpart, C, T, V, dyp)                                                 \
            : bn_bwd_reduce_ja_kernel<NT, L, PJ, RL, RB, false><<<g, NT, 0, st>>>(               \
                  dy, y, x, mean, invstd, r, rmean, rinvstd, dy_coef, (float2*)part,            \
-                 (float2*)rpart, C, T, V))
+                 (float2*)rpart, C, T, V, dyp))
 #define SGCN_RJ_L(NT, PJ, RL, RB)                                                              \
   do {                                                                                         \
     if (lpt == 8) SGCN_RJ(NT, 8, PJ, RL, RB); else if (lpt == 16) SGCN_RJ(NT, 16, PJ, RL, RB); \
@@ -1244,10 +1259,10 @@
 #define SGCN_RED(PJ, RL, RB)                                                                \
   (dy_coef ? bn_bwd_reduce_kernel<PJ, RL, RB, true><<<g, kThreads, 0, st>>>(                   \
                  dy, y, x, mean, invstd, r, rmean, rinvstd, dy_coef, (float2*)part,           \
-                 (float2*)rpart, C, T, V)                                                     \
+                 (float2*)rpart, C, T, V, dyp)                                                \
            : bn_bwd_reduce_kernel<PJ, RL, RB, false><<<g, kThreads, 0, st>>>(                  \
                  dy, y, x, mean, invstd, r, rmean, rinvstd, dy_coef, (float2*)part,           \
-                 (float2*)rpart, C, T, V))
+                 (float2*)rpart, C, T, V, dyp))
   if (per_joint == 3) {
     if (rb) SGCN_RED(true, true, true); else SGCN_RED(true, true, false);
   } else {
@@ -1416,10 +1431,12 @@
                        const float* add2, const float* add2_mask, float* dx, float* dmask_part,
                        const float* prev_s, const float* prev_mean, const float* prev_invstd,
                        float* prev_part, int B,
-                       int C, int T, int V, void* stream) {
+                       int C, int T, int V, int flags, void* stream) {
   SGCN_PLANE_CHECK();
   if (B == 0 || T == 0) return 0;
   SGCN_REQUIRE(dxt && x0 && m && dx && dmask_part);
+  SGCN_REQUIRE((flags & ~(SGCN_DXF_MASK_DX | SGCN_DXF_ADD2_PLANE)) == 0);
+  SGCN_REQUIRE(!(flags & SGCN_DXF_ADD2_PLANE) || add2_mask);
   SGCN_REQUIRE(!prev_part || (prev_s && prev_mean && prev_invstd));
   SGCN_REQUIRE(!add2_mask || add2);
   hipStream_t st = (hipStream_t)stream;
@@ -1432,7 +1449,7 @@
 #define SGCN_FJ(NT, L, A1, A2, PT, AM)                                                         \
   gcn_dx_finish_ja_kernel<NT, L, A1, A2, PT, AM><<<B * C, NT, 0, st>>>(                        \
       dxt, x0, m, add1, add2, dx, dmask_part, prev_s, prev_mean, prev_invstd, pp, C, T, V,     \
-      add2_mask)
+      add2_mask, flags)
 #define SGCN_FJ_L(NT, A1, A2, PT, AM)                                                          \
   do {                                                                                         \
     if (lpt == 8) SGCN_FJ(NT, 8, A1, A2, PT, AM);                                              \
@@ -1444,9 +1461,9 @@
   do { if (nt == kThreads) SGCN_FJ_L(kThreads, A1, A2, PT, AM); else SGCN_FJ_L(512, A1, A2, PT, AM); } while (0)
 #define SGCN_FJ_P(A1, A2, AM)                                                                  \
   do { if (pp) SGCN_FJ_T(A1, A2, true, AM); else SGCN_FJ_T(A1, A2, false, AM); } while (0)
-      if (add2_mask) SGCN_FJ_P(true, true, true);
-      else if (add1) { if (add2) SGCN_FJ_P(true, true, false); else SGCN_FJ_P(true, false, false); }
-      else { if (add2) SGCN_FJ_P(false, true, false); else SGCN_FJ_P(false, false, false); }
+      if (add2_mask) { if (flags & SGCN_DXF_ADD2_PLANE) SGCN_FJ_P(true, true, 2); else SGCN_FJ_P(true, true, 1); }
+      else if (add1) { if (add2) SGCN_FJ_P(true, true, 0); else SGCN_FJ_P(true, false, 0); }
+      else { if (add2) SGCN_FJ_P(false, true, 0); else SGCN_FJ_P(false, false, 0); }
 #undef SGCN_FJ_P
 #undef SGCN_FJ_T
 #undef SGCN_FJ_L
@@ -1459,18 +1476,18 @@
     if (pp)
       gcn_dx_finish_kernel<true, true, true, true><<<B * C, kThreads, 0, st>>>(
           dxt, x0, m, add1, add2, dx, dmask_part, prev_s, prev_mean, prev_invstd, pp, C, T, V,
-          add2_mask);
+          add2_mask, flags);
     else
       gcn_dx_finish_kernel<true, true, false, true><<<B * C, kThreads, 0, st>>>(
           dxt, x0, m, add1, add2, dx, dmask_part, prev_s, prev_mean, prev_invstd, pp, C, T, V,
-          add2_mask);
+          add2_mask, flags);
     SGCN_LAUNCH_CHECK();
     return 0;
   }
 #define SGCN_FIN(A1, A2, PT)                                                                \
   gcn_dx_finish_kernel<A1, A2, PT><<<B * C, kThreads, 0, st>>>(                           \
       dxt, x0, m, add1, add2, dx, dmask_part, prev_s, prev_mean, prev_invstd, pp, C, T, V,  \
-      nullptr)
+      nullptr, flags)
 #define SGCN_FIN_P(A1, A2)                                                                  \
   do {                                                                                      \
     if (pp) SGCN_FIN(A1, A2, true);                                                         \
diff --git a/shift-gcn_amd/csrc/head.hip b/shift-gcn_amd/csrc/head.hip
--- a/shift-gcn_amd/csrc/head.hip
+++ b/shift-gcn_amd/csrc/head.hip
@@ -188,6 +188,18 @@
   }
 }
 
+__global__ __launch_bounds__(kHT) void pool_bwd_planes_kernel(const float* __restrict__ dout,
+                                                              float* __restrict__ dplane,
+                                                              long long rows, int C, int M,
+                                                              long long P) {
+  const long long row = (long long)blockIdx.x * kHT + threadIdx.x;
+  if (row >= rows) return;
+  const float rm = 1.f / (float)M, rp = 1.f / (float)P;
+  const int c = (int)(row % C);
+  const long long n = row / C / M;
+  dplane[row] = (dout[n * C + c] * rm) * rp;
+}
+
 unsigned grid1(long long total) { return (unsigned)((total + kHT - 1) / kHT); }
 
 }
@@ -273,4 +285,16 @@
   return 0;
 }
 
-}
+int sgcn_pool_bwd_planes(const float* dout, float* dplane, int N, int M, int C, long long P,
+                         void* stream) {
+  SGCN_REQUIRE(N >= 0 && M > 0 && C > 0 && P > 0);
+  const long long rows = (long long)N * M * C;
+  if (rows == 0) return 0;
+  SGCN_REQUIRE(dout && dplane && rows < (1ll << 31));
+  pool_bwd_planes_kernel<<<grid1(rows), kHT, 0, (hipStream_t)stream>>>(dout, dplane, rows, C, M,
+                                                                       P);
+  SGCN_LAUNCH_CHECK();
+  return 0;
+}
+
+}
diff --git a/shift-gcn_amd/csrc/tshift.hip b/shift-gcn_amd/csrc/tshift.hip
--- a/shift-gcn_amd/csrc/tshift.hip
+++ b/shift-gcn_amd/csrc/tshift.hip
@@ -766,7 +766,7 @@
   }
 }
 
-template <int NT, int LPT, bool AFFINE, bool RELU_MASK, bool BNP, bool GP, bool GBN,
+template <int NT, int LPT, bool AFFINE, bool RELU_MASK, bool BNP, int GP, bool GBN,
           bool GBD = false>
 __global__ __launch_bounds__(NT) void tshift_bwd_ra_kernel(
     const float* __restrict__ gout, const float* __restrict__ in,
@@ -779,7 +779,7 @@
     const float* __restrict__ gz, const float* __restrict__ gzm,
     const float* __restrict__ gzi, float* __restrict__ gzpart, const float* __restrict__ gd = nullptr,
     const float* __restrict__ gdm = nullptr, const float* __restrict__ gdi = nullptr,
-    float* __restrict__ gdpart = nullptr) {
+    float* __restrict__ gdpart = nullptr, int gdyp = 0) {
   SGCN_CRIT_PRIO();
   static_assert(!GBN || (AFFINE && BNP && !GP), "GBN: shift_in with BNP");
   static_assert(!GBD || GBN, "GBD extends GBN");
@@ -805,21 +805,34 @@
   {
     const auto inr = make_rsrc(in + poff, nbytes);
     if (GP) {
-      const auto dyr = make_rsrc(gdy + poff, nbytes);
-      const auto yr = make_rsrc(gy + poff, nbytes);
       const auto xr = make_rsrc(gx + poff, nbytes);
-      float u1[LPT], u2[LPT];
+      float u1[GP == 1 ? LPT : 1], u2[LPT];
+      if (gdyp) {
+        const float pv = gdy[plane];
+#pragma unroll
+        for (int e = 0; e < LPT; ++e) t[e] = pv;
+      } else {
+        const auto dyr = make_rsrc(gdy + poff, nbytes);
+#pragma unroll
+        for (int e = 0; e < LPT; ++e) t[e] = bload(dyr, vo + e * vstep, 0);
+      }
+      if (GP == 1) {
+        const auto yr = make_rsrc(gy + poff, nbytes);
+#pragma unroll
+        for (int e = 0; e < LPT; ++e) u1[e] = bload(yr, vo + e * vstep, 0);
+      }
 #pragma unroll
       for (int e = 0; e < LPT; ++e) {
         const unsigned vb = vo + e * vstep;
-        t[e] = bload(dyr, vb, 0);
-        u1[e] = bload(yr, vb, 0);
         u2[e] = bload(xr, vb, 0);
         rin_r[e] = bload(inr, vb, 0);
       }
       const float k1 = gcoef[c], k2 = gcoef[C + c], k3 = gcoef[2 * C + c];
 #pragma unroll
-      for (int e = 0; e < LPT; ++e) t[e] = k1 * (u1[e] > 0.f ? t[e] : 0.f) + k2 * u2[e] + k3;
+      for (int e = 0; e < LPT; ++e) {
+        const float gm = GP == 1 ? (u1[e] > 0.f ? t[e] : 0.f) : t[e];
+        t[e] = k1 * gm + k2 * u2[e] + k3;
+      }
     } else {
       const auto gr = make_rsrc(gout + poff, gbytes);
 #pragma unroll
@@ -1221,21 +1234,21 @@
 }
 constexpr size_t kRaLdsMax = 65536;
 
-template <bool AFFINE, bool RELU, bool BNP, bool GP, bool GBN, bool GBD = false>
+template <bool AFFINE, bool RELU, bool BNP, int GP, bool GBN, bool GBD = false>
 bool launch_ra(int nt, const float* gout, const float* in, const float* xpos,
                const float* ypos, const float* scale, const float* shift, const float* bmu,
                const float* bis, float* gin, float2* pg, float2* bp, int B, int C, int H,
                int W, const float* gdy, const float* gy, const float* gx, const float* gcoef,
                const float* gz, const float* gzm, const float* gzi, float* gzpart,
                hipStream_t st, const float* gd = nullptr, const float* gdm = nullptr,
-               const float* gdi = nullptr, float* gdpart = nullptr) {
+               const float* gdi = nullptr, float* gdpart = nullptr, int gdyp = 0) {
   const int lpt = ra_lpt(H * W, nt, W);
   const size_t lds = ra_lds_bytes(H, W, nt, GBN);
   if (lpt == 0 || lds > kRaLdsMax) return false;
 #define SGCN_RA(NT, L)                                                                         \
   tshift_bwd_ra_kernel<NT, L, AFFINE, RELU, BNP, GP, GBN, GBD><<<B * C, NT, lds, st>>>(        \
       gout, in, xpos, ypos, scale, shift, bmu, bis, gin, pg, bp, C, H, W, gdy, gy, gx, gcoef,  \
-      gz, gzm, gzi, gzpart, gd, gdm, gdi, gdpart)
+      gz, gzm, gzi, gzpart, gd, gdm, gdi, gdpart, gdyp)
   if (nt == 256) {
     if (lpt == 8) SGCN_RA(256, 8); else if (lpt == 16) SGCN_RA(256, 16); else if (lpt == 24) SGCN_RA(256, 24); else SGCN_RA(256, 32);
   } else {
@@ -1435,10 +1448,10 @@
 int sgcn_tshift_bwd_bnin(const float* dy, const float* y, const float* s, const float* coef,
                          const float* in, const float* xpos, const float* ypos, float* gin,
                          float* gx, float* gy, void* ws, size_t ws_bytes, int B, int C, int H,
-                         int W, int ypos_is_raw, void* stream) {
+                         int W, int ypos_is_raw, int dy_plane, void* stream) {
   SGCN_REQUIRE(B > 0 && C > 0 && H > 0 && W > 0);
   SGCN_REQUIRE(H * W <= kBwdLdsMax);
-  SGCN_REQUIRE(dy && y && s && coef && in && xpos && ypos && gin && ws);
+  SGCN_REQUIRE(dy && s && coef && in && xpos && ypos && gin && ws);
   SGCN_REQUIRE((gx == nullptr) == (gy == nullptr));
   SGCN_REQUIRE(ws_bytes >= sgcn_tshift_bwd_ws_bytes(B, C));
   SGCN_REQUIRE((long long)B * C < (1LL << 31));
@@ -1446,9 +1459,16 @@
   hipStream_t st = (hipStream_t)stream;
   float2* pg = (float2*)ws;
   const int ntb = H * W <= 4096 ? 256 : 512;
-  const bool ok = launch_ra<false, true, false, true, false>(
-      ntb, nullptr, in, xpos, ypos, nullptr, nullptr, nullptr, nullptr, gin, pg, nullptr, B, C,
-      H, W, dy, y, s, coef, nullptr, nullptr, nullptr, nullptr, st);
+  const int dyp = dy_plane != 0;
+  const bool ok =
+      y ? launch_ra<false, true, false, 1, false>(
+              ntb, nullptr, in, xpos, ypos, nullptr, nullptr, nullptr, nullptr, gin, pg, nullptr,
+              B, C, H, W, dy, y, s, coef, nullptr, nullptr, nullptr, nullptr, st, nullptr,
+              nullptr, nullptr, nullptr, dyp)
+        : launch_ra<false, true, false, 2, false>(
+              ntb, nullptr, in, xpos, ypos, nullptr, nullptr, nullptr, nullptr, gin, pg, nullptr,
+              B, C, H, W, dy, nullptr, s, coef, nullptr, nullptr, nullptr, nullptr, st, nullptr,
+              nullptr, nullptr, nullptr, dyp);
   SGCN_REQUIRE(ok);
   SGCN_LAUNCH_CHECK();
   if (gx) tshift_pos_finalize_kernel<<<(C + 3) / 4, 256, 0, st>>>(pg, B, C, gx, gy);
diff --git a/shift-gcn_amd/shiftgcn/_lib.py b/shift-gcn_amd/shiftgcn/_lib.py
--- a/shift-gcn_amd/shiftgcn/_lib.py
+++ b/shift-gcn_amd/shiftgcn/_lib.py
@@ -8,7 +8,7 @@
 LIB_NAME = "libshiftgcn_hip.so"
 LIB_PATH = os.path.join(os.path.dirname(os.path.abspath(__file__)), LIB_NAME)
 LIB_PATH = os.environ.get("SGCN_LIB_PATH", LIB_PATH)
-ABI_VERSION = 23
+ABI_VERSION = 24
 BATCH_MAX = 32
 ABI_DIAG_FLAG = 0x10000
 EINVAL = -22
@@ -54,16 +54,16 @@
     "sgcn_bn_apply": (_I, [_P, _P, _P, _I, _P, _P, _P, _I, _P, _P, _P, _P, _I, _I, _I, _I,
                            _P]),
     "sgcn_bn_bwd_reduce": (_I, [_P, _P, _I, _P, _P, _P, _I, _P, _P, _P, _P, _P, _P, _I, _I, _I,
-                                _I, _P]),
+                                _I, _I, _P]),
     "sgcn_bn_bwd_finalize": (_I, [_P, _I, _I, _L, _I, _P, _P, _P, _P, _P, _I, _I, _P, _P]),
     "sgcn_bn_bwd_apply": (_I, [_P, _P, _I, _P, _P, _I, _P, _P, _P, _P, _P, _I, _I, _I, _I,
                                _P]),
     "sgcn_mask_prep": (_I, [_P, _P, _I, _P]),
     "sgcn_gcn_gather": (_I, [_P, _P, _P, _I, _I, _I, _I, _P]),
     "sgcn_gcn_dx_finish": (_I, [_P, _P, _P, _P, _P, _P, _P, _P, _P, _P, _P, _P, _I, _I, _I, _I,
-                                _P]),
+                                _I, _P]),
     "sgcn_tshift_bwd_bnin": (_I, [_P, _P, _P, _P, _P, _P, _P, _P, _P, _P, _P, _Z, _I, _I, _I,
-                                  _I, _I, _P]),
+                                  _I, _I, _I, _P]),
     "sgcn_mask_grad_finalize": (_I, [_P, _P, _I, _I, _I, _P, _I, _P]),
     "sgcn_modalities": (_I, [_P, _P, _P, _P, _P, _P, _P, _P, _I, _I, _I, _I, _I, _I, _P]),
     "sgcn_tshift_bwd_gbn": (_I, [_P, _P, _P, _P, _P, _P, _P, _P, _P, _P, _P, _P, _P, _P, _P, _P,
@@ -77,6 +77,7 @@
     "sgcn_head_bwd_apply": (_I, [_P, _P, _P, _P, _I, _I, _I, _I, _I, _P]),
     "sgcn_pool": (_I, [_P, _P, _I, _I, _I, _L, _P]),
     "sgcn_pool_bwd": (_I, [_P, _P, _I, _I, _I, _L, _P]),
+    "sgcn_pool_bwd_planes": (_I, [_P, _P, _I, _I, _I, _L, _P]),
     "sgcn_tshift_pos_finalize_many": (_I, [_P, _P, _P, _P, _P, _I, _P]),
     "sgcn_mask_prep_many": (_I, [_P, _P, _P, _I, _P]),
     "sgcn_mask_grad_finalize_many": (_I, [_P, _P, _P, _P, _P, _P, _I, _P]),
diff --git a/shift-gcn_amd/shiftgcn/fused.py b/shift-gcn_amd/shiftgcn/fused.py
--- a/shift-gcn_amd/shiftgcn/fused.py
+++ b/shift-gcn_amd/shiftgcn/fused.py
@@ -220,8 +220,9 @@
 
 
 def gcn_backward(mod, s: GcnSaved, dH, extra_dx=None, dy_coef=None, prev=None, extra_out=None,
-                 pre6=None, off=False):
+                 pre6=None, off=False, mask_dx=False):
     x0 = s.x0
+    assert not (mask_dx and mod.has_down)
     B, Cin, T, V = x0.shape
     Cout = mod.out_channels
     g = {}
@@ -266,9 +267,10 @@
     if prev is not None:
         dx, mpart, extra_out["prev_part"] = ops.gcn_dx_finish(dXt, x0, s.m, add1=g_id,
                                                               add2=a2, prev=prev,
-                                                              add2_mask=a2m)
-    else:
-        dx, mpart = ops.gcn_dx_finish(dXt, x0, s.m, add1=g_id, add2=a2, add2_mask=a2m)
+                                                              add2_mask=a2m, mask_dx=mask_dx)
+    else:
+        dx, mpart = ops.gcn_dx_finish(dXt, x0, s.m, add1=g_id, add2=a2, add2_mask=a2m,
+                                      mask_dx=mask_dx)
     dmask = ops.grad_like(mod.Feature_Mask)
     fm = mod.Feature_Mask
     if BATCH_SIDE and (off or _defer_ok((fm,))):
@@ -467,7 +469,7 @@
 
 
 class UnitSaved:
-    __slots__ = ("x", "gs", "ts", "rs", "out", "prev", "off")
+    __slots__ = ("x", "gs", "ts", "rs", "out", "prev", "off", "pm")
 
 
 def unit_forward(unit, x, training):
@@ -491,6 +493,9 @@
         return out, None
     prev = unit.__dict__.pop("_prev_tail", None)
     prev = prev[1:] if prev is not None and prev[0] is x else None
+    pm = unit.__dict__.pop("_prev_out", None)
+    pm = pm[1] if (pm is not None and pm[0] is x and unit.residual_kind != "conv" and
+                   not unit.gcn1.has_down) else None
     off = (ASYNC_DW and bool(unit.__dict__.get("_off_path")) and
            not torch.cuda.is_current_stream_capturing())
     mp = None
@@ -526,9 +531,11 @@
     if (nxt is not None and unit.residual_kind != "conv" and nxt.residual_kind != "conv"
             and not nxt.gcn1.has_down):
         nxt.__dict__["_prev_tail"] = (out, (S, sst), unit)
+    if nxt is not None:
+        nxt.__dict__["_prev_out"] = (out, unit)
     s = UnitSaved()
     s.x, s.gs, s.ts, s.rs, s.out, s.prev = x, gs, ts, rs, out, prev
-    s.off = off
+    s.off, s.pm = off, pm
     return out, s
 
 
@@ -551,6 +558,21 @@
     return _unit_backward(unit, s, dout, _off_path_ok(unit, s))
 
 
+def _premask_ok(unit, x, off):
+    if not PREMASK or torch.cuda.is_current_stream_capturing():
+        return False
+    if getattr(x, "_backward_hooks", None) or x.retains_grad or x.grad_fn is None:
+        return False
+    if not off:
+        params = [p for p in unit.parameters() if p.requires_grad]
+        if not params or not _defer_ok(params):
+            return False
+    try:
+        return bool(torch._C._will_engine_execute_node(x.grad_fn))
+    except RuntimeError:
+        return False
+
+
 def _unit_backward(unit, s: UnitSaved, dout, off):
     ts = s.ts
     S = ts.S
@@ -558,29 +580,35 @@
     B, Cout, To, V = S.shape
     kind = unit.residual_kind
     g = {}
+    pmk = unit.__dict__.pop("_premasked", None)
+    masked = pmk is not None and pmk is dout
+    y, relu = (None, False) if masked else (s.out, True)
+    mask_dx = s.pm is not None and _premask_ok(unit, s.x, off)
     cached = unit.__dict__.pop("_bwd_part", None)
     if cached is not None and cached[0] is dout and kind != "conv":
         part, rpart = cached[1], None
     elif kind == "conv":
-        part, rpart = ops.bn_bwd_reduce(dout, s.out, True, S, ts.sst, False, r=s.rs.Rc,
+        part, rpart = ops.bn_bwd_reduce(dout, y, relu, S, ts.sst, False, r=s.rs.Rc,
                                         rst=s.rs.rst)
     else:
-        part, rpart = ops.bn_bwd_reduce(dout, s.out, True, S, ts.sst, False)
+        part, rpart = ops.bn_bwd_reduce(dout, y, relu, S, ts.sst, False)
     coef2, g["tcn1.bn2.weight"], g["tcn1.bn2.bias"] = ops.bn_bwd_finalize(
         part, B, Cout, B * To * V, ts.sst, unit.tcn1.bn2)
     if kind != "conv" and so.stride == 1 and ops.ra_fits(To * V, V):
         fo = {}
         (dA, coefA), gt = tcn_core_backward(unit.tcn1, ts, None, materialize_dx=False,
-                                            gpre=(dout, s.out, coef2), gcn_z=_gcn_z(unit, s),
+                                            gpre=(dout, y, coef2), gcn_z=_gcn_z(unit, s),
                                             out=fo, off=off)
         g.update({"tcn1." + k: v for k, v in gt.items()})
         extra = {}
         dx, gg = gcn_backward(unit.gcn1, s.gs, dA,
-                              extra_dx=(dout, s.out) if kind == "identity" else None,
+                              extra_dx=(dout, y) if kind == "identity" else None,
                               dy_coef=coefA, prev=None if s.prev is None else s.prev[0],
-                              extra_out=extra, pre6=fo.get("pre6"), off=off)
+                              extra_out=extra, pre6=fo.get("pre6"), off=off, mask_dx=mask_dx)
         if s.prev is not None:
             s.prev[1].__dict__["_bwd_part"] = (dx, extra["prev_part"])
+        if mask_dx:
+            s.pm.__dict__["_premasked"] = dx
         g.update({"gcn1." + k: v for k, v in gg.items()})
         return dx, g
     dS = torch.empty_like(S)
@@ -589,13 +617,13 @@
         coefR, g["residual.bn.weight"], g["residual.bn.bias"] = ops.bn_bwd_finalize(
             rpart, B, Cout, B * To * V, s.rs.rst, unit.residual.bn)
         dres = torch.empty_like(s.rs.Rc)
-        ops.bn_bwd_apply(dout, s.out, True, S, coef2, False, r=s.rs.Rc, rcoef=coefR, dr=dres,
+        ops.bn_bwd_apply(dout, y, relu, S, coef2, False, r=s.rs.Rc, rcoef=coefR, dr=dres,
                          dx=dS)
     elif kind == "identity":
         dres = torch.empty_like(s.x)
-        ops.bn_bwd_apply(dout, s.out, True, S, coef2, False, dr=dres, dx=dS)
-    else:
-        ops.bn_bwd_apply(dout, s.out, True, S, coef2, False, dx=dS)
+        ops.bn_bwd_apply(dout, y, relu, S, coef2, False, dr=dres, dx=dS)
+    else:
+        ops.bn_bwd_apply(dout, y, relu, S, coef2, False, dx=dS)
     fo = {}
     (dA, coefA), gt = tcn_core_backward(unit.tcn1, ts, dS, materialize_dx=False,
                                         gcn_z=_gcn_z(unit, s), out=fo, off=off)
@@ -603,9 +631,11 @@
     extra = {}
     dx, gg = gcn_backward(unit.gcn1, s.gs, dA, extra_dx=dres if kind == "identity" else None,
                           dy_coef=coefA, prev=None if s.prev is None else s.prev[0],
-                          extra_out=extra, pre6=fo.get("pre6"), off=off)
+                          extra_out=extra, pre6=fo.get("pre6"), off=off, mask_dx=mask_dx)
     if s.prev is not None:
         s.prev[1].__dict__["_bwd_part"] = (dx, extra["prev_part"])
+    if mask_dx:
+        s.pm.__dict__["_premasked"] = dx
     g.update({"gcn1." + k: v for k, v in gg.items()})
     if kind == "conv":
         gr = convbn_dx_and_dw(unit.residual, s.rs, dres, dx, accumulate=True, off=off)
@@ -618,6 +648,7 @@
 EVAL_FOLD = int(os.environ.get("SGCN_EVAL_FOLD", "1"))
 GBN_FUSION = int(os.environ.get("SGCN_GBN_FUSION", "2"))
 ASYNC_DW = int(os.environ.get("SGCN_ASYNC_DW", "1"))
+PREMASK = int(os.environ.get("SGCN_PREMASK", "1"))
 
 
 def trainable(module):
@@ -646,7 +677,8 @@
                 "called a second time; its saved activations are released after the first "
                 "backward (retain_graph=True / double backward is not supported)")
         _, bwd = ctx.impl
-        dx, grads = bwd(ctx.module, ctx.saved, dy.contiguous())
+        dyp = _plane_dy(ctx, dy)
+        dx, grads = bwd(ctx.module, ctx.saved, dy.contiguous() if dyp is None else dyp)
         ctx.saved = None
         out = []
         for n, p in zip(ctx.names, ctx.params):
@@ -658,6 +690,18 @@
         return (None, None, dx) + tuple(out)
 
 
+def _plane_dy(ctx, dy):
+    if not (PREMASK and ctx.impl is UNIT_IMPL and dy.dim() == 4 and dy.stride(2) == 0 and
+            dy.stride(3) == 0 and isinstance(ctx.saved, UnitSaved)):
+        return None
+    unit = ctx.module
+    To, V = dy.shape[2], dy.shape[3]
+    if (unit.residual_kind == "conv" or unit.tcn1.shift_out.stride != 1 or
+            not ops.ra_fits(To * V, V)):
+        return None
+    return dy[:, :, 0, 0].contiguous()
+
+
 class _InferFlag(threading.local):
     active = False
 
diff --git a/shift-gcn_amd/shiftgcn/head.py b/shift-gcn_amd/shiftgcn/head.py
--- a/shift-gcn_amd/shiftgcn/head.py
+++ b/shift-gcn_amd/shiftgcn/head.py
@@ -2,7 +2,7 @@
 
 import torch
 
-from . import ops
+from . import fused, ops
 
 
 def _batch_stats(bn) -> bool:
@@ -46,6 +46,9 @@
 
     @staticmethod
     def backward(ctx, g):
+        if fused.PREMASK:
+            dp = ops.pool_bwd(g.contiguous(), ctx.shape, ctx.N, ctx.M, planes=True)
+            return dp[:, :, None, None].expand(ctx.shape), None, None
         return ops.pool_bwd(g.contiguous(), ctx.shape, ctx.N, ctx.M), None, None
 
 
diff --git a/shift-gcn_amd/shiftgcn/ops.py b/shift-gcn_amd/shiftgcn/ops.py
--- a/shift-gcn_amd/shiftgcn/ops.py
+++ b/shift-gcn_amd/shiftgcn/ops.py
@@ -410,21 +410,32 @@
 BNIN_MAX_PLANE = 16384
 
 
+def _plane_dy(dy, x):
+    if dy.dim() == 2:
+        if tuple(dy.shape) != tuple(x.shape[:2]):
+            raise ValueError(f"per-plane gradient {tuple(dy.shape)} of planes {tuple(x.shape)}")
+        return True
+    return False
+
+
 def tshift_bwd_bnin(dy, y, s, coef, inp, xpos, ypos, defer_pos=False, pos_out=None):
     for t, n in ((dy, "dy"), (y, "y"), (s, "s"), (inp, "input"), (coef, "coef")):
-        check_input(t, n)
+        if t is not None:
+            check_input(t, n)
     B, C, H, W = inp.shape
+    dyp = _plane_dy(dy, inp)
     lib = _lib.load()
     dev = inp.device
     gin = torch.empty_like(inp)
     nbytes = lib.sgcn_tshift_bwd_ws_bytes(B, C)
     ws = torch.empty((max(nbytes, 4) + 3) // 4, device=dev, dtype=_F32)
     gx, gy, pp = _pos_out(defer_pos, ws, B, C, dev, pos_out)
-    nb = 4 * (3 * dy.numel() + 2 * inp.numel())
+    nb = 4 * (dy.numel() + (2 + (y is not None)) * s.numel() + inp.numel())
     with _timed("tshift_bwd", 0, nb, inp, _shp(inp)):
         rc = lib.sgcn_tshift_bwd_bnin(
             _ptr(dy), _ptr(y), _ptr(s), _ptr(coef), _ptr(inp), _ptr(xpos), _ptr(ypos),
-            _ptr(gin), _ptr(gx), _ptr(gy), _ptr(ws), nbytes, B, C, H, W, 1, _stream(inp))
+            _ptr(gin), _ptr(gx), _ptr(gy), _ptr(ws), nbytes, B, C, H, W, 1, int(dyp),
+            _stream(inp))
     _lib.check(rc, "sgcn_tshift_bwd_bnin")
     return gin, (pp if pp is not None else gx), gy
 
@@ -634,16 +645,18 @@
                   dy_coef=None):
     check_input(dy, "grad_output")
     B, C, T, V = x.shape
+    dyp = _plane_dy(dy, x)
     dev = x.device
     part = torch.empty((B * C * (V if per_joint else 1) * 2,), device=dev, dtype=_F32)
     rpart = torch.empty((B * C * 2,), device=dev, dtype=_F32) if r is not None else None
-    nb = 4 * x.numel() * (2 + (y is not None) + (r is not None))
+    nb = 4 * (dy.numel() + x.numel() * (1 + (y is not None) + (r is not None)))
     with _timed("bn_bwd_reduce", 0, nb, x, _shp(x)):
         rc = _lib.load().sgcn_bn_bwd_reduce(_ptr(dy), _ptr(y), int(relu), _ptr(x),
                                             _ptr(st.mean), _ptr(st.invstd), int(per_joint),
                                             _ptr(r), _ptr(rst.mean) if rst else None,
                                             _ptr(rst.invstd) if rst else None, _ptr(dy_coef),
-                                            _ptr(part), _ptr(rpart), B, C, T, V, _stream(x))
+                                            _ptr(part), _ptr(rpart), B, C, T, V, int(dyp),
+                                            _stream(x))
     _lib.check(rc, "sgcn_bn_bwd_reduce")
     return part, rpart
 
@@ -764,19 +777,22 @@
     return xg
 
 
-def gcn_dx_finish(dxt, x0, m, add1=None, add2=None, prev=None, add2_mask=None):
+def gcn_dx_finish(dxt, x0, m, add1=None, add2=None, prev=None, add2_mask=None,
+                  mask_dx=False):
     B, C, T, V = dxt.shape
+    flags = int(bool(mask_dx)) | (2 if add2 is not None and _plane_dy(add2, dxt) else 0)
     dx = torch.empty_like(dxt)
     part = torch.empty((B * C * V,), device=dxt.device, dtype=_F32)
     pp = torch.empty((B * C * 2,), device=dxt.device, dtype=_F32) if prev is not None else None
     ps, pst = prev if prev is not None else (None, None)
-    nb = 4 * dxt.numel() * (3 + sum(t is not None for t in (add1, add2, add2_mask, ps)))
+    nb = 4 * (dxt.numel() * (3 + sum(t is not None for t in (add1, add2_mask, ps))) +
+              (add2.numel() if add2 is not None else 0))
     with _timed("gcn_dx_finish", 0, nb, dxt, _shp(dxt)):
         rc = _lib.load().sgcn_gcn_dx_finish(_ptr(dxt), _ptr(x0), _ptr(m), _ptr(add1),
                                             _ptr(add2), _ptr(add2_mask), _ptr(dx), _ptr(part),
                                             _ptr(ps), _ptr(pst.mean) if pst else None,
                                             _ptr(pst.invstd) if pst else None, _ptr(pp), B, C,
-                                            T, V, _stream(dxt))
+                                            T, V, flags, _stream(dxt))
     _lib.check(rc, "sgcn_gcn_dx_finish")
     return (dx, part) if prev is None else (dx, part, pp)
 
@@ -842,11 +858,20 @@
     return out
 
 
-def pool_bwd(dout, shape, N, M):
+def pool_bwd(dout, shape, N, M, planes=False):
     check_input(dout, "grad_output")
+    C = shape[1]
+    P = 1
+    for d in shape[2:]:
+        P *= d
+    if planes:
+        dp = torch.empty((N * M, C), device=dout.device, dtype=_F32)
+        with _timed("pool", 0, 4 * (dout.numel() + dp.numel()), dout):
+            rc = _lib.load().sgcn_pool_bwd_planes(_ptr(dout), _ptr(dp), N, M, C, P,
+                                                  _stream(dout))
+        _lib.check(rc, "sgcn_pool_bwd_planes")
+        return dp
     dx = torch.empty(shape, device=dout.device, dtype=_F32)
-    C = shape[1]
-    P = dx.numel() // max(1, N * M * C)
     with _timed("pool", 0, 4 * dx.numel(), dout):
         rc = _lib.load().sgcn_pool_bwd(_ptr(dout), _ptr(dx), N, M, C, P, _stream(dout))
     _lib.check(rc, "sgcn_pool_bwd")
diff --git a/shift-gcn_amd/shiftgcn/shift_gcn.py b/shift-gcn_amd/shiftgcn/shift_gcn.py
--- a/shift-gcn_amd/shiftgcn/shift_gcn.py
+++ b/shift-gcn_amd/shiftgcn/shift_gcn.py
@@ -200,5 +200,6 @@
             u.__dict__.pop("_next_unit", None)
             u.__dict__.pop("_off_path", None)
             u.__dict__.pop("_prev_tail", None)
+            u.__dict__.pop("_prev_out", None)
             u.gcn1.__dict__.pop("_gather_cache", None)
             u.gcn1.__dict__.pop("_mask_ready", None)
```

After: 2063 clips/s (median of 6 runs). 1.03x the previous value.
